# fauzanardh/OsuFusion

Measured on AMD Instinct MI355X. Metric: denoise-steps/sec (train fwd+bwd) at B=32 L=4096, higher is better.
Workload: dtype bf16; 1 GPU; full OsuFusion UNet dim_h=256 (343.5M params) train step: fwd+bwd+grad-norm+clip+AdamW, per-GPU batch 32, L=4096, x (B,6,L), audio (B,96,L) [BASELINE 'audio-ctx=1024x128' maps to the (B,1024,L/8) bottleneck code]; global_batch=32, seq_len=4096, parallelism=dp1

## Files before the change

### include/osufusion_hip.h

```cpp
#ifndef OSUFUSION_HIP_H
#define OSUFUSION_HIP_H

#include <hip/hip_runtime_api.h>

#ifdef __cplusplus
extern "C" {
#endif

#define OSUF_DT_F32 0
#define OSUF_DT_BF16 1
#define OSUF_DT_F32X3 2
#define OSUF_ATTN_AUTO 0
#define OSUF_ATTN_PLAIN 1
#define OSUF_ATTN_PIPE 2
#define OSUF_DQ_ATOMIC 0
#define OSUF_DQ_SLABS 1
#define OSUF_DQ_ATOMIC_256 2
#define OSUF_DQ_ATOMIC_512 3
#define OSUF_DQ_ATOMIC_512A 5
#define OSUF_DQ_PREZEROED 0x100

int osuf_version(void);

int osuf_gemm_nt(int dtype, const void* A, long lda, const void* W, long ldw, long tapstride,
                 void* C, long ldc, void* C2, long ldc2, const void* R, long ldr, const void* U, long ldu,
                 const float* bias, const float* rscale, double* stats,
                 int M, int N, int K, int taps, int Lin, int Lout, int stride, int pad, int mode, int act,
                 hipStream_t stream);

int osuf_gemm_nt_rowdot(int dtype, const void* A, long lda, const void* W, long ldw, void* C, long ldc, const void* O, long ldo,
                        float* delta, int M, int N, int K, int L, int heads, hipStream_t stream);

int osuf_gemm_tn(int dtype, const void* dY, long ldy, const void* X, long ldx, float* dW, long ldw, long tapstride,
                 int M, int N1, int N2, int taps, int Lin, int Lout, int stride, int pad, int mode,
                 int splits, int out_layout, int accumulate, float* workspace, long workspace_bytes, hipStream_t stream);
long osuf_gemm_tn_workspace_bytes(int dtype, int M, int N1, int N2, int taps);
int osuf_gemm_tn_bias(int dtype, const void* dY, long ldy, const void* X, long ldx, float* dW, long ldw, long tapstride,
                      int M, int N1, int N2, int taps, int Lin, int Lout, int stride, int pad, int mode,
                      int splits, int out_layout, int accumulate, float* workspace, long workspace_bytes, float* dbias, hipStream_t stream);

int osuf_colsum(int dtype, const void* Y, long ldy, int M, int N, float* out, hipStream_t stream);

int osuf_gn_finalize(const double* stats, float* mean_rstd, int B, long count, hipStream_t stream);
int osuf_gn_stats(int dtype, const void* y, long ldy, double* partial, float* mean_rstd, int M, int C, int L, hipStream_t stream);
long osuf_gn_stats_workspace_bytes(int M, int C, int L);
int osuf_gn_apply_fwd(int dtype, const void* y, long ldy, void* h, long ldh, const float* mean_rstd, const float* gamma,
                      const float* beta, const float* scale_shift, int M, int C, int L, hipStream_t stream);
int osuf_gn_apply_fwd_stats(int dtype, const void* y, long ldy, void* h, long ldh, const double* stats, long count, float* mr_out,
                            const float* gamma, const float* beta, const float* ss, int M, int C, int L, hipStream_t stream);
int osuf_gn_stats_parts(int dtype, const void* y, long ldy, double* partial, int M, int C, int L, hipStream_t stream);
int osuf_gn_apply_fwd_parts(int dtype, const void* y, long ldy, void* h, long ldh, const double* partial, float* mr_out,
                            const float* gamma, const float* beta, const float* ss, int M, int C, int L, hipStream_t stream);
int osuf_gn_bwd(int dtype, const void* dh, long lddh, const void* y, long ldy, void* dy, long lddy, const float* mean_rstd,
                const float* gamma, const float* beta, const float* scale_shift, float* T1234, float* S, float* dss,
                float* dgamma, float* dbeta, float* dbias, float* dyy, int M, int C, int L, hipStream_t stream);

int osuf_ln_fwd(int dtype, const void* x, long ldx, void* out, long ldo, float* mean_rstd, const float* gamma, const float* beta,
                int M, int C, hipStream_t stream);
int osuf_ln_bwd(int dtype, const void* dy, long lddy, const void* x, long ldx, void* dx, long lddx, const float* mean_rstd,
                const float* gamma, float* dgamma, float* dbeta, int M, int C, hipStream_t stream);

int osuf_rowdot(int dtype, const void* h, long ldh, const float* w, long w_stride, const float* bias, float* out,
                int M, int C, int L, hipStream_t stream);
long osuf_gca_pool_workspace_bytes(int M, int C, int L);
int osuf_gca_pool(int dtype, const void* h, long ldh, const float* wk, const float* bk, float* part, float* p, float* pooled,
                  int M, int C, int L, hipStream_t stream);
int osuf_softmax_rows(float* p, int B, int L, hipStream_t stream);
int osuf_wcolsum(int dtype, const void* a, long lda, const void* bmul, long ldb, const float* w, float* out,
                 int B, int C, int L, float* partial, hipStream_t stream);
int osuf_gate_residual(int dtype, const void* h, long ldh, const float* gate, const void* res, long ldr, void* out, long ldo,
                       int M, int C, int L, hipStream_t stream);
int osuf_gca_bwd_apply(int dtype, const void* dout, long lddo, const void* h, long ldh, void* dh, long lddh, const float* p,
                       const float* gate, const float* dpooled, const float* sdot, const float* wk, float* dlogit,
                       int M, int C, int L, float* dwk, float* dbk, float* workspace, long workspace_bytes, hipStream_t stream);
long osuf_gca_bwd_apply_workspace_bytes(int M, int C);

int osuf_rope_cast(int dtype, const void* in, long ld_in, void* out_bf16, long ld_out, const float* cos_tab, const float* sin_tab,
                   int M, int N, int n_rot_heads, int n_heads_total, int head_dim, hipStream_t stream);
int osuf_rope_cast_qs(int dtype, const void* in, long ld_in, void* out_bf16, long ld_out, const float* cos_tab, const float* sin_tab,
                      int M, int N, int n_rot_heads, int n_heads_total, int head_dim, float q_mul, int n_q_heads, hipStream_t stream);
int osuf_rope_bwd(int dtype, const float* in, long ld_in, void* out, long ld_out, const float* cos_tab, const float* sin_tab,
                  int M, int N, int n_rot_heads, int n_heads_total, int head_dim, hipStream_t stream);
int osuf_mqa_fwd(const void* q, long ldq, const void* k, long ldk, const void* v, long ldv, void* o, long ldo, int o_dtype,
                 float* lse2, int B, int H, int N, int head_dim, float scale, hipStream_t stream);
int osuf_gqa_fwd(const void* q, long ldq, const void* k, long ldk, const void* v, long ldv, void* o, long ldo, int o_dtype,
                 float* lse2, int B, int H, int G, int N, int head_dim, float scale, hipStream_t stream);
int osuf_mqa_fwd_qs(const void* q, long ldq, const void* k, long ldk, const void* v, long ldv, void* o, long ldo, int o_dtype,
                    float* lse2, int B, int H, int N, int head_dim, float scale, hipStream_t stream);
int osuf_mqa_fwd_zdq(const void* q, long ldq, const void* k, long ldk, const void* v, long ldv, void* o, long ldo, int o_dtype,
                     float* lse2, int B, int H, int N, int head_dim, float scale, int qs, float* zero_dq, hipStream_t stream);
int osuf_mqa_fwd_rope(const void* q_raw, long ldq, const void* k, long ldk, const void* v, long ldv, void* o, long ldo, int o_dtype,
                      float* lse2, int B, int H, int N, int head_dim, float scale, const float* rope_cos, const float* rope_sin,
                      float q_mul, void* q_out, long ldqo, float* zero_dq, hipStream_t stream);
int osuf_mqa_fwd_masked(const void* q, long ldq, const void* k, long ldk, const void* v, long ldv, void* o, long ldo, int o_dtype,
                        float* lse2, const void* mask, long mask_b, long mask_h, long mask_q, long mask_k, int B, int H, int N,
                        int head_dim, float scale, hipStream_t stream);
int osuf_mqa_bwd_masked(const void* q, long ldq, const void* k, long ldk, const void* v, long ldv, const void* dout, long lddo,
                        const float* lse2, const float* delta, const void* mask, long mask_b, long mask_h, long mask_q, long mask_k,
                        void* dq, long lddq, void* dk, void* dv, long lddk, int B, int H, int N, int head_dim, float scale,
                        int out_dtype, float* dbias, hipStream_t stream);
int osuf_xattn_fwd(const void* q, long ldq, const void* k, long ldk, const void* v, long ldv, void* o, long ldo, int o_dtype,
                   float* lse2, const void* mask, long mask_b, long mask_h, long mask_q, long mask_k, int B, int H, int Nq, int Nk,
                   int head_dim, float scale, hipStream_t stream);
int osuf_xattn_bwd(const void* q, long ldq, const void* k, long ldk, const void* v, long ldv, const void* dout, long lddo,
                   const float* lse2, const float* delta, const void* mask, long mask_b, long mask_h, long mask_q, long mask_k,
                   void* dq, long lddq, void* dk, void* dv, long lddk, int B, int H, int Nq, int Nk, int head_dim, float scale,
                   int out_dtype, float* dbias, hipStream_t stream);
int osuf_attn_delta(const void* dout, long lddo, const void* o, long ldo, int o_dtype, float* delta, int B, int H, int N,
                    int head_dim, hipStream_t stream);
int osuf_mqa_bwd_dq(const void* q, long ldq, const void* k, long ldk, const void* v, long ldv, const void* dout, long lddo,
                    const float* lse2, const float* delta, void* dq, long lddq, int B, int H, int N, int head_dim, float scale,
                    int out_dtype, const float* rope_cos, const float* rope_sin, int variant, hipStream_t stream);
int osuf_mqa_bwd_dkv(const void* q, long ldq, const void* k, long ldk, const void* v, long ldv, const void* dout, long lddo,
                     const float* lse2, const float* delta, void* dk, void* dv, long lddk, int B, int H, int N, int head_dim,
                     float scale, int out_dtype, const float* rope_cos, const float* rope_sin, float* workspace, long workspace_bytes,
                     int qsplit, int variant, hipStream_t stream);
long osuf_mqa_bwd_dkv_workspace_bytes(int B, int N, int qsplit);

int osuf_mqa_bwd_fused(const void* q, long ldq, const void* k, long ldk, const void* v, long ldv, const void* dout, long lddo,
                       const float* lse2, const float* delta, void* dq, long lddq, void* dk, void* dv, long lddk, int B, int H,
                       int N, int head_dim, float scale, int out_dtype, const float* rope_cos, const float* rope_sin,
                       float* workspace, long workspace_bytes, int qsplit, int dq_mode, hipStream_t stream);
int osuf_mqa_bwd_fused_qs(const void* q, long ldq, const void* k, long ldk, const void* v, long ldv, const void* dout, long lddo,
                          const float* lse2, const float* delta, void* dq, long lddq, void* dk, void* dv, long lddk, int B, int H,
                          int N, int head_dim, float scale, int out_dtype, const float* rope_cos, const float* rope_sin,
                          float* workspace, long workspace_bytes, int qsplit, int dq_mode, hipStream_t stream);
long osuf_mqa_bwd_fused_workspace_bytes(int B, int H, int N, int out_dtype, int qsplit, int dq_mode);

int osuf_ncl_to_rows(int dtype, const float* in, void* out, long ld, int width, int B, int C, int L, int KT, hipStream_t stream);
int osuf_rows_to_ncl(int dtype, const void* in, long ld, float* out, int B, int C, int L, hipStream_t stream);
int osuf_copy2d(int src_dtype, const void* src, long lds, int dst_dtype, void* dst, long ldd, int M, int cols, hipStream_t stream);
int osuf_add2d(int dtype, const void* a, long lda, const void* b, long ldb, void* dst, long ldd, int M, int cols, hipStream_t stream);
int osuf_axpby_rows(const float* x, const float* y, const float* ca, const float* cb, float* out, int B, long per_sample, hipStream_t stream);
int osuf_ddim_step(const float* x, const float* cond, const float* nullp, float cond_scale, const float* coef, float* out,
                   int B, long per_sample, hipStream_t stream);
int osuf_ct_schedule(const float* t, const float* t_next, int kind, float* out, int B, hipStream_t stream);
int osuf_ct_step(const float* x, const float* cond, const float* nullp, float cond_scale, const float* coef, const float* noise,
                 float* out, int B, long per_sample, hipStream_t stream);
#define OSUF_CT_OBJ_NOISE 0
#define OSUF_CT_OBJ_X_START 1
#define OSUF_CT_OBJ_V 2
int osuf_ct_step_ex(const float* x, const float* cond, const float* nullp, float cond_scale, const float* coef, const float* noise,
                    int objective, const float* s, long s_ld, float* out, int B, long per_sample, hipStream_t stream);
int osuf_ct_x0_quantile(const float* x, const float* cond, const float* nullp, float cond_scale, const float* coef, int objective,
                        long k_lo, float frac, float* out, void* workspace, int B, long per_sample, hipStream_t stream);
long osuf_ct_x0_quantile_workspace_bytes(int B);
int osuf_ct_qsample(const float* x0, const float* noise, const float* sched, int sched_ld, int objective, float* x_noisy, float* target,
                    int B, long per_sample, hipStream_t stream);
#define OSUF_CT_SAMPLER_DDIM 0
#define OSUF_CT_SAMPLER_DPMPP_2M 1
int osuf_ct_solver_schedule(const float* log_snr, int steps, int sampler, float eta, float* rows, float* fac, int B, hipStream_t stream);
int osuf_ct_solver_step(const float* x, const float* cond, const float* nullp, float cond_scale, const float* coef, const float* fac,
                        const float* x0_prev, const float* noise, int objective, const float* s, long s_ld, float* x_next, float* x0, int B,
                        long per_sample, hipStream_t stream);
int osuf_mse(const float* pred, const float* target, const int* orig_len, float* grad, double* loss_sum, int B, int Dch, int L,
             hipStream_t stream);
int osuf_mse_w(const float* pred, const float* target, const int* orig_len, const float* w, float* grad, double* loss_sum, int B, int Dch,
               int L, hipStream_t stream);
int osuf_sqnorm(const float* g, long n, double* out, hipStream_t stream);
int osuf_adamw(float* p, const float* g, float* m, float* v, long n, float lr, float beta1, float beta2, float eps, float wd,
               int step, const float* gscale, hipStream_t stream);
int osuf_clip_coef(const double* sumsq, float max_norm, float base, float* coef, float* total_norm, hipStream_t stream);
int osuf_cast_f32_bf16(const float* src, void* dst, long n, hipStream_t stream);
int osuf_pack_weight(const float* w, int O, int I, int k, int out_dtype, void* F, long f_ld, long f_tapstride, void* D, long d_ld,
                     long d_tapstride, int dkind, hipStream_t stream);

#ifndef OSUF_PACK_DESC_DEFINED
#define OSUF_PACK_DESC_DEFINED
typedef struct osuf_pack_desc {
  const float* w;
  void* F;
  void* D;
  long f_ld, f_tapstride, d_ld, d_tapstride;
  int O, I, k, dkind;
  int block0, reserved;
} osuf_pack_desc;
#endif
int osuf_pack_weight_group(const osuf_pack_desc* descs, int n, int total_blocks, int out_dtype, hipStream_t stream);

int osuf_dora_effective(const float* W, const float* A, const float* B, const float* mag, int O, int IK, int r, float scaling,
                        float* Weff, float* g, hipStream_t stream);
int osuf_dora_gain(const float* W, const float* A, const float* B, const float* mag, int O, int I, int k, int r, float scaling,
                   float* partial, float* g, float* sgbt32, void* sgbt16, hipStream_t stream);
int osuf_pack_weight_adapted(const float* w, const float* A, const float* B, const float* g, float scaling, int r, int O, int I, int k,
                             int out_dtype, void* F, long f_ld, long f_tapstride, void* D, long d_ld, long d_tapstride, int dkind,
                             hipStream_t stream);
int osuf_adapter_finish(const float* tb, const float* sg, float* dB, const float* gt, float* dA, const float* s0, const float* s1,
                        const float* bias, const float* m, float* dm, int O, int I, int k, int r, int accumulate, hipStream_t stream);

int osuf_skinny_fwd(int mode, const float* x, long ldx, const float* W, const float* bias, float* y, long ldy, int M, int N, int K,
                    int in_act, int out_act, hipStream_t stream);
int osuf_skinny_bwd(int mode, const float* dy, long lddy, const float* y, long ldy, const float* x, long ldx, const float* W,
                    float* dx, long lddx, float* dW, float* db, int M, int N, int K, int in_act, int out_act, int accumulate,
                    hipStream_t stream);

#ifndef OSUF_LINEAR_DESC_DEFINED
#define OSUF_LINEAR_DESC_DEFINED
typedef struct osuf_linear_desc {
  const float* W;
  const float* bias;
  float* y;
  const float* dy;
  long ldy, lddy;
  int N, block0;
} osuf_linear_desc;
#endif
int osuf_skinny_fwd_group(int mode, const float* x, long ldx, const osuf_linear_desc* descs, int n, int total_blocks, int M, int K,
                          int in_act, hipStream_t stream);
int osuf_skinny_dx_group(int mode, const osuf_linear_desc* descs, int n, int total_slices, const float* x, long ldx, float* dx, long lddx,
                         int M, int K, int in_act, hipStream_t stream);

int osuf_log_vqt(const float* wave_pad, long n_pad, const float* bank, int K, int bins, int hop, const float* scale, float eps,
                 float* spec_ws, float* out, long ldo, long frames, hipStream_t stream);
int osuf_vqt_logmag(const float* spec, long ld, float* out, long ldo, const float* scale, int bins, long frames, float eps,
                    hipStream_t stream);

int osuf_fir_decimate2(const float* in, long n_in, const float* taps, int ntaps, float* out, long n_out, hipStream_t stream);
int osuf_frame_rows(const float* in, long n_in, int hop, int K, float* out, long frames, hipStream_t stream);

int osuf_adaln_fwd(int dtype, const void* x, long ldx, void* out, long ldo, float* mr, const float* shift, const float* scale, long ldm,
                   int M, int C, int L, float eps, hipStream_t stream);
long osuf_adaln_bwd_workspace_bytes(int M, int C, int L);
int osuf_adaln_bwd(int dtype, const void* dy, long lddy, const void* x, long ldx, const void* dres, long ldr, void* dx, long lddx,
                   const float* mr, const float* scale, long ldm, float* dmod, long ldd, long off2, float* workspace, long workspace_bytes,
                   int M, int C, int L, hipStream_t stream);
int osuf_qknorm_fwd(int dtype, const void* x, long ldx, void* y, long ldy, float* inv, const float* gamma_q, const float* gamma_k,
                    int M, int H, int D, hipStream_t stream);
long osuf_qknorm_bwd_workspace_bytes(int M, int H, int D);
int osuf_qknorm_bwd(int dtype, const float* g, long ldg, const void* x, long ldx, const float* inv, const float* gamma_q,
                    const float* gamma_k, void* dx, long lddx, float* dgamma, float* workspace, long workspace_bytes,
                    int M, int H, int D, hipStream_t stream);
int osuf_stat_pool(const float* a, float* out, int B, int C, int L, hipStream_t stream);

int osuf_joint_qknorm_fwd(int dtype, const void* x, long ldx, void* y, long ldy, float* inv, const float* gamma_q, const float* gamma_k,
                          int M, int Ns, int Nj, int off, int H, int G, int D, hipStream_t stream);
int osuf_joint_pack(int dtype, const void* x, long ldx, void* joint, long ldj, int M, int Ns, int Nj, int off, int H, int G, int D,
                    hipStream_t stream);
int osuf_joint_unpack(int dtype, const void* joint, long ldj, void* out, long ldo, int M, int Ns, int Nj, int off, int H, int G, int D,
                      hipStream_t stream);
long osuf_joint_qknorm_bwd_workspace_bytes(int M, int H, int G, int D);
int osuf_joint_qknorm_bwd(int dtype, const float* g, long ldg, const void* x, long ldx, const float* inv, const float* gamma_q,
                          const float* gamma_k, void* dx, long lddx, float* dgamma, float* workspace, long workspace_bytes,
                          int M, int Ns, int Nj, int off, int H, int G, int D, hipStream_t stream);

int osuf_clock_probe(int blocks, int iters, int mode, long* out, hipStream_t stream);

#ifdef __cplusplus
}
#endif
#endif
```

### osufusion_amd/_lib.py

```python
from __future__ import annotations

import ctypes
import os
from ctypes import c_double, c_float, c_int, c_long, c_void_p
from pathlib import Path

_CSRC = Path(__file__).resolve().parent / "csrc"
LIB_PATH = Path(os.environ["OSUF_HIP_LIB"]).resolve() if os.environ.get("OSUF_HIP_LIB") else _CSRC / "libosuf_hip.so"

P, L, I, F = c_void_p, c_long, c_int, c_float

SIGNATURES = {
    "osuf_version": [],
    "osuf_gemm_nt": [I, P, L, P, L, L, P, L, P, L, P, L, P, L, P, P, P, I, I, I, I, I, I, I, I, I, I, P],
    "osuf_gemm_nt_rowdot": [I, P, L, P, L, P, L, P, L, P, I, I, I, I, I, P],
    "osuf_gemm_tn": [I, P, L, P, L, P, L, L, I, I, I, I, I, I, I, I, I, I, I, I, P, L, P],
    "osuf_gemm_tn_bias": [I, P, L, P, L, P, L, L, I, I, I, I, I, I, I, I, I, I, I, I, P, L, P, P],
    "osuf_gemm_tn_workspace_bytes": [I, I, I, I, I],
    "osuf_colsum": [I, P, L, I, I, P, P],
    "osuf_gn_finalize": [P, P, I, L, P],
    "osuf_gn_apply_fwd": [I, P, L, P, L, P, P, P, P, I, I, I, P],
    "osuf_gn_apply_fwd_stats": [I, P, L, P, L, P, L, P, P, P, P, I, I, I, P],
    "osuf_gn_bwd": [I, P, L, P, L, P, L, P, P, P, P, P, P, P, P, P, P, P, I, I, I, P],
    "osuf_ln_fwd": [I, P, L, P, L, P, P, P, I, I, P],
    "osuf_ln_bwd": [I, P, L, P, L, P, L, P, P, P, P, I, I, P],
    "osuf_rowdot": [I, P, L, P, L, P, P, I, I, I, P],
    "osuf_softmax_rows": [P, I, I, P],
    "osuf_wcolsum": [I, P, L, P, L, P, P, I, I, I, P, P],
    "osuf_gn_stats": [I, P, L, P, P, I, I, I, P],
    "osuf_gca_pool": [I, P, L, P, P, P, P, P, I, I, I, P],
    "osuf_gca_pool_workspace_bytes": [I, I, I],
    "osuf_gn_stats_parts": [I, P, L, P, I, I, I, P],
    "osuf_gn_apply_fwd_parts": [I, P, L, P, L, P, P, P, P, P, I, I, I, P],
    "osuf_gn_stats_workspace_bytes": [I, I, I],
    "osuf_gate_residual": [I, P, L, P, P, L, P, L, I, I, I, P],
    "osuf_gca_bwd_apply": [I, P, L, P, L, P, L, P, P, P, P, P, P, I, I, I, P, P, P, L, P],
    "osuf_gca_bwd_apply_workspace_bytes": [I, I],
    "osuf_rope_cast": [I, P, L, P, L, P, P, I, I, I, I, I, P],
    "osuf_rope_cast_qs": [I, P, L, P, L, P, P, I, I, I, I, I, F, I, P],
    "osuf_rope_bwd": [I, P, L, P, L, P, P, I, I, I, I, I, P],
    "osuf_mqa_fwd": [P, L, P, L, P, L, P, L, I, P, I, I, I, I, F, P],
    "osuf_gqa_fwd": [P, L, P, L, P, L, P, L, I, P, I, I, I, I, I, F, P],
    "osuf_mqa_fwd_qs": [P, L, P, L, P, L, P, L, I, P, I, I, I, I, F, P],
    "osuf_mqa_fwd_zdq": [P, L, P, L, P, L, P, L, I, P, I, I, I, I, F, I, P, P],
    "osuf_mqa_fwd_rope": [P, L, P, L, P, L, P, L, I, P, I, I, I, I, F, P, P, F, P, L, P, P],
    "osuf_mqa_fwd_masked": [P, L, P, L, P, L, P, L, I, P, P, L, L, L, L, I, I, I, I, F, P],
    "osuf_mqa_bwd_masked": [P, L, P, L, P, L, P, L, P, P, P, L, L, L, L, P, L, P, P, L, I, I, I, I, F, I, P, P],
    "osuf_xattn_fwd": [P, L, P, L, P, L, P, L, I, P, P, L, L, L, L, I, I, I, I, I, F, P],
    "osuf_xattn_bwd": [P, L, P, L, P, L, P, L, P, P, P, L, L, L, L, P, L, P, P, L, I, I, I, I, I, F, I, P, P],
    "osuf_attn_delta": [P, L, P, L, I, P, I, I, I, I, P],
    "osuf_mqa_bwd_dq": [P, L, P, L, P, L, P, L, P, P, P, L, I, I, I, I, F, I, P, P, I, P],
    "osuf_mqa_bwd_dkv": [P, L, P, L, P, L, P, L, P, P, P, P, L, I, I, I, I, F, I, P, P, P, L, I, I, P],
    "osuf_mqa_bwd_dkv_workspace_bytes": [I, I, I],
    "osuf_mqa_bwd_fused": [P, L, P, L, P, L, P, L, P, P, P, L, P, P, L, I, I, I, I, F, I, P, P, P, L, I, I, P],
    "osuf_mqa_bwd_fused_qs": [P, L, P, L, P, L, P, L, P, P, P, L, P, P, L, I, I, I, I, F, I, P, P, P, L, I, I, P],
    "osuf_mqa_bwd_fused_workspace_bytes": [I, I, I, I, I, I],
    "osuf_ncl_to_rows": [I, P, P, L, I, I, I, I, I, P],
    "osuf_rows_to_ncl": [I, P, L, P, I, I, I, P],
    "osuf_copy2d": [I, P, L, I, P, L, I, I, P],
    "osuf_add2d": [I, P, L, P, L, P, L, I, I, P],
    "osuf_axpby_rows": [P, P, P, P, P, I, L, P],
    "osuf_ddim_step": [P, P, P, F, P, P, I, L, P],
    "osuf_ct_schedule": [P, P, I, P, I, P],
    "osuf_ct_step": [P, P, P, F, P, P, P, I, L, P],
    "osuf_ct_step_ex": [P, P, P, F, P, P, I, P, L, P, I, L, P],
    "osuf_ct_x0_quantile": [P, P, P, F, P, I, L, F, P, P, I, L, P],
    "osuf_ct_x0_quantile_workspace_bytes": [I],
    "osuf_ct_qsample": [P, P, P, I, I, P, P, I, L, P],
    "osuf_ct_solver_schedule": [P, I, I, F, P, P, I, P],
    "osuf_ct_solver_step": [P, P, P, F, P, P, P, P, I, P, L, P, P, I, L, P],
    "osuf_mse": [P, P, P, P, P, I, I, I, P],
    "osuf_mse_w": [P, P, P, P, P, P, I, I, I, P],
    "osuf_sqnorm": [P, L, P, P],
    "osuf_adamw": [P, P, P, P, L, F, F, F, F, F, I, P, P],
    "osuf_clip_coef": [P, F, F, P, P, P],
    "osuf_cast_f32_bf16": [P, P, L, P],
    "osuf_pack_weight": [P, I, I, I, I, P, L, L, P, L, L, I, P],
    "osuf_pack_weight_group": [P, I, I, I, P],
    "osuf_dora_effective": [P, P, P, P, I, I, I, F, P, P, P],
    "osuf_dora_gain": [P, P, P, P, I, I, I, I, F, P, P, P, P, P],
    "osuf_adapter_finish": [P, P, P, P, P, P, P, P, P, P, I, I, I, I, I, P],
    "osuf_pack_weight_adapted": [P, P, P, P, F, I, I, I, I, I, P, L, L, P, L, L, I, P],
    "osuf_clock_probe": [I, I, I, P, P],
    "osuf_log_vqt": [P, L, P, I, I, I, P, F, P, P, L, L, P],
    "osuf_vqt_logmag": [P, L, P, L, P, I, L, F, P],
    "osuf_fir_decimate2": [P, L, P, I, P, L, P],
    "osuf_frame_rows": [P, L, I, I, P, L, P],
    "osuf_skinny_fwd": [I, P, L, P, P, P, L, I, I, I, I, I, P],
    "osuf_skinny_bwd": [I, P, L, P, L, P, L, P, P, L, P, P, I, I, I, I, I, I, P],
    "osuf_skinny_fwd_group": [I, P, L, P, I, I, I, I, I, P],
    "osuf_skinny_dx_group": [I, P, I, I, P, L, P, L, I, I, I, P],
    "osuf_adaln_fwd": [I, P, L, P, L, P, P, P, L, I, I, I, F, P],
    "osuf_adaln_bwd_workspace_bytes": [I, I, I],
    "osuf_adaln_bwd": [I, P, L, P, L, P, L, P, L, P, P, L, P, L, L, P, L, I, I, I, P],
    "osuf_qknorm_fwd": [I, P, L, P, L, P, P, P, I, I, I, P],
    "osuf_qknorm_bwd_workspace_bytes": [I, I, I],
    "osuf_qknorm_bwd": [I, P, L, P, L, P, P, P, P, L, P, P, L, I, I, I, P],
    "osuf_stat_pool": [P, P, I, I, I, P],
    "osuf_joint_qknorm_fwd": [I, P, L, P, L, P, P, P, I, I, I, I, I, I, I, P],
    "osuf_joint_pack": [I, P, L, P, L, I, I, I, I, I, I, I, P],
    "osuf_joint_unpack": [I, P, L, P, L, I, I, I, I, I, I, I, P],
    "osuf_joint_qknorm_bwd_workspace_bytes": [I, I, I, I],
    "osuf_joint_qknorm_bwd": [I, P, L, P, L, P, P, P, P, L, P, P, L, I, I, I, I, I, I, I, P],
}

_lib = None


class HipExtensionMissing(RuntimeError):
    pass


def load(build_if_missing: bool = True) -> ctypes.CDLL:
    global _lib
    if _lib is not None:
        return _lib
    if not LIB_PATH.exists() and build_if_missing:
        try:
            from .csrc import build as _build
            _build.build()
        except Exception as e:
            raise HipExtensionMissing(f"libosuf_hip.so is missing and could not be built: {e}") from e
    if not LIB_PATH.exists():
        raise HipExtensionMissing(f"{LIB_PATH} not found: run `python -c 'import __graft_entry__ as g; g.build()'`")
    try:
        lib = ctypes.CDLL(str(LIB_PATH), mode=os.RTLD_NOW | os.RTLD_LOCAL)
    except OSError as e:
        raise HipExtensionMissing(f"cannot load {LIB_PATH}: {e}") from e
    for name, argtypes in SIGNATURES.items():
        try:
            fn = getattr(lib, name)
        except AttributeError as e:
            raise HipExtensionMissing(f"{LIB_PATH} does not export {name} (stale or partial build of the C ABI)") from e
        fn.argtypes = argtypes
        fn.restype = c_long if name.endswith("_bytes") else c_int
    _lib = lib
    return lib


def check(status: int, what: str) -> None:
    if status != 0:
        kind = {-1: "invalid argument", -2: "unsupported configuration"}.get(status, f"hipError {status}")
        raise RuntimeError(f"{what} failed: {kind}")
```

### osufusion_amd/csrc/common.hpp

```cpp
#pragma once
#include <hip/hip_runtime.h>
#include <stdint.h>

#ifndef OSUF_PACK_DESC_DEFINED
#define OSUF_PACK_DESC_DEFINED
typedef struct osuf_pack_desc {
  const float* w;
  void* F;
  void* D;
  long f_ld, f_tapstride, d_ld, d_tapstride;
  int O, I, k, dkind;
  int block0, reserved;
} osuf_pack_desc;
#endif
static_assert(sizeof(osuf_pack_desc) == 80, "osuf_pack_desc is part of the C ABI");
#ifndef OSUF_LINEAR_DESC_DEFINED
#define OSUF_LINEAR_DESC_DEFINED
typedef struct osuf_linear_desc {
  const float* W;
  const float* bias;
  float* y;
  const float* dy;
  long ldy, lddy;
  int N, block0;
} osuf_linear_desc;
#endif
static_assert(sizeof(osuf_linear_desc) == 56, "osuf_linear_desc is part of the C ABI");

#define OSUF_DT_F32 0
#define OSUF_DT_BF16 1
#define OSUF_DT_F32X3 2
#define OSUF_ATTN_AUTO 0
#define OSUF_ATTN_PLAIN 1
#define OSUF_ATTN_PIPE 2
#define OSUF_DQ_ATOMIC 0
#define OSUF_DQ_SLABS 1
#define OSUF_DQ_ATOMIC_256 2
#define OSUF_DQ_ATOMIC_512 3
#define OSUF_DQ_ATOMIC_512A 5
#define OSUF_DQ_PREZEROED 0x100

typedef uint16_t bf16_t;
typedef __attribute__((ext_vector_type(4))) float f32x4;
typedef __attribute__((ext_vector_type(16))) float f32x16;
typedef __attribute__((ext_vector_type(8))) __bf16 bf16x8;
typedef __attribute__((ext_vector_type(4))) short s16x4;
typedef __attribute__((ext_vector_type(4))) uint32_t u32x4;
typedef __attribute__((ext_vector_type(2))) uint32_t u32x2;

#define LDS_PTR(T) __attribute__((address_space(3))) T*

__device__ __forceinline__ float bf16_to_f32(bf16_t v) { return __uint_as_float(((uint32_t)v) << 16); }

__device__ __forceinline__ bf16_t f32_to_bf16(float f) {
  __bf16 b = (__bf16)f;
  return __builtin_bit_cast(uint16_t, b);
}
__device__ __forceinline__ uint32_t pack_bf16x2(float lo, float hi) {
  typedef __attribute__((ext_vector_type(2))) float f32x2_t;
  typedef __attribute__((ext_vector_type(2))) __bf16 bf16x2_t;
  f32x2_t v = {lo, hi};
  return __builtin_bit_cast(uint32_t, __builtin_convertvector(v, bf16x2_t));
}
__device__ __forceinline__ float round_bf16(float f) { return bf16_to_f32(f32_to_bf16(f)); }

template <typename T> struct ElemTraits;
template <> struct ElemTraits<float> {
  static constexpr int kPer16B = 4;
  __device__ static __forceinline__ float load(const float* p) { return *p; }
  __device__ static __forceinline__ void store(float* p, float v) { *p = v; }
  __device__ static __forceinline__ float rnd(float v) { return v; }
};
template <> struct ElemTraits<bf16_t> {
  static constexpr int kPer16B = 8;
  __device__ static __forceinline__ float load(const bf16_t* p) { return bf16_to_f32(*p); }
  __device__ static __forceinline__ void store(bf16_t* p, float v) { *p = f32_to_bf16(v); }
  __device__ static __forceinline__ float rnd(float v) { return round_bf16(v); }
};

__device__ __forceinline__ void load8(const bf16_t* p, float (&v)[8]) {
  u32x4 r = *reinterpret_cast<const u32x4*>(p);
#pragma unroll
  for (int i = 0; i < 4; ++i) {
    v[2 * i] = __uint_as_float(r[i] << 16);
    v[2 * i + 1] = __uint_as_float(r[i] & 0xFFFF0000u);
  }
}
__device__ __forceinline__ void load8(const float* p, float (&v)[8]) {
  f32x4 a = *reinterpret_cast<const f32x4*>(p);
  f32x4 b = *reinterpret_cast<const f32x4*>(p + 4);
#pragma unroll
  for (int i = 0; i < 4; ++i) { v[i] = a[i]; v[4 + i] = b[i]; }
}
__device__ __forceinline__ void store8(bf16_t* p, const float (&v)[8]) {
  u32x4 r;
#pragma unroll
  for (int i = 0; i < 4; ++i) r[i] = pack_bf16x2(v[2 * i], v[2 * i + 1]);
  *reinterpret_cast<u32x4*>(p) = r;
}
__device__ __forceinline__ void store8(float* p, const float (&v)[8]) {
  f32x4 a, b;
#pragma unroll
  for (int i = 0; i < 4; ++i) { a[i] = v[i]; b[i] = v[4 + i]; }
  *reinterpret_cast<f32x4*>(p) = a;
  *reinterpret_cast<f32x4*>(p + 4) = b;
}
__device__ __forceinline__ void load4(const bf16_t* p, float (&v)[4]) {
  u32x2 r = *reinterpret_cast<const u32x2*>(p);
  v[0] = __uint_as_float(r[0] << 16); v[1] = __uint_as_float(r[0] & 0xFFFF0000u);
  v[2] = __uint_as_float(r[1] << 16); v[3] = __uint_as_float(r[1] & 0xFFFF0000u);
}
__device__ __forceinline__ void load4(const float* p, float (&v)[4]) {
  f32x4 a = *reinterpret_cast<const f32x4*>(p);
  v[0] = a[0]; v[1] = a[1]; v[2] = a[2]; v[3] = a[3];
}
__device__ __forceinline__ void store4(bf16_t* p, const float (&v)[4]) {
  u32x2 r; r[0] = pack_bf16x2(v[0], v[1]); r[1] = pack_bf16x2(v[2], v[3]);
  *reinterpret_cast<u32x2*>(p) = r;
}
__device__ __forceinline__ void store4(float* p, const float (&v)[4]) {
  f32x4 a; a[0] = v[0]; a[1] = v[1]; a[2] = v[2]; a[3] = v[3];
  *reinterpret_cast<f32x4*>(p) = a;
}

__device__ __forceinline__ float sigmoid_f(float x) { return __builtin_amdgcn_rcpf(1.0f + __expf(-x)); }
__device__ __forceinline__ float silu_f(float x) { return x * sigmoid_f(x); }
__device__ __forceinline__ float silu_grad_f(float x) {
  float s = sigmoid_f(x);
  return s * (1.0f + x * (1.0f - s));
}

template <int WIDTH = 64> __device__ __forceinline__ float group_sum(float v) {
#pragma unroll
  for (int o = WIDTH >> 1; o > 0; o >>= 1) v += __shfl_xor(v, o, 64);
  return v;
}
template <int WIDTH = 64> __device__ __forceinline__ float group_max(float v) {
#pragma unroll
  for (int o = WIDTH >> 1; o > 0; o >>= 1) v = fmaxf(v, __shfl_xor(v, o, 64));
  return v;
}
__device__ __forceinline__ float group_sum_dyn(float v, int width) {
  for (int o = width >> 1; o > 0; o >>= 1) v += __shfl_xor(v, o, 64);
  return v;
}
__device__ __forceinline__ float group_max_dyn(float v, int width) {
  for (int o = width >> 1; o > 0; o >>= 1) v = fmaxf(v, __shfl_xor(v, o, 64));
  return v;
}

__device__ __forceinline__ void atomic_add_f64(double* p, double v) { unsafeAtomicAdd(p, v); }
__device__ __forceinline__ void atomic_add_f32(float* p, float v) { unsafeAtomicAdd(p, v); }

#define OSUF_OK 0
#define OSUF_EINVAL (-1)
#define OSUF_EUNSUPPORTED (-2)

static inline int osuf_launch_status() {
  hipError_t e = hipGetLastError();
  return e == hipSuccess ? OSUF_OK : (int)e;
}

#define DISPATCH_T(dtype, ...)                                  \
  if ((dtype) == OSUF_DT_BF16) { using T = bf16_t; __VA_ARGS__; } \
  else if ((dtype) == OSUF_DT_F32) { using T = float; __VA_ARGS__; } \
  else return OSUF_EUNSUPPORTED;
static inline int ew_grid(long total_threads) {
  long blocks = (total_threads + 255) / 256;
  if (blocks > 2048) blocks = 2048;
  if (blocks < 1) blocks = 1;
  return (int)blocks;
}
static inline bool al16(const void* p) { return (reinterpret_cast<uintptr_t>(p) & 15) == 0; }
static inline bool bad_c(int C) { return C <= 0 || (C & 7) || C > 2048; }

template <auto KERNEL> static void allow_lds(int bytes) {
  static const bool once = ((void)hipFuncSetAttribute((const void*)KERNEL, hipFuncAttributeMaxDynamicSharedMemorySize, bytes), true);
  (void)once;
}
```

### osufusion_amd/csrc/gemm.hip

```cpp
#include "common.hpp"
#include <optional>
#include <stdlib.h>

struct RowMap {
  int Lin, Lout, stride, pad, mode;
};
__device__ __forceinline__ int map_row(const RowMap& rm, int i, int t) {
  if (rm.mode == 3) {
    if (t == 3) return (i == rm.Lout - 2) ? rm.Lin - 1 : -1;
    int e = i - t;
    if (e < 0 || (e & 1)) return -1;
    e >>= 1;
    return e < rm.Lin ? e : -1;
  }
  int s = i * rm.stride + t - rm.pad;
  if (rm.mode == 2) {
    if (s < 0 || s >= 2 * rm.Lin) return -1;
    return s >> 1;
  }
  if (rm.mode == 1 && s == rm.Lin) s = rm.Lin - 2;
  return (s >= 0 && s < rm.Lin) ? s : -1;
}

struct GemmArgs {
// ... 1651 lines not shown
  asm volatile("s_waitcnt lgkmcnt(" #n ")"                                                                        \
               : "+v"(fa[slot][0][0]), "+v"(fa[slot][0][1]), "+v"(fa[slot][1][0]), "+v"(fa[slot][1][1]), "+v"(fb[slot][0][0]),  \
                 "+v"(fb[slot][0][1]), "+v"(fb[slot][1][0]), "+v"(fb[slot][1][1]), "+v"(fb[slot][2][0]), "+v"(fb[slot][2][1]));  \
  __builtin_amdgcn_sched_barrier(0);
#define T3_MFMA(slot)                                                                                             \
  _Pragma("unroll") for (int i = 0; i < 2; ++i) _Pragma("unroll") for (int t = 0; t < 3; ++t) {                   \
    u32x4 va = {fa[slot][i][0][0], fa[slot][i][0][1], fa[slot][i][1][0], fa[slot][i][1][1]};                       \
    u32x4 vb = {fb[slot][t][0][0], fb[slot][t][0][1], fb[slot][t][1][0], fb[slot][t][1][1]};                       \
    acc[i][t] = __builtin_amdgcn_mfma_f32_32x32x16_bf16(__builtin_bit_cast(bf16x8, va), __builtin_bit_cast(bf16x8, vb), acc[i][t], 0, 0, 0); \
  }

  const bool do_bias = g.dbias != nullptr && n2_0 == 0 && wc == 0;
  float bsum[2] = {0.f, 0.f};
#define T3_BIAS(slot)                                                                                             \
  if (do_bias) { _Pragma("unroll") for (int i = 0; i < 2; ++i) bsum[i] = bf16x8_sum(fa[slot][i][0], fa[slot][i][1], bsum[i]); }
  issue(m_begin, 0);
  asm volatile("s_waitcnt vmcnt(0)" ::: "memory");
  __builtin_amdgcn_s_barrier();
  int buf = 0;
  for (int mb = m_begin; mb < m_end; mb += BKM, buf ^= 1) {
    if (mb + BKM < m_end) issue(mb + BKM, buf ^ 1);
    const uint32_t base = lds0 + buf * STAGE;
    T3_READS(0, 0, base)
    T3_READS(1, 1, base)
    T3_WAIT(0, 10)  T3_MFMA(0)  T3_BIAS(0)  T3_READS(0, 2, base)
    T3_WAIT(1, 10)  T3_MFMA(1)  T3_BIAS(1)  T3_READS(1, 3, base)
    T3_WAIT(0, 10)  T3_MFMA(0)  T3_BIAS(0)  T3_READS(0, 4, base)
    T3_WAIT(1, 10)  T3_MFMA(1)  T3_BIAS(1)  T3_READS(1, 5, base)
    T3_WAIT(0, 10)  T3_MFMA(0)  T3_BIAS(0)  T3_READS(0, 6, base)
    T3_WAIT(1, 10)  T3_MFMA(1)  T3_BIAS(1)  T3_READS(1, 7, base)
    T3_WAIT(0, 10)  T3_MFMA(0)  T3_BIAS(0)
    T3_WAIT(1, 0)   T3_MFMA(1)  T3_BIAS(1)
    asm volatile("s_waitcnt vmcnt(0)" ::: "memory");
    __builtin_amdgcn_s_barrier();
  }
#undef T3_READS
#undef T3_WAIT
#undef T3_MFMA
#undef T3_BIAS
  if (do_bias) {
#pragma unroll
    for (int i = 0; i < 2; ++i) {
      const float v = bsum[i] + __shfl_xor(bsum[i], 32, 64);
      const int n1 = n1_0 + wr * 64 + i * 32 + lr;
      if (lh == 0 && n1 < g.N1) atomic_add_f32(g.dbias + n1, v);
    }
  }

  if (g.ws && g.ws_pk) {
#pragma unroll
    for (int t = 0; t < 3; ++t) {
      uint32_t* out = reinterpret_cast<uint32_t*>(g.ws) + ((long)split * 3 + t) * (g.N1 >> 1) * g.N2;
#pragma unroll
      for (int i = 0; i < 2; ++i) {
        const int n2 = n2_0 + wc * 32 + lr;
        if (n2 < g.N2) {
#pragma unroll
          for (int r = 0; r < 16; r += 2) {
            const int n1 = n1_0 + wr * 64 + i * 32 + (r & 3) + 8 * (r >> 2) + 4 * lh;
            if (n1 < g.N1) out[(long)(n1 >> 1) * g.N2 + n2] = pack_bf16x2(acc[i][t][r], acc[i][t][r + 1]);
          }
        }
      }
    }
    return;
  }
#pragma unroll
  for (int t = 0; t < 3; ++t) {
    float* out = g.ws ? g.ws + ((long)split * 3 + t) * g.N1 * g.N2 : g.dW + (long)t * g.tapstride;
#pragma unroll
    for (int i = 0; i < 2; ++i) {
      const int n2 = n2_0 + wc * 32 + lr;
      if (n2 < g.N2) {
#pragma unroll
        for (int r = 0; r < 16; ++r) {
          const int n1 = n1_0 + wr * 64 + i * 32 + (r & 3) + 8 * (r >> 2) + 4 * lh;
          if (n1 < g.N1) {
            if (g.ws) out[(long)n1 * g.N2 + n2] = acc[i][t][r];
            else atomic_add_f32(out + (long)n1 * g.ldw + (long)n2 * g.es, acc[i][t][r]);
          }
        }
      }
    }
  }
}

__global__ __launch_bounds__(512, 2) void gemm_tn_taps3_x3_kernel(WgradArgs g) {
  extern __shared__ __attribute__((aligned(16))) char smem[];
  constexpr int BKM = 64, ROWB = 512, YB = BKM * ROWB, XROWS = 66, STAGE = YB + XROWS * ROWB;
  const int tid = threadIdx.x, lane = tid & 63;
  const int wave = __builtin_amdgcn_readfirstlane(tid >> 6);
  const int wr = wave >> 2, wc = wave & 3;
  const WgradUnit u = wgrad_unit<128>(g, 1);
  const int split = u.split, n1_0 = u.n1_0, n2_0 = u.n2_0, m_begin = u.m_begin, m_end = u.m_end;
  if (m_begin >= m_end) return;
  const float* dY = reinterpret_cast<const float*>(g.dY);
  const float* X = reinterpret_cast<const float*>(g.X);
  const char* zero = reinterpret_cast<const char*>(g_zero_page);
  const int L = g.rm.Lout;
  const int col = (lane & 31) * 4;
  const bool y_ok = n1_0 + col < g.N1, x_ok = n2_0 + col < g.N2;
  int pos = m_begin % L;
  auto issue = [&](int mb, int buf) {
    char* sy = smem + buf * STAGE;
    char* sx = sy + YB;
#pragma unroll
    for (int i = 0; i < 4; ++i) {
      const int m = mb + (wave * 4 + i) * 2 + (lane >> 5);
      const char* qy = (m < m_end && y_ok) ? reinterpret_cast<const char*>(dY + (long)m * g.ldy + n1_0 + col) : zero;
      __builtin_amdgcn_global_load_lds((gas_ptr)qy, (las_ptr)(sy + (wave * 4 + i) * 1024), 16, 0, 0);
    }
#pragma unroll
    for (int i = 0; i < 5; ++i) {
      if (i == 4 && wave != 0) break;
      const int gi = i < 4 ? wave * 4 + i : 32;
      const int pr = gi * 2 + (lane >> 5);
      const int q = pos - 1 + pr;
      const bool ok = q >= 0 && q < L && mb - 1 + pr < g.M && x_ok;
      const char* qx = ok ? reinterpret_cast<const char*>(X + (long)(mb - 1 + pr) * g.ldx + n2_0 + col) : zero;
      __builtin_amdgcn_global_load_lds((gas_ptr)qx, (las_ptr)(sx + gi * 1024), 16, 0, 0);
    }
    pos += BKM;
    if (pos >= L) pos -= L;
  };

  f32x16 acc[2][3];
  zero_acc(acc);

  const int lr = lane & 31, lh = lane >> 5;
  issue(m_begin, 0);
  asm volatile("s_waitcnt vmcnt(0)" ::: "memory");
  __builtin_amdgcn_s_barrier();
  int buf = 0;
  for (int mb = m_begin; mb < m_end; mb += BKM, buf ^= 1) {
    if (mb + BKM < m_end) issue(mb + BKM, buf ^ 1);
    const char* sy = smem + buf * STAGE;
    const char* sx = sy + YB;
#pragma unroll
    for (int kk = 0; kk < 4; ++kk) {
      bf16x8 ah[2], al[2], bh[3], bl[3];
      {
        typedef __attribute__((ext_vector_type(2))) float f32x2;
        f32x2 y[8];
#pragma unroll
        for (int e = 0; e < 8; ++e) y[e] = *reinterpret_cast<const f32x2*>(sy + (16 * kk + 8 * lh + e) * ROWB + (wr * 64 + 2 * lr) * 4);
#pragma unroll
        for (int i = 0; i < 2; ++i) {
          const float x[8] = {y[0][i], y[1][i], y[2][i], y[3][i], y[4][i], y[5][i], y[6][i], y[7][i]};
          split_bf16x8(x, ah[i], al[i]);
        }
      }
      {
        float xw[10];
#pragma unroll
        for (int e = 0; e < 10; ++e) xw[e] = *reinterpret_cast<const float*>(sx + (16 * kk + 8 * lh + e) * ROWB + (wc * 32 + lr) * 4);
#pragma unroll
        for (int t = 0; t < 3; ++t) {
          const float x[8] = {xw[t], xw[t + 1], xw[t + 2], xw[t + 3], xw[t + 4], xw[t + 5], xw[t + 6], xw[t + 7]};
          split_bf16x8(x, bh[t], bl[t]);
        }
      }
#pragma unroll
      for (int i = 0; i < 2; ++i)
#pragma unroll
        for (int t = 0; t < 3; ++t) mfma_x3(acc[i][t], ah[i], al[i], bh[t], bl[t]);
    }
    asm volatile("s_waitcnt vmcnt(0)" ::: "memory");
    __builtin_amdgcn_s_barrier();
  }
#pragma unroll
  for (int t = 0; t < 3; ++t) {
    float* out = g.ws ? g.ws + ((long)split * 3 + t) * g.N1 * g.N2 : g.dW + (long)t * g.tapstride;
#pragma unroll
    for (int i = 0; i < 2; ++i) {
      const int n2 = n2_0 + wc * 32 + lr;
      if (n2 < g.N2) {
#pragma unroll
        for (int r = 0; r < 16; ++r) {
          const int n1 = n1_0 + wr * 64 + 2 * ((r & 3) + 8 * (r >> 2) + 4 * lh) + i;
          if (n1 < g.N1) {
            if (g.ws) out[(long)n1 * g.N2 + n2] = acc[i][t][r];
            else atomic_add_f32(out + (long)n1 * g.ldw + (long)n2 * g.es, acc[i][t][r]);
          }
        }
      }
    }
  }
}

__global__ __launch_bounds__(512, 2) void gemm_tn_skinny_kernel(WgradArgs g) {
  extern __shared__ __attribute__((aligned(16))) char smem[];
  constexpr int BKM = 64, ROWB = 512, TILEB = BKM * ROWB, XTILEB = BKM * 64, STAGE = TILEB + XTILEB;
  const int tid = threadIdx.x, lane = tid & 63;
  const int wave = __builtin_amdgcn_readfirstlane(tid >> 6);
  const int tiles_n1 = (g.N1 + kBig - 1) / kBig;
  const int tile = blockIdx.x % tiles_n1;
  const int t = (blockIdx.x / tiles_n1) % g.taps;
  const int split = blockIdx.x / (tiles_n1 * g.taps);
  const int n1_0 = tile * kBig;
  const int m_begin = split * g.rows_per_split;
  const int m_end = min(g.M, m_begin + g.rows_per_split);
  if (m_begin >= m_end) return;
  const bf16_t* dY = reinterpret_cast<const bf16_t*>(g.dY);
  const bf16_t* X = reinterpret_cast<const bf16_t*>(g.X);
  const char* zero = reinterpret_cast<const char*>(g_zero_page);

  int srow[4], scol[4];
  const char* py[4];
  bool y_ok[4];
#pragma unroll
  for (int i = 0; i < 4; ++i) {
    srow[i] = (wave * 4 + i) * 2 + (lane >> 5);
    scol[i] = ((lane & 31) ^ ((srow[i] & 3) << 2)) * 8;
    y_ok[i] = n1_0 + scol[i] < g.N1;
    py[i] = reinterpret_cast<const char*>(dY + (long)(m_begin + srow[i]) * g.ldy + n1_0 + scol[i]);
  }
  const long ystep = (long)BKM * g.ldy * (long)sizeof(bf16_t);
  const int xrow = wave * 16 + (lane >> 2), xcol = (lane & 3) * 8;
  const bool x_ok = wave < 4 && xcol < g.N2;
  int xb = 0, xp = 0;
  if (wave < 4) { const int m = m_begin + xrow; xb = m / g.rm.Lout; xp = m - xb * g.rm.Lout; }
  auto issue = [&](int mb, int buf) {
    char* sy = smem + buf * STAGE + wave * 4096;
#pragma unroll
    for (int i = 0; i < 4; ++i) {
      const char* qy = (mb + srow[i] < m_end && y_ok[i]) ? py[i] : zero;
      __builtin_amdgcn_global_load_lds((gas_ptr)qy, (las_ptr)(sy + i * 1024), 16, 0, 0);
      py[i] += ystep;
    }
    if (wave < 4) {
      const char* qx = zero;
      if (x_ok && mb + xrow < m_end) {
        const int s2 = map_row(g.rm, xp, t);
        if (s2 >= 0) qx = reinterpret_cast<const char*>(X + (long)(xb * g.rm.Lin + s2) * g.ldx + xcol);
      }
      __builtin_amdgcn_global_load_lds((gas_ptr)qx, (las_ptr)(smem + buf * STAGE + TILEB + wave * 1024), 16, 0, 0);
      xp += BKM;
      while (xp >= g.rm.Lout) { xp -= g.rm.Lout; ++xb; }
    }
  };

  f32x16 acc;
#pragma unroll
  for (int r = 0; r < 16; ++r) acc[r] = 0.f;
  const int lr = lane & 31, lh = lane >> 5;
  const int ip = lane & 15, cb = ((lane >> 4) & 1) * 16, tq = ip >> 2, tp = ip & 3;
  const uint32_t lds0 = (uint32_t)(uintptr_t)(LDS_PTR(char))smem;
  const uint32_t offA = (8 * lh + tq) * ROWB + ((((wave * 32 + cb + 4 * tp) * 2)) ^ (tq << 6));
  const uint32_t offB = TILEB + (8 * lh + tq) * 64 + (cb + 4 * tp) * 2;

  issue(m_begin, 0);
  asm volatile("s_waitcnt vmcnt(0)" ::: "memory");
  __builtin_amdgcn_s_barrier();
  int buf = 0;
  for (int mb = m_begin; mb < m_end; mb += BKM, buf ^= 1) {
    if (mb + BKM < m_end) issue(mb + BKM, buf ^ 1);
    const uint32_t base = lds0 + buf * STAGE;
    u32x2 a0[4], a1[4], b0[4], b1[4];
    OSUF_TR_READ(a0[0], base + offA, 0 * 16 * 512);  OSUF_TR_READ(a1[0], base + offA, (0 * 16 + 4) * 512);
    OSUF_TR_READ(b0[0], base + offB, 0 * 16 * 64);   OSUF_TR_READ(b1[0], base + offB, (0 * 16 + 4) * 64);
    OSUF_TR_READ(a0[1], base + offA, 1 * 16 * 512);  OSUF_TR_READ(a1[1], base + offA, (1 * 16 + 4) * 512);
    OSUF_TR_READ(b0[1], base + offB, 1 * 16 * 64);   OSUF_TR_READ(b1[1], base + offB, (1 * 16 + 4) * 64);
    OSUF_TR_READ(a0[2], base + offA, 2 * 16 * 512);  OSUF_TR_READ(a1[2], base + offA, (2 * 16 + 4) * 512);
    OSUF_TR_READ(b0[2], base + offB, 2 * 16 * 64);   OSUF_TR_READ(b1[2], base + offB, (2 * 16 + 4) * 64);
    OSUF_TR_READ(a0[3], base + offA, 3 * 16 * 512);  OSUF_TR_READ(a1[3], base + offA, (3 * 16 + 4) * 512);
    OSUF_TR_READ(b0[3], base + offB, 3 * 16 * 64);   OSUF_TR_READ(b1[3], base + offB, (3 * 16 + 4) * 64);
    asm volatile("s_waitcnt lgkmcnt(0)"
                 : "+v"(a0[0]), "+v"(a1[0]), "+v"(b0[0]), "+v"(b1[0]), "+v"(a0[1]), "+v"(a1[1]), "+v"(b0[1]), "+v"(b1[1]),
                   "+v"(a0[2]), "+v"(a1[2]), "+v"(b0[2]), "+v"(b1[2]), "+v"(a0[3]), "+v"(a1[3]), "+v"(b0[3]), "+v"(b1[3]));
#pragma unroll
    for (int ks = 0; ks < 4; ++ks) {
      const u32x4 va = {a0[ks][0], a0[ks][1], a1[ks][0], a1[ks][1]};
      const u32x4 vb = {b0[ks][0], b0[ks][1], b1[ks][0], b1[ks][1]};
      acc = __builtin_amdgcn_mfma_f32_32x32x16_bf16(__builtin_bit_cast(bf16x8, va), __builtin_bit_cast(bf16x8, vb), acc, 0, 0, 0);
    }
    asm volatile("s_waitcnt vmcnt(0)" ::: "memory");
    __builtin_amdgcn_s_barrier();
  }
  float* dW = g.dW + (long)t * g.tapstride;
  if (lr < g.N2) {
#pragma unroll
    for (int r = 0; r < 16; ++r) {
      const int n1 = n1_0 + wave * 32 + (r & 3) + 8 * (r >> 2) + 4 * lh;
      if (n1 < g.N1) atomic_add_f32(dW + (long)n1 * g.ldw + (long)lr * g.es, acc[r]);
    }
  }
}

__device__ __forceinline__ f32x4 sum_partials(const float* p, long stride, int splits) {
  f32x4 a0 = {0.f, 0.f, 0.f, 0.f}, a1 = a0, a2 = a0, a3 = a0;
  int sidx = 0;
  for (; sidx + 4 <= splits; sidx += 4) {
    const f32x4 b0 = *reinterpret_cast<const f32x4*>(p + (long)sidx * stride);
    const f32x4 b1 = *reinterpret_cast<const f32x4*>(p + (long)(sidx + 1) * stride);
    const f32x4 b2 = *reinterpret_cast<const f32x4*>(p + (long)(sidx + 2) * stride);
    const f32x4 b3 = *reinterpret_cast<const f32x4*>(p + (long)(sidx + 3) * stride);
    a0 += b0; a1 += b1; a2 += b2; a3 += b3;
  }
  for (; sidx < splits; ++sidx) a0 += *reinterpret_cast<const f32x4*>(p + (long)sidx * stride);
  return (a0 + a1) + (a2 + a3);
}

template <int LAYOUT>
__global__ __launch_bounds__(256) void wgrad_reduce_kernel(const float* ws, float* dW, long n12, int taps, int splits, int accumulate) {
  if constexpr (LAYOUT == 0) {
    const long n = n12 * taps, n4 = n >> 2;
    for (long i = (long)blockIdx.x * blockDim.x + threadIdx.x; i < n4; i += (long)gridDim.x * blockDim.x) {
      f32x4 a = sum_partials(ws + 4 * i, n, splits);
      if (accumulate) a += reinterpret_cast<f32x4*>(dW)[i];
      reinterpret_cast<f32x4*>(dW)[i] = a;
    }
  } else {
    const long n = n12 * taps, q12 = n12 >> 2;
    for (long q = (long)blockIdx.x * blockDim.x + threadIdx.x; q < q12; q += (long)gridDim.x * blockDim.x) {
      if (taps == 3) {
        f32x4 a[3];
#pragma unroll
        for (int t = 0; t < 3; ++t) a[t] = sum_partials(ws + (long)t * n12 + 4 * q, n, splits);
        f32x4* dst = reinterpret_cast<f32x4*>(dW + 12 * q);
        f32x4 o0 = {a[0][0], a[1][0], a[2][0], a[0][1]}, o1 = {a[1][1], a[2][1], a[0][2], a[1][2]}, o2 = {a[2][2], a[0][3], a[1][3], a[2][3]};
        if (accumulate) { o0 += dst[0]; o1 += dst[1]; o2 += dst[2]; }
        dst[0] = o0; dst[1] = o1; dst[2] = o2;
      } else {
        for (int t = 0; t < taps; ++t) {
          const f32x4 a = sum_partials(ws + (long)t * n12 + 4 * q, n, splits);
#pragma unroll
          for (int e = 0; e < 4; ++e) {
            float* dst = dW + (4 * q + e) * taps + t;
            *dst = accumulate ? *dst + a[e] : a[e];
          }
        }
      }
    }
  }
}

template <int LAYOUT>
__global__ __launch_bounds__(256) void wgrad_reduce4_kernel(const float* ws, float* dW, long n12, int taps, int splits, int accumulate) {
  __shared__ f32x4 red[3][3][64];
  const int tq = threadIdx.x & 63, ts = threadIdx.x >> 6;
  const long n = n12 * taps;
  const int mine = (splits - ts + 3) >> 2;
  if constexpr (LAYOUT == 0) {
    const long n4 = n >> 2;
    const long i = (long)blockIdx.x * 64 + tq;
    const long ic = min(i, n4 - 1);
    f32x4 a = sum_partials(ws + (long)ts * n + 4 * ic, 4 * n, mine);
    if (ts) red[ts - 1][0][tq] = a;
    __syncthreads();
    if (ts == 0 && i < n4) {
      a = ((a + red[0][0][tq]) + red[1][0][tq]) + red[2][0][tq];
      if (accumulate) a += reinterpret_cast<f32x4*>(dW)[i];
      reinterpret_cast<f32x4*>(dW)[i] = a;
    }
  } else {
    const long q12 = n12 >> 2;
    const long q = (long)blockIdx.x * 64 + tq;
    const long qc = min(q, q12 - 1);
    f32x4 a[3];
#pragma unroll
    for (int t = 0; t < 3; ++t) a[t] = sum_partials(ws + (long)ts * n + (long)t * n12 + 4 * qc, 4 * n, mine);
    if (ts) {
#pragma unroll
      for (int t = 0; t < 3; ++t) red[ts - 1][t][tq] = a[t];
    }
    __syncthreads();
    if (ts == 0 && q < q12) {
#pragma unroll
      for (int t = 0; t < 3; ++t) a[t] = ((a[t] + red[0][t][tq]) + red[1][t][tq]) + red[2][t][tq];
      f32x4* dst = reinterpret_cast<f32x4*>(dW + 12 * q);
      f32x4 o0 = {a[0][0], a[1][0], a[2][0], a[0][1]}, o1 = {a[1][1], a[2][1], a[0][2], a[1][2]}, o2 = {a[2][2], a[0][3], a[1][3], a[2][3]};
      if (accumulate) { o0 += dst[0]; o1 += dst[1]; o2 += dst[2]; }
      dst[0] = o0; dst[1] = o1; dst[2] = o2;
    }
  }
}

template <int LAYOUT, int NT>
__global__ __launch_bounds__(256) void wgrad_reduce_pk_kernel(const uint32_t* ws, float* dW, int N1, int N2, int taps, int splits, int accumulate) {
  __shared__ f32x4 red[3][2 * NT][64];
  const int tq = threadIdx.x & 63, ts = threadIdx.x >> 6;
  const long quads = N2 >> 2, per_tap = (long)(N1 >> 1) * quads, groups = NT == 3 ? per_tap : per_tap * taps;
  const long gi = (long)blockIdx.x * 64 + tq, gc = min(gi, groups - 1);
  const int t0 = NT == 3 ? 0 : (int)(gc / per_tap);
  const long rem = gc - (long)t0 * per_tap;
  const long p = rem / quads, q = rem - p * quads;
  const long tile = (long)(N1 >> 1) * N2, stride = tile * taps;
  const uint32_t* src = ws + (long)t0 * tile + p * N2 + 4 * q;
  f32x4 ev[NT], od[NT];
#pragma unroll
  for (int t = 0; t < NT; ++t) { ev[t] = f32x4{0.f, 0.f, 0.f, 0.f}; od[t] = ev[t]; }
  for (int sidx = ts; sidx < splits; sidx += 4) {
    u32x4 a[NT];
#pragma unroll
    for (int t = 0; t < NT; ++t) a[t] = *reinterpret_cast<const u32x4*>(src + (long)sidx * stride + (long)t * tile);
#pragma unroll
    for (int t = 0; t < NT; ++t)
#pragma unroll
      for (int e = 0; e < 4; ++e) {
        ev[t][e] += __builtin_bit_cast(float, a[t][e] << 16);
        od[t][e] += __builtin_bit_cast(float, a[t][e] & 0xffff0000u);
      }
  }
  if (ts) {
#pragma unroll
    for (int t = 0; t < NT; ++t) { red[ts - 1][2 * t][tq] = ev[t]; red[ts - 1][2 * t + 1][tq] = od[t]; }
  }
  __syncthreads();
  if (ts == 0 && gi < groups) {
#pragma unroll
    for (int t = 0; t < NT; ++t) {
      ev[t] = ((ev[t] + red[0][2 * t][tq]) + red[1][2 * t][tq]) + red[2][2 * t][tq];
      od[t] = ((od[t] + red[0][2 * t + 1][tq]) + red[1][2 * t + 1][tq]) + red[2][2 * t + 1][tq];
    }
#pragma unroll
    for (int h = 0; h < 2; ++h) {
      const long n1 = 2 * p + h;
      if constexpr (NT == 3) {
        const f32x4 a0 = h ? od[0] : ev[0], a1 = h ? od[1] : ev[1], a2 = h ? od[2] : ev[2];
        f32x4* dst = reinterpret_cast<f32x4*>(dW + (n1 * N2 + 4 * q) * 3);
        f32x4 o0 = {a0[0], a1[0], a2[0], a0[1]}, o1 = {a1[1], a2[1], a0[2], a1[2]}, o2 = {a2[2], a0[3], a1[3], a2[3]};
        if (accumulate) { o0 += dst[0]; o1 += dst[1]; o2 += dst[2]; }
        dst[0] = o0; dst[1] = o1; dst[2] = o2;
      } else if constexpr (LAYOUT == 0) {
        const f32x4 v = h ? od[0] : ev[0];
        f32x4* dst = reinterpret_cast<f32x4*>(dW + ((long)t0 * N1 + n1) * N2 + 4 * q);
        *dst = accumulate ? *dst + v : v;
      } else {
        const f32x4 v = h ? od[0] : ev[0];
#pragma unroll
        for (int e = 0; e < 4; ++e) {
          float* dst = dW + (n1 * N2 + 4 * q + e) * taps + t0;
          *dst = accumulate ? *dst + v[e] : v[e];
        }
      }
    }
  }
}

static void launch_wgrad_reduce(const WgradArgs& gb, float* dW, int N1, int N2, int taps, int sp, int out_layout, int accumulate, bool many_splits_ok,
                                hipStream_t stream) {
  const long n12 = (long)N1 * N2, n = n12 * taps;
  if (gb.ws_pk) {
    const uint32_t* w = reinterpret_cast<const uint32_t*>(gb.ws);
    const long per_tap = (long)(N1 >> 1) * (N2 >> 2);
    if (out_layout == 1 && taps == 3) hipLaunchKernelGGL((wgrad_reduce_pk_kernel<1, 3>), dim3((int)((per_tap + 63) / 64)), dim3(256), 0, stream, w, dW, N1, N2, taps, sp, accumulate);
    else if (out_layout == 1) hipLaunchKernelGGL((wgrad_reduce_pk_kernel<1, 1>), dim3((int)((per_tap * taps + 63) / 64)), dim3(256), 0, stream, w, dW, N1, N2, taps, sp, accumulate);
    else hipLaunchKernelGGL((wgrad_reduce_pk_kernel<0, 1>), dim3((int)((per_tap * taps + 63) / 64)), dim3(256), 0, stream, w, dW, N1, N2, taps, sp, accumulate);
    return;
  }
  const long groups = out_layout == 1 ? n12 / 4 : n / 4;
  long blocks = (groups + 255) / 256;
  if (blocks > 2048) blocks = 2048;
  if (sp >= 8 && blocks < 512 && many_splits_ok) {
    const long b4 = (groups + 63) / 64;
    if (out_layout == 1) hipLaunchKernelGGL(wgrad_reduce4_kernel<1>, dim3((int)b4), dim3(256), 0, stream, gb.ws, dW, n12, taps, sp, accumulate);
    else hipLaunchKernelGGL(wgrad_reduce4_kernel<0>, dim3((int)b4), dim3(256), 0, stream, gb.ws, dW, n12, taps, sp, accumulate);
  } else if (out_layout == 1) hipLaunchKernelGGL(wgrad_reduce_kernel<1>, dim3((int)blocks), dim3(256), 0, stream, gb.ws, dW, n12, taps, sp, accumulate);
  else hipLaunchKernelGGL(wgrad_reduce_kernel<0>, dim3((int)blocks), dim3(256), 0, stream, gb.ws, dW, n12, taps, sp, accumulate);
}

template <typename T>
__global__ __launch_bounds__(256) void colsum_kernel(const T* Y, long ldy, int M, int N, float* out, int rows_per_block) {
  const int cchunk = blockIdx.x * 32 + (threadIdx.x & 31);
  const int rl = threadIdx.x >> 5;
  const int n = cchunk * 8;
  const int m_begin = blockIdx.y * rows_per_block;
  const int m_end = min(M, m_begin + rows_per_block);
  float acc[8] = {0, 0, 0, 0, 0, 0, 0, 0};
  if (n < N) {
    int m = m_begin + rl;
    for (; m + 24 < m_end; m += 32) {
      float v0[8], v1[8], v2[8], v3[8];
      load8(Y + (long)m * ldy + n, v0);
      load8(Y + (long)(m + 8) * ldy + n, v1);
      load8(Y + (long)(m + 16) * ldy + n, v2);
      load8(Y + (long)(m + 24) * ldy + n, v3);
#pragma unroll
      for (int e = 0; e < 8; ++e) acc[e] += (v0[e] + v1[e]) + (v2[e] + v3[e]);
    }
    for (; m < m_end; m += 8) {
      float v[8];
      load8(Y + (long)m * ldy + n, v);
#pragma unroll
      for (int e = 0; e < 8; ++e) acc[e] += v[e];
    }
  }
  __shared__ float red[8][32 * 8 + 1];
#pragma unroll
  for (int e = 0; e < 8; ++e) red[rl][(threadIdx.x & 31) * 8 + e] = acc[e];
  __syncthreads();
  const int col = threadIdx.x;
  float s = 0.f;
#pragma unroll
  for (int r = 0; r < 8; ++r) s += red[r][col];
  const int nn = blockIdx.x * 256 + col;
  if (nn < N) atomic_add_f32(out + nn, s);
}

static bool aligned16(const void* p) { return (reinterpret_cast<uintptr_t>(p) & 15) == 0; }

static std::optional<long> big_min_tiles_override() {
  const char* s = getenv("OSUF_GEMM_BIG_MIN_TILES");
  if (!s) return std::nullopt;
  return atol(s);
}

static int gemm_nt_launch(int dtype, const void* A, long lda, const void* W, long ldw, long tapstride,
                          void* C, long ldc, void* C2, long ldc2, const void* R, long ldr, const void* U, long ldu,
                          const float* bias, const float* rscale, double* stats,
                          int M, int N, int K, int taps, int Lin, int Lout, int stride, int pad, int mode, int act,
                          float* delta, int heads, hipStream_t stream) {
  const int epc = dtype == OSUF_DT_BF16 ? 8 : 4;
  if (dtype != OSUF_DT_BF16 && dtype != OSUF_DT_F32 && dtype != OSUF_DT_F32X3) return OSUF_EUNSUPPORTED;
  if (M <= 0 || N <= 0 || K <= 0 || taps <= 0 || Lout <= 0 || Lin <= 0) return OSUF_EINVAL;
  if (M % Lout != 0) return OSUF_EINVAL;
  if (K % epc || lda % epc || ldw % epc || tapstride % epc || N % 4 || ldc % 4) return OSUF_EINVAL;
  if ((C2 && ldc2 % 4) || (R && ldr % 4) || (U && ldu % 4)) return OSUF_EINVAL;
  if (!aligned16(A) || !aligned16(W) || !aligned16(C) || (bias && !aligned16(bias)) || (rscale && !aligned16(rscale))) return OSUF_EINVAL;
  if ((long)(M / Lout) * Lin >= (1L << 31)) return OSUF_EINVAL;
  GemmArgs g;
  g.A = A; g.W = W; g.C = C; g.C2 = C2; g.R = R; g.U = U; g.bias = bias; g.rscale = rscale; g.stats = stats;
  g.delta = delta; g.heads = heads;
  g.lda = lda; g.ldw = ldw; g.tapstride = tapstride; g.ldc = ldc; g.ldc2 = ldc2; g.ldr = ldr; g.ldu = ldu;
  g.M = M; g.N = N; g.K = K; g.taps = taps;
  g.rm = RowMap{Lin, Lout, stride, pad, mode};
  g.act = act;
  const int grid = ((M + kTile - 1) / kTile) * ((N + kTile - 1) / kTile);
  const int lds = 2 * kStageBytes + 512;
  allow_lds<gemm_nt_glds_kernel<bf16_t>>(lds);
  allow_lds<gemm_nt_glds_kernel<float>>(lds);
  allow_lds<gemm_nt_glds_kernel<float, true>>(lds);
  if (dtype == OSUF_DT_BF16 && N <= 32 && N % 8 == 0 && ldc % 8 == 0 && M >= 4096 && !C2 && !R && !U && !bias && !rscale && !stats &&
      act == 0) {
    const int lds_sk = 2 * kSkStage;
    allow_lds<gemm_nt_skinny_kernel>(lds_sk);
    hipLaunchKernelGGL(gemm_nt_skinny_kernel, dim3((M + kBig - 1) / kBig), dim3(512), lds_sk, stream, g);
    return osuf_launch_status();
  }
  const std::optional<long> bigenv = big_min_tiles_override();
  const long min_tiles = bigenv.value_or(192);
  const long big_tiles = (long)((M + kBig - 1) / kBig) * ((N + kBig - 1) / kBig);
  const bool use_big = (dtype == OSUF_DT_BF16 || dtype == OSUF_DT_F32X3) && min_tiles > 0 && big_tiles >= min_tiles && (N >= 192 || bigenv) && N % 8 == 0 &&
                       ldc % 8 == 0 && (!C2 || ldc2 % 8 == 0) && (!R || ldr % 8 == 0) && (!U || ldu % 8 == 0) &&
                       (!bias || (reinterpret_cast<uintptr_t>(bias) & 31) == 0) && (!rscale || (reinterpret_cast<uintptr_t>(rscale) & 31) == 0);
  if (use_big) {
    const int lds_big = 2 * kBigStage + 2112;
    const int lds_p8 = kP8Tbl + taps * kBig * 4;
    allow_lds<gemm_nt_big_kernel<bf16_t>>(lds_big);
    allow_lds<gemm_nt_big_kernel<float, true>>(lds_big);
    const long tm = (M + kBig - 1) / kBig, tn = (N + kBig - 1) / kBig;
    const dim3 grid_big((int)(((tm + 7) / 8) * 8 * tn));
    const bool halo3 = taps == 3 && mode == 0 && stride == 1 && pad == 1 && Lin == Lout && Lout % kBig == 0 && K % (dtype == OSUF_DT_BF16 ? 64 : 32) == 0 &&
                       getenv("OSUF_GEMM_NOHALO") == nullptr;
    if (halo3) {
      allow_lds<gemm_nt_big_halo3_kernel<bf16_t>>(lds_big);
      allow_lds<gemm_nt_big_halo3_kernel<float>>(lds_big);
      if (dtype == OSUF_DT_BF16 && getenv("OSUF_GEMM_NO8P") == nullptr && K <= 8192) {
        const int lds_h8 = kH8B + 65536 + 2112;
        allow_lds<gemm_nt_big8_halo3_kernel>(lds_h8);
        hipLaunchKernelGGL(gemm_nt_big8_halo3_kernel, grid_big, dim3(512), lds_h8, stream, g);
      } else if (dtype == OSUF_DT_BF16) hipLaunchKernelGGL(gemm_nt_big_halo3_kernel<bf16_t>, grid_big, dim3(512), lds_big, stream, g);
      else hipLaunchKernelGGL(gemm_nt_big_halo3_kernel<float>, grid_big, dim3(512), lds_big, stream, g);
    } else if (dtype == OSUF_DT_BF16 && getenv("OSUF_GEMM_NO8P") == nullptr && taps <= kP8MaxTaps && K <= 8192 && K % 64 == 0) {
      allow_lds<gemm_nt_big8_kernel>(kP8Tbl + kP8MaxTaps * kBig * 4);
      hipLaunchKernelGGL(gemm_nt_big8_kernel, grid_big, dim3(512), lds_p8, stream, g);
    } else if (dtype == OSUF_DT_F32X3) hipLaunchKernelGGL((gemm_nt_big_kernel<float, true>), grid_big, dim3(512), lds_big, stream, g);
    else hipLaunchKernelGGL(gemm_nt_big_kernel<bf16_t>, grid_big, dim3(512), lds_big, stream, g);
  } else {
    if (dtype == OSUF_DT_BF16) hipLaunchKernelGGL(gemm_nt_glds_kernel<bf16_t>, dim3(grid), dim3(256), lds, stream, g);
    else if (dtype == OSUF_DT_F32X3) hipLaunchKernelGGL((gemm_nt_glds_kernel<float, true>), dim3(grid), dim3(256), lds, stream, g);
    else hipLaunchKernelGGL(gemm_nt_glds_kernel<float>, dim3(grid), dim3(256), lds, stream, g);
  }
  return osuf_launch_status();
}

extern "C" int osuf_gemm_nt(int dtype, const void* A, long lda, const void* W, long ldw, long tapstride,
                            void* C, long ldc, void* C2, long ldc2, const void* R, long ldr, const void* U, long ldu,
                            const float* bias, const float* rscale, double* stats,
                            int M, int N, int K, int taps, int Lin, int Lout, int stride, int pad, int mode, int act,
                            hipStream_t stream) {
  return gemm_nt_launch(dtype, A, lda, W, ldw, tapstride, C, ldc, C2, ldc2, R, ldr, U, ldu, bias, rscale, stats, M, N, K, taps, Lin, Lout,
                        stride, pad, mode, act, nullptr, 0, stream);
}

extern "C" int osuf_gemm_nt_rowdot(int dtype, const void* A, long lda, const void* W, long ldw, void* C, long ldc, const void* O, long ldo,
                                   float* delta, int M, int N, int K, int L, int heads, hipStream_t stream) {
  if (!O || !delta || heads <= 0 || N != heads * 64 || L <= 0 || !aligned16(O) || ldo % 8) return OSUF_EINVAL;
  return gemm_nt_launch(dtype, A, lda, W, ldw, 0, C, ldc, nullptr, 0, O, ldo, nullptr, 0, nullptr, nullptr, nullptr, M, N, K, 1, L, L, 1, 0, 0, 0,
                        delta, heads, stream);
}

static bool tn_big_plan(int dtype, int M, int N1, int N2, int taps, int* rows_out, int* splits_out) {
  const std::optional<long> bigenv = big_min_tiles_override();
  const bool forced = bigenv == 1, off = bigenv && *bigenv <= 0;
  if ((dtype != OSUF_DT_BF16 && dtype != OSUF_DT_F32X3) || off || !(forced || (N1 >= 64 && N2 >= 64 && (N1 >= 192 || N2 >= 192)))) return false;
  const int btiles = ((N1 + kBig - 1) / kBig) * ((N2 + kBig - 1) / kBig);
  int sp = (256 + btiles * taps / 2) / (btiles * taps);
  if (sp < 1) sp = 1;
  while (sp > 1 && ((sp * btiles + 7) / 8) * 8 * taps > 256) --sp;
  int rows = (M + sp - 1) / sp;
  rows = ((rows + 63) / 64) * 64;
  if (rows_out) *rows_out = rows;
  if (splits_out) *splits_out = (M + rows - 1) / rows;
  return true;
}

extern "C" long osuf_gemm_tn_workspace_bytes(int dtype, int M, int N1, int N2, int taps) {
  int rows, sp;
  if (M <= 0 || N1 <= 0 || N2 <= 0 || taps <= 0 || !tn_big_plan(dtype, M, N1, N2, taps, &rows, &sp)) return 0;
  if ((N1 * (long)N2 * taps) % 4) return 0;
  return (long)sp * taps * N1 * N2 * (long)sizeof(float);
}
static bool wgrad_pk(int dtype, int N1, int N2) {
  return dtype == OSUF_DT_BF16 && (N1 % 2) == 0 && (N2 % 4) == 0 && getenv("OSUF_WGRAD_F32_PARTIALS") == nullptr;
}

extern "C" int osuf_colsum(int dtype, const void* Y, long ldy, int M, int N, float* out, hipStream_t stream) {
  if (M <= 0 || N <= 0 || N % 8 || ldy % 8 || !aligned16(Y)) return OSUF_EINVAL;
  const int rows_per_block = 256;
  dim3 grid((N + 255) / 256, (M + rows_per_block - 1) / rows_per_block);
  if (dtype == OSUF_DT_BF16) {
    hipLaunchKernelGGL(colsum_kernel<bf16_t>, grid, dim3(256), 0, stream, (const bf16_t*)Y, ldy, M, N, out, rows_per_block);
  } else if (dtype == OSUF_DT_F32) {
    hipLaunchKernelGGL(colsum_kernel<float>, grid, dim3(256), 0, stream, (const float*)Y, ldy, M, N, out, rows_per_block);
  } else {
    return OSUF_EUNSUPPORTED;
  }
  return osuf_launch_status();
}

static int gemm_tn_launch(int dtype, const void* dY, long ldy, const void* X, long ldx, float* dW, long ldw, long tapstride,
                          int M, int N1, int N2, int taps, int Lin, int Lout, int stride, int pad, int mode,
                          int splits, int out_layout, int accumulate, float* workspace, long workspace_bytes, float* dbias, hipStream_t stream) {
  long es = 1;
  if (out_layout == 1) { ldw = (long)N2 * taps; tapstride = 1; es = taps; }
  else if (out_layout != 0) return OSUF_EINVAL;
  const int epc = dtype == OSUF_DT_BF16 ? 8 : 4;
  if (dtype != OSUF_DT_BF16 && dtype != OSUF_DT_F32 && dtype != OSUF_DT_F32X3) return OSUF_EUNSUPPORTED;
  if (M <= 0 || N1 <= 0 || N2 <= 0 || taps <= 0 || Lout <= 0 || Lin <= 0 || M % Lout) return OSUF_EINVAL;
  if (N1 % epc || N2 % epc || ldy % epc || ldx % epc) return OSUF_EINVAL;
  if (!aligned16(dY) || !aligned16(X)) return OSUF_EINVAL;
  auto bias_by_colsum = [&]() -> int {
    return dbias ? osuf_colsum(dtype == OSUF_DT_BF16 ? OSUF_DT_BF16 : OSUF_DT_F32, dY, ldy, M, N1, dbias, stream) : OSUF_OK;
  };
  auto wgrad_args = [&](int rows_per_split) {
    WgradArgs a{};
    a.dY = dY; a.X = X; a.dW = dW; a.es = es; a.ldy = ldy; a.ldx = ldx; a.ldw = ldw; a.tapstride = tapstride;
    a.M = M; a.N1 = N1; a.N2 = N2; a.taps = taps; a.rm = RowMap{Lin, Lout, stride, pad, mode};
    a.rows_per_split = rows_per_split;
    return a;
  };
  auto plan_partials = [&](WgradArgs& gb, int sp) -> int {
    const long n = (long)taps * N1 * N2;
    const bool dense = (out_layout == 1 && ((long)N1 * N2) % 4 == 0) ||
                       (out_layout == 0 && ldw == N2 && (taps == 1 || tapstride == (long)N1 * N2) && n % 4 == 0 && aligned16(dW));
    gb.ws = (workspace && dense && aligned16(workspace) && workspace_bytes >= (long)sp * n * (long)sizeof(float)) ? workspace : nullptr;
    gb.ws_pk = gb.ws && wgrad_pk(dtype, N1, N2);
    gb.dbias = dtype == OSUF_DT_BF16 ? dbias : nullptr;
    if (dtype != OSUF_DT_BF16) { if (int rc = bias_by_colsum()) return rc; }
    if (!gb.ws && !accumulate) (void)hipMemsetAsync(dW, 0, (size_t)n * sizeof(float), stream);
    return OSUF_OK;
  };
  const int bkm = dtype == OSUF_DT_BF16 ? 64 : 32;
  if (splits <= 0 && dtype == OSUF_DT_BF16 && N2 <= 32 && M >= 4096) {
    const int tiles_n1 = (N1 + kBig - 1) / kBig;
    int sp = 512 / (tiles_n1 * taps);
    if (sp < 1) sp = 1;
    int rows = (M + sp - 1) / sp;
    rows = ((rows + 63) / 64) * 64;
    if (rows < 256) rows = 256;
    sp = (M + rows - 1) / rows;
    WgradArgs gs = wgrad_args(rows);
    if (!accumulate) {
      if (out_layout == 0 && !(ldw == N2 && (taps == 1 || tapstride == (long)N1 * N2))) return OSUF_EINVAL;
      (void)hipMemsetAsync(dW, 0, (size_t)taps * N1 * N2 * sizeof(float), stream);
    }
    const int lds_sk = 2 * (64 * 512 + 64 * 64);
    allow_lds<gemm_tn_skinny_kernel>(lds_sk);
    hipLaunchKernelGGL(gemm_tn_skinny_kernel, dim3(tiles_n1 * taps * sp), dim3(512), lds_sk, stream, gs);
    if (int rc = bias_by_colsum()) return rc;
    return osuf_launch_status();
  }
  if (splits <= 0 && (dtype == OSUF_DT_BF16 || dtype == OSUF_DT_F32X3) && taps == 3 && mode == 0 && stride == 1 && pad == 1 && Lin == Lout && Lout % 128 == 0 && N1 >= 64 &&
      N2 >= 64 && tn_big_plan(dtype, M, N1, N2, taps, nullptr, nullptr) && getenv("OSUF_GEMM_NOHALO") == nullptr) {
    const int btiles = ((N1 + 127) / 128) * ((N2 + 127) / 128);
    int sp = 256 / btiles;
    if (sp < 1) sp = 1;
    int rows = (M + sp - 1) / sp;
    rows = ((rows + 127) / 128) * 128;
    sp = (M + rows - 1) / rows;
    WgradArgs gb = wgrad_args(rows);
    if (int rc = plan_partials(gb, sp)) return rc;
    const int lds_t3 = 2 * (128 * 256 + 132 * 256);
    allow_lds<gemm_tn_taps3_kernel>(lds_t3);
    allow_lds<gemm_tn_taps3_x3_kernel>(lds_t3);
    const dim3 grid_t3(((sp * btiles + 7) / 8) * 8);
    if (dtype == OSUF_DT_F32X3) hipLaunchKernelGGL(gemm_tn_taps3_x3_kernel, grid_t3, dim3(512), lds_t3, stream, gb);
    else hipLaunchKernelGGL(gemm_tn_taps3_kernel, grid_t3, dim3(512), lds_t3, stream, gb);
    if (gb.ws) launch_wgrad_reduce(gb, dW, N1, N2, taps, sp, out_layout, accumulate, true, stream);
    return osuf_launch_status();
  }
  {
    int rows, sp;
    if (splits <= 0 && tn_big_plan(dtype, M, N1, N2, taps, &rows, &sp)) {
      WgradArgs gb = wgrad_args(rows);
      if (int rc = plan_partials(gb, sp)) return rc;
      const int btiles = ((N1 + kBig - 1) / kBig) * ((N2 + kBig - 1) / kBig);
      const int lds_big = 2 * 65536;
      allow_lds<gemm_tn_big_kernel>(lds_big);
      allow_lds<gemm_tn_big_x3_kernel>(lds_big);
      if (dtype == OSUF_DT_F32X3) hipLaunchKernelGGL(gemm_tn_big_x3_kernel, dim3(((sp * btiles + 7) / 8) * 8 * taps), dim3(512), lds_big, stream, gb);
      else hipLaunchKernelGGL(gemm_tn_big_kernel, dim3(((sp * btiles + 7) / 8) * 8 * taps), dim3(512), lds_big, stream, gb);
      if (gb.ws) launch_wgrad_reduce(gb, dW, N1, N2, taps, sp, out_layout, accumulate, out_layout == 0 || taps == 3, stream);
      return osuf_launch_status();
    }
  }
  const int tiles = ((N1 + kTile - 1) / kTile) * ((N2 + kTile - 1) / kTile);
  if (splits <= 0) {
    splits = (768 + tiles * taps - 1) / (tiles * taps);
  }
  int rows = (M + splits - 1) / splits;
  rows = ((rows + bkm - 1) / bkm) * bkm;
  splits = (M + rows - 1) / rows;
  const WgradArgs g = wgrad_args(rows);
  if (!accumulate) {
    if (out_layout == 0 && !(ldw == N2 && (taps == 1 || tapstride == (long)N1 * N2))) return OSUF_EINVAL;
    (void)hipMemsetAsync(dW, 0, (size_t)taps * N1 * N2 * sizeof(float), stream);
  }
  if (int rc = bias_by_colsum()) return rc;
  const int lds = 4 * 16384;
  if (dtype == OSUF_DT_BF16) {
    hipLaunchKernelGGL(gemm_tn_kernel<bf16_t>, dim3(tiles, taps, splits), dim3(256), lds, stream, g);
  } else if (dtype == OSUF_DT_F32X3) {
    hipLaunchKernelGGL((gemm_tn_kernel<float, true>), dim3(tiles, taps, splits), dim3(256), lds, stream, g);
  } else {
    hipLaunchKernelGGL(gemm_tn_kernel<float>, dim3(tiles, taps, splits), dim3(256), lds, stream, g);
  }
  return osuf_launch_status();
}

extern "C" int osuf_gemm_tn(int dtype, const void* dY, long ldy, const void* X, long ldx, float* dW, long ldw, long tapstride,
                            int M, int N1, int N2, int taps, int Lin, int Lout, int stride, int pad, int mode,
                            int splits, int out_layout, int accumulate, float* workspace, long workspace_bytes, hipStream_t stream) {
  return gemm_tn_launch(dtype, dY, ldy, X, ldx, dW, ldw, tapstride, M, N1, N2, taps, Lin, Lout, stride, pad, mode, splits, out_layout, accumulate,
                        workspace, workspace_bytes, nullptr, stream);
}

extern "C" int osuf_gemm_tn_bias(int dtype, const void* dY, long ldy, const void* X, long ldx, float* dW, long ldw, long tapstride,
                                 int M, int N1, int N2, int taps, int Lin, int Lout, int stride, int pad, int mode,
                                 int splits, int out_layout, int accumulate, float* workspace, long workspace_bytes, float* dbias,
                                 hipStream_t stream) {
  if (!dbias) return OSUF_EINVAL;
  return gemm_tn_launch(dtype, dY, ldy, X, ldx, dW, ldw, tapstride, M, N1, N2, taps, Lin, Lout, stride, pad, mode, splits, out_layout, accumulate,
                        workspace, workspace_bytes, dbias, stream);
}
```

### osufusion_amd/functional.py

```python
from __future__ import annotations

import weakref
from typing import Dict, Optional, Tuple

import torch

from . import ops
from .tracing import scope

_WEIGHT_EPOCH = 0


def bump_weight_epoch() -> None:
    global _WEIGHT_EPOCH
    _WEIGHT_EPOCH += 1


class PackCache:

    def __init__(self) -> None:
        self._d: Dict[Tuple, Tuple] = {}

    def get(self, key: Tuple, params: Tuple[torch.Tensor, ...], builder) -> torch.Tensor:
        ver = (_WEIGHT_EPOCH, *[(p._version, p.data_ptr()) for p in params])
        hit = self._d.get(key)
        if hit is not None and hit[0] == ver:
            return hit[1]
        with torch.no_grad():
            t = builder().contiguous()
        self._d[key] = (ver, t, None)
        return t

    def packs(self, key: Tuple, params: Tuple[torch.Tensor, ...], weights, kind: str, dt: torch.dtype):
        ver = (_WEIGHT_EPOCH, *[(p._version, p.data_ptr()) for p in params])
        hit = self._d.get(key)
        if hit is not None and hit[0] == ver:
            if hit[2] is not None:
                hit[2].used = True
            return hit[1]
        ws = weights if isinstance(weights, (tuple, list)) else (weights,)
        with torch.no_grad():
            if len(ws) == 1:
                pair = _pack_one(ws[0], dt, kind)
            else:
                I = ws[0].shape[1]
                total = sum(w.shape[0] for w in ws)
                dev = ws[0].device
                fwd = torch.empty((1, total, I), dtype=dt, device=dev)
                dgr = torch.empty((1, I, total), dtype=dt, device=dev)
                off = 0
                for w in ws:
                    _pack_one(w, dt, kind, fwd=fwd, dgrad=dgr, row_offset=off)
                    off += w.shape[0]
                pair = (fwd, dgr)
        job = None
        if all(_plain_master(w, params) for w in ws):
            job = _PackJob(self, key, tuple(params), tuple(ws), kind, dt, pair)
            _PACK_JOBS[(id(self), key)] = job
        self._d[key] = (ver, pair, job)
        return pair


def _plain_master(w, params=()) -> bool:
    return (isinstance(w, torch.nn.Parameter) and any(w is p for p in params) and w.dtype == torch.float32
            and w.is_contiguous() and w.is_cuda)


class _PackJob:
    __slots__ = ("cache", "key", "params", "ws", "kind", "dt", "pair", "used")

    def __init__(self, cache, key, params, ws, kind, dt, pair) -> None:
        self.cache, self.key, self.params, self.ws, self.kind, self.dt, self.pair = weakref.ref(cache), key, params, ws, kind, dt, pair
        self.used = True


_PACK_JOBS: Dict[Tuple, _PackJob] = {}
_PACK_TABLES: Dict[torch.dtype, Tuple] = {}


def refresh_packs() -> int:
    by_dt: Dict[torch.dtype, list] = {}
    for k, job in list(_PACK_JOBS.items()):
        cache = job.cache()
        ent = cache._d.get(job.key) if cache is not None else None
        if ent is None or ent[2] is not job:
            del _PACK_JOBS[k]
            continue
        if job.used:
            by_dt.setdefault(job.dt, []).append(job)
    done = 0
    with torch.no_grad():
        for dt, jobs in by_dt.items():
            sig = tuple((id(j), tuple(w.data_ptr() for w in j.ws)) for j in jobs)
            tab = _PACK_TABLES.get(dt)
            if tab is None or tab[0] != sig:
                items = []
                for j in jobs:
                    off = 0
                    for w in j.ws:
                        items.append((w.detach(), j.kind, j.pair[0], j.pair[1], off))
                        off += w.shape[0]
                dev, n, blocks = ops.pack_desc_table(items, dt, jobs[0].ws[0].device)
                tab = (sig, dev, n, blocks)
                _PACK_TABLES[dt] = tab
            ops.pack_weight_group(tab[1], tab[2], tab[3], dt)
            for j in jobs:
                ver = (_WEIGHT_EPOCH, *[(p._version, p.data_ptr()) for p in j.params])
                j.cache()._d[j.key] = (ver, j.pair, j)
                j.used = False
            done += len(jobs)
    return done


def _pack_one(w, dt, kind, **kw):
    if isinstance(w, EffWeight):
        ad = w.ad
        return ops.pack_weight(ad.w.detach().float().contiguous(), dt, kind, adapt=(ad.a.detach().float().contiguous(),
                               ad.b.detach().float().contiguous(), w.g if ad.m is not None else None, ad.scaling), **kw)
    return ops.pack_weight(w.detach().float().contiguous(), dt, kind, **kw)


class EffWeight:

    def __init__(self, ad, g) -> None:
        self.ad, self.g, self.shape, self.device = ad, g, ad.w.shape, ad.w.device

    def dim(self) -> int:
        return len(self.shape)


_DIRECT = False
_GRAD_DONE_CB = None
_GRAD_COMPLETE_CB = None
_PENDING_USES: Dict[int, int] = {}


def enable_direct_grads(flag: bool, done_callback=None, complete_callback=None) -> None:
    global _DIRECT, _GRAD_DONE_CB, _GRAD_COMPLETE_CB
    _DIRECT, _GRAD_DONE_CB, _GRAD_COMPLETE_CB = bool(flag), done_callback, complete_callback
    _PENDING_USES.clear()


def grad_use(p: torch.Tensor) -> None:
    _PENDING_USES[id(p)] = _PENDING_USES.get(id(p), 0) + 1


def grad_used(p: torch.Tensor) -> None:
    left = _PENDING_USES.get(id(p), 1) - 1
    if left > 0:
        _PENDING_USES[id(p)] = left
        return
    _PENDING_USES.pop(id(p), None)
    if _GRAD_DONE_CB is not None:
        _GRAD_DONE_CB(p)
    if _GRAD_COMPLETE_CB is not None:
        _GRAD_COMPLETE_CB(p)


def reset_grad_uses() -> None:
    _PENDING_USES.clear()


def grad_target(p: Optional[torch.Tensor]) -> Optional[torch.Tensor]:
    if not _DIRECT or p is None or not p.is_leaf or not p.requires_grad:
        return None
    g = p.grad
    if g is None or g.dtype != torch.float32 or g.shape != p.shape or not g.is_contiguous():
        return None
    return g


def grad_done(p: torch.Tensor) -> None:
    if _GRAD_DONE_CB is not None:
        _GRAD_DONE_CB(p)


def _bias_grad(dy: torch.Tensor, bias: Optional[torch.Tensor], n: Optional[int] = None):
    tgt = grad_target(bias)
    if tgt is not None:
        ops.colsum(dy, n, out=tgt)
        grad_done(bias)
        return None
    return ops.colsum(dy, n)


def _rc(t: torch.Tensor) -> torch.Tensor:
    if t.stride(-1) != 1 or (t.dim() == 3 and t.shape[0] > 1 and t.stride(0) != t.shape[1] * t.stride(1)) or t.data_ptr() % 16:
        return t.contiguous()
    if t.dim() == 3 and t.stride(1) % 8:
        return t.contiguous()
    return t


_CONV_KINDS = {
    "same": dict(stride=1, mode=0),
    "down": dict(stride=2, mode=1),
    "up": dict(stride=1, mode=2),
}


def _conv_geom(kind: str, k: int, Lin: int) -> Tuple[int, int, int, int]:
    if kind == "same":
        return Lin, 1, k // 2, 0
    if kind == "down":
        if Lin % 2:
            raise ValueError("Downsample needs an even length (UNet pads to a multiple of 2^depth)")
        return Lin // 2, 2, 0, 1
    if kind == "up":
        return 2 * Lin, 1, 1, 2
    raise ValueError(kind)


def _vkey(vp, w):
    return (vp[0], tuple(vp[1:])) if vp is not None else ("", (w,))


def conv_forward(x, w, bias, cache: PackCache, kind: str, vp=None, **epi):
    B, Lin, Cin = x.shape
    k = w.shape[2] if w.dim() == 3 else 1
    Lout, stride, pad, mode = _conv_geom(kind, k, Lin)
    tag, vparams = _vkey(vp, w)
    wp = cache.packs(("p", kind, x.dtype, tag), vparams, w, kind, x.dtype)[0]
    return ops.gemm_nt(x, wp, bias, taps=k, lin=Lin, lout=Lout, stride=stride, pad=pad, mode=mode, out_shape=(B, Lout, wp.shape[1]), **epi)


def conv_dgrad(dy, w, cache: PackCache, kind: str, Lin: int, residual=None, vp=None):
    B, Lout, Cout = dy.shape
    k = w.shape[2] if w.dim() == 3 else 1
    tag, vparams = _vkey(vp, w)
    wp = cache.packs(("p", kind, dy.dtype, tag), vparams, w, kind, dy.dtype)[1]
    Cin = wp.shape[1]
    if kind == "same":
        geom = dict(taps=k, stride=1, pad=k - 1 - k // 2, mode=0)
    elif kind == "down":
        geom = dict(taps=4, stride=1, pad=0, mode=3)
    else:
        geom = dict(taps=4, stride=2, pad=1, mode=0)
    return ops.gemm_nt(dy, wp, None, lin=Lout, lout=Lin, residual=residual, out_shape=(B, Lin, Cin), **geom)


def conv_wgrad_bias(dy, x, w, kind: str, bias, need_w: bool, need_b: bool, n: Optional[int] = None):
    if need_w and need_b and bias is not None:
        tgt = grad_target(bias)
        if tgt is not None and tgt.numel() == w.shape[0]:
            dw = conv_wgrad(dy, x, w, kind, bias_out=tgt)
            grad_done(bias)
            return dw, None
    dw = conv_wgrad(dy, x, w, kind) if need_w else None
    db = _bias_grad(dy, bias, n) if (need_b and bias is not None) else None
    return dw, db


def conv_wgrad(dy, x, w, kind: str, direct: bool = True, bias_out: Optional[torch.Tensor] = None):
    B, Lin, Cin = x.shape
    conv = w.dim() == 3
    k = w.shape[2] if conv else 1
    Lout, stride, pad, mode = _conv_geom(kind, k, Lin)
    tgt = grad_target(w) if direct else None
    g = ops.gemm_tn(dy, x, taps=k, lin=Lin, lout=Lout, stride=stride, pad=pad, mode=mode, n1=w.shape[0], out=tgt, conv_layout=conv,
                    accumulate=tgt is not None, bias_out=bias_out)
    if tgt is not None:
        grad_done(w)
        return None
    return g if conv else g[0]


class Adapter:

    def __init__(self, base_weight, lora_a, lora_b, magnitude, scaling: float) -> None:
        self.w, self.a, self.b, self.m, self.scaling = base_weight, lora_a, lora_b, magnitude, float(scaling)
        self._eff = None

    @property
    def params(self) -> Tuple[torch.Tensor, ...]:
        return (self.w, self.a, self.b) + ((self.m,) if self.m is not None else ())

    def effective(self):
        ver = (_WEIGHT_EPOCH, *[(p._version, p.data_ptr()) for p in self.params])
        if self._eff is None or self._eff[0] != ver:
            with torch.no_grad():
                m = self.m.detach().float().reshape(-1).contiguous() if self.m is not None else None
                g, t32, t16 = ops.dora_gain(self.w.detach().float().contiguous(), self.a.detach().float().contiguous(),
                                            self.b.detach().float().contiguous(), m, self.scaling)
                self.sg = g * self.scaling
                self.sgbt = {torch.float32: t32, torch.bfloat16: t16}
            self._eff = (ver, EffWeight(self, g), g)
        return self._eff[1], self._eff[2]


def adapter_grads(ad: Adapter, dy, x, y, bias, kind: str, cache: PackCache, sums=None):
    B_, Lin, I = x.shape
    O = dy.shape[-1]
    r = ad.a.shape[0]
    conv = ad.a.dim() == 3
    k = ad.a.shape[2] if conv else 1
    dt = x.dtype
    _, g = ad.effective()
    Lout, stride, pad, mode = _conv_geom(kind, k, Lin)
    with torch.no_grad():
        pa = cache.packs(("lora_a", id(ad), kind, dt), (ad.a,), ad.a, "same", dt)[0]
        sg, pbt = ad.sg, ad.sgbt[dt]
        u = ops.gemm_nt(x, pa, None, taps=k, lin=Lin, lout=Lout, stride=stride, pad=pad, mode=mode, out_shape=(B_, Lout, r))
        du = ops.gemm_nt(dy, pbt, None, out_shape=(B_, Lout, r))
        tb = ops.gemm_tn(dy, u, n1=O, out=ops.zeros((1, O, r), torch.float32, x.device), accumulate=True)
        s0 = s1 = None
        if ad.m is not None:
            if sums is not None:
                s0, s1 = sums
            else:
                s0 = ops.wcolsum(dy, y, None, B_, Lout).sum(0)
                s1 = ops.colsum(dy, O) if bias is not None else None
        bias32 = bias.detach().float().contiguous() if bias is not None else None
        if kind == "same":
            gt = ops.gemm_tn(x, du, taps=k, lin=Lin, lout=Lout, stride=1, pad=k - 1 - pad, mode=0, n1=I,
                             out=ops.zeros((k, I, r), torch.float32, x.device), accumulate=True)
            tgt = [grad_target(ad.a), grad_target(ad.b)] + ([grad_target(ad.m)] if ad.m is not None else [])
            direct = all(t is not None for t in tgt)
            da = tgt[0] if direct else torch.empty(ad.a.shape, dtype=torch.float32, device=x.device)
            db = tgt[1] if direct else torch.empty(ad.b.shape, dtype=torch.float32, device=x.device)
            dm = None
            if ad.m is not None:
                dm = tgt[2] if direct else torch.empty(ad.m.shape, dtype=torch.float32, device=x.device)
            ops.adapter_finish(tb, sg, db, gt, da, s0, s1, bias32, ad.m.detach().float().contiguous() if ad.m is not None else None, dm,
                               O, I, k, r, accumulate=direct)
            if direct:
                for p_ in (ad.a, ad.b) + ((ad.m,) if ad.m is not None else ()):
                    grad_done(p_)
                return None, None, None
            return da, db, dm
        db = tb[0] * sg[:, None]
        da = ops.gemm_tn(du, x, taps=k, lin=Lin, lout=Lout, stride=stride, pad=pad, mode=mode, n1=r, conv_layout=conv)
        da = da if conv else da[0]
        dm = None
        if ad.m is not None:
            sm = s0 - bias32 * s1 if bias is not None else s0
            dm = (sm / ad.m.detach().float().reshape(-1)).reshape(ad.m.shape)
    return da.reshape(ad.a.shape), db.reshape(ad.b.shape), dm


class ConvFn(torch.autograd.Function):

    @staticmethod
    def forward(ctx, x, w, bias, cache, kind, vp=None):
        ctx.save_for_backward(x, w)
        ctx.cache, ctx.kind, ctx.has_bias, ctx.vp = cache, kind, bias is not None, vp
        ctx.bias_ref = bias
        return conv_forward(x, w, bias, cache, kind, vp)

    @staticmethod
    def backward(ctx, dy):
        with scope({"up": "Upsample (backward)", "down": "Downsample (backward)"}.get(ctx.kind, "Conv (backward)")):
            return ConvFn._backward(ctx, dy)

    @staticmethod
    def _backward(ctx, dy):
        x, w = ctx.saved_tensors
        dy = _rc(dy)
        dx = conv_dgrad(dy, w, ctx.cache, ctx.kind, x.shape[1], vp=ctx.vp) if ctx.needs_input_grad[0] else None
        dw, db = conv_wgrad_bias(dy, x, w, ctx.kind, ctx.bias_ref if ctx.has_bias else None, ctx.needs_input_grad[1], ctx.needs_input_grad[2], w.shape[0])
        return dx, dw, db, None, None, None


class AdaptedConvFn(torch.autograd.Function):

    @staticmethod
    def forward(ctx, x, bias, cache, kind, adapter, la, lb, lm):
        y = conv_forward(x, adapter.effective()[0], bias, cache, kind, ("dora", *adapter.params))
        ctx.save_for_backward(x, y)
        ctx.cache, ctx.kind, ctx.adapter, ctx.bias_ref = cache, kind, adapter, bias
        return y

    @staticmethod
    def backward(ctx, dy):
        x, y = ctx.saved_tensors
        ad, need = ctx.adapter, ctx.needs_input_grad
        dy = _rc(dy)
        dx = conv_dgrad(dy, ad.effective()[0], ctx.cache, ctx.kind, x.shape[1], vp=("dora", *ad.params)) if need[0] else None
        db = _bias_grad(dy, ctx.bias_ref, dy.shape[-1]) if ctx.bias_ref is not None and need[1] else None
        da = dlb = dm = None
        if need[5] or need[6] or need[7]:
            da, dlb, dm = adapter_grads(ad, dy, x, y, ctx.bias_ref, ctx.kind, ctx.cache)
        return dx, db, None, None, None, da, dlb, dm


class SkinnyLinearFn(torch.autograd.Function):

    @staticmethod
    def forward(ctx, x, w, bias, mode_dtype, in_act, out_act):
        x = x.contiguous()
        y = ops.skinny_fwd(x, w, bias, mode_dtype, in_act, out_act)
        ctx.save_for_backward(x, w, y if out_act else x)
        ctx.cfg, ctx.bias_ref = (mode_dtype, in_act, out_act), bias
        return y

    @staticmethod
    def backward(ctx, dy):
        x, w, y = ctx.saved_tensors
        mode_dtype, in_act, out_act = ctx.cfg
        need = ctx.needs_input_grad
        bias = ctx.bias_ref
        dy = dy.contiguous().float()
        dw = db = None
        tw = tb = None
        direct = False
        if need[1]:
            tw = grad_target(w)
            direct = tw is not None
            if not direct:
                dw = tw = torch.empty(w.shape, dtype=torch.float32, device=w.device)
            if bias is not None and need[2]:
                tb = grad_target(bias) if direct else None
                if tb is None:
                    db = tb = torch.zeros(bias.shape, dtype=torch.float32, device=w.device)
        dx = ops.skinny_bwd(dy, y if out_act else None, x, w, mode_dtype, in_act, out_act, need[0], tw, tb, direct)
        if direct:
            grad_done(w)
            if tb is not None and db is None:
                grad_done(bias)
        return dx, dw, db, None, None, None


class LinearGroupFn(torch.autograd.Function):

    @staticmethod
    def forward(ctx, x, mode_dtype, in_act, direct, *wb):
        n = len(wb) // 2
        ws, bs = wb[:n], wb[n:]
        x = x.contiguous()
        ys = ops.skinny_fwd_group(x, ws, bs, mode_dtype, in_act)
        ctx.save_for_backward(x, *ws)
        ctx.cfg, ctx.bs = (mode_dtype, in_act, direct, n), bs
        ctx.set_materialize_grads(False)
        return tuple(ys)

    @staticmethod
    def backward(ctx, *gouts):
        x, *ws = ctx.saved_tensors
        mode_dtype, in_act, direct, n = ctx.cfg
        dys = [g.contiguous().float() if g is not None else None for g in gouts]
        dx = ops.skinny_dx_group(dys, ws, x, mode_dtype, in_act) if ctx.needs_input_grad[0] else None
        dws, dbs = [None] * n, [None] * n
        if not direct:
            for i, (dy, w, b) in enumerate(zip(dys, ws, ctx.bs)):
                if dy is None or not ctx.needs_input_grad[4 + i]:
                    continue
                dws[i] = torch.empty(w.shape, dtype=torch.float32, device=w.device)
                if b is not None and ctx.needs_input_grad[4 + n + i]:
                    dbs[i] = torch.zeros(b.shape, dtype=torch.float32, device=w.device)
                ops.skinny_bwd(dy, None, x, w, mode_dtype, in_act, 0, False, dws[i], dbs[i], False)
        return (dx, None, None, None, *dws, *dbs)


def film_group(x: torch.Tensor, linears, mode_dtype: torch.dtype, in_act: int):
    ws = tuple(l.weight for l in linears)
    bs = tuple(l.bias for l in linears)
    direct = _DIRECT and _GRAD_COMPLETE_CB is not None and torch.is_grad_enabled() and x.requires_grad and \
        all(not w.requires_grad or grad_target(w) is not None for w in ws) and \
        all(b is None or not b.requires_grad or grad_target(b) is not None for b in bs)
    if direct:
        ys = LinearGroupFn.apply(x, mode_dtype, in_act, True, *(w.detach() for w in ws), *(None if b is None else b.detach() for b in bs))
        xs = x.detach()
        return {id(w): (y, (xs, w, b, mode_dtype, in_act) if y.requires_grad and w.requires_grad else None) for w, b, y in zip(ws, bs, ys)}
    ys = LinearGroupFn.apply(x, mode_dtype, in_act, False, *ws, *bs)
    return {id(w): (y, None) for w, y in zip(ws, ys)}


def film_tap(entry):
    y, info = entry
    if info is None:
        return y
    xs, w, b, mode_dtype, in_act = info
    grad_use(w)
    if b is not None and b.requires_grad:
        grad_use(b)
    return _FilmTapFn.apply(y, xs, (w, b), mode_dtype, in_act)


class _FilmTapFn(torch.autograd.Function):

    @staticmethod
    def forward(ctx, y, x, wb, mode_dtype, in_act):
        ctx.refs = (x, wb[0], wb[1], mode_dtype, in_act)
        return y.view_as(y)

    @staticmethod
    def backward(ctx, dy):
        x, w, b, mode_dtype, in_act = ctx.refs
        dy = dy.contiguous().float()
        tb = grad_target(b) if b is not None and b.requires_grad else None
        ops.skinny_bwd(dy, None, x, w.detach(), mode_dtype, in_act, 0, False, grad_target(w), tb, True)
        grad_used(w)
        if tb is not None:
            grad_used(b)
        return dy, None, None, None, None


_UNIT_NORM: Dict[Tuple, Tuple[torch.Tensor, torch.Tensor]] = {}


def _unit_norm(C: int, device):
    key = (C, str(device))
    if key not in _UNIT_NORM:
        _UNIT_NORM[key] = (torch.ones(C, dtype=torch.float32, device=device), torch.zeros(C, dtype=torch.float32, device=device))
    return _UNIT_NORM[key]


class BlockFn(torch.autograd.Function):

    @staticmethod
    def forward(ctx, x, w, bias, gamma, beta, ss, cache, adapter=None, la=None, lb=None, lm=None, reslink=None):
        B, L, _ = x.shape
        C = w.shape[0]
        ctx.identity_norm = gamma is None
        if ctx.identity_norm:
            gamma, beta = _unit_norm(C, x.device)
        repro = ops.reproducible() or ctx.identity_norm
        stats = None if repro else ops.zeros((B, 2), torch.float64, x.device)
        if adapter is not None:
            weff, _ = adapter.effective()
            y = conv_forward(x, weff, bias, cache, "same", ("dora", *adapter.params), stats=stats)
        else:
            y = conv_forward(x, w, bias, cache, "same", None, stats=stats)
        ssc = ss.contiguous() if ss is not None else None
        if ctx.identity_norm:
            mr = torch.tensor([0.0, 1.0], dtype=torch.float32, device=x.device).repeat(B, 1)
            h = ops.gn_apply(y, mr, gamma, beta, ssc, L)
        elif repro:
            h, mr = ops.gn_apply_reproducible(y, gamma, beta, ssc, L)
        else:
            h, mr = ops.gn_apply_from_stats(y, stats, gamma, beta, ssc, L)
        ctx.save_for_backward(x, w, y, mr, gamma, beta, ssc if ssc is not None else mr)
        ctx.cache, ctx.has_ss, ctx.adapter = cache, ss is not None, adapter
        ctx.bias_ref, ctx.reslink = bias, reslink
        return h

    @staticmethod
    def backward(ctx, dh):
        with scope("Residual's Block (backward)"):
            return BlockFn._backward(ctx, dh)

    @staticmethod
    def _backward(ctx, dh):
        x, w, y, mr, gamma, beta, ss = ctx.saved_tensors
        ss = ss if ctx.has_ss else None
        L = x.shape[1]
        need = ctx.needs_input_grad
        tg, tb = (None, None) if ctx.identity_norm else (grad_target(gamma), grad_target(beta))
        direct_norm = tg is not None and tb is not None
        bias = ctx.bias_ref
        ad = ctx.adapter
        db = None
        tbias = dyy = sdy = None
        if need[2] and bias is not None:
            tbias = grad_target(bias)
            if tbias is None:
                db = tbias = torch.zeros(bias.shape, dtype=torch.float32, device=dh.device)
        want_dm = ad is not None and ad.m is not None and need[10]
        if want_dm:
            dyy = ops.zeros((y.shape[-1],), torch.float32, dh.device)
            sdy = tbias if db is not None else ops.zeros((y.shape[-1],), torch.float32, dh.device)
        dy, dgamma, dbeta, dss = ops.gn_bwd(_rc(dh), y, mr, gamma, beta, ss, L, tg if direct_norm else None, tb if direct_norm else None,
                                            sdy if want_dm else tbias, dyy, identity_norm=ctx.identity_norm)
        if tbias is not None and db is None:
            if want_dm:
                tbias.add_(sdy)
            grad_done(bias)
        if direct_norm:
            grad_done(gamma); grad_done(beta)
            dgamma = dbeta = None
        dx = None
        if need[0]:
            extra = None
            if ctx.reslink is not None and ctx.reslink.dx is not None:
                extra, ctx.reslink.dx = ctx.reslink.dx, None
            dx = conv_dgrad(dy, ad.effective()[0], ctx.cache, "same", L, residual=extra, vp=("dora", *ad.params)) if ad is not None \
                else conv_dgrad(dy, w, ctx.cache, "same", L, residual=extra)
        dw = conv_wgrad(dy, x, w, "same") if need[1] else None
        da = dlb = dm = None
        if ad is not None and (need[8] or need[9] or need[10]):
            da, dlb, dm = adapter_grads(ad, dy, x, y, ctx.bias_ref, "same", ctx.cache, sums=(dyy, sdy) if want_dm else None)
        return dx, dw, db, dgamma if need[3] else None, dbeta if need[4] else None, dss, None, None, da, dlb, dm, None


class GateLink:
    __slots__ = ("dout", "gate")

    def __init__(self) -> None:
        self.dout = self.gate = None


class ResLink:
    __slots__ = ("dx",)

    def __init__(self) -> None:
        self.dx = None


class GCAPoolFn(torch.autograd.Function):

    @staticmethod
    def forward(ctx, h, wk, bk, link=None):
        wkv = wk.reshape(-1).contiguous()
        pooled, p = ops.gca_pool(h, wkv, bk.reshape(-1), h.shape[1])
        ctx.save_for_backward(h, wkv, p, pooled)
        ctx.wshape, ctx.link = wk.shape, link
        ctx.wk_ref, ctx.bk_ref = wk, bk
        return pooled

    @staticmethod
    def backward(ctx, dpooled):
        with scope("GlobalContext (backward)"):
            return GCAPoolFn._backward(ctx, dpooled)

    @staticmethod
    def _backward(ctx, dpooled):
        h, wkv, p, pooled = ctx.saved_tensors
        B, L, C = h.shape
        dpooled = dpooled.contiguous().float()
        sdot = ops.rowdot(pooled, dpooled, None, 1, per_sample=True)
        link = ctx.link
        if link is not None and link.dout is not None:
            dout, gate = link.dout, link.gate
            link.dout = link.gate = None
        else:
            dout, gate = h, torch.zeros((B, C), dtype=torch.float32, device=h.device)
        need_w, need_b = ctx.needs_input_grad[1], ctx.needs_input_grad[2]
        dwk = dbk = tw = tb = None
        direct = False
        if need_w or need_b:
            gw, gb = grad_target(ctx.wk_ref), grad_target(ctx.bk_ref)
            direct = gw is not None and gb is not None
            if direct:
                tw, tb = gw.view(-1), gb.view(-1)
            else:
                tw = ops.zeros(C, torch.float32, h.device)
                tb = ops.zeros(1, torch.float32, h.device)
        dh, dlogit = ops.gca_bwd_apply(dout, h, p, gate, dpooled, sdot, wkv, L, tw, tb)
        if direct:
            grad_done(ctx.wk_ref); grad_done(ctx.bk_ref)
        elif tw is not None:
            dwk = tw.reshape(ctx.wshape) if need_w else None
            dbk = tb.reshape(ctx.bk_ref.shape) if need_b else None
        return dh, dwk, dbk, None


class MeanPoolFn(torch.autograd.Function):

    @staticmethod
    def forward(ctx, h, link=None):
        B, L, C = h.shape
        ctx.save_for_backward(h)
        ctx.link = link
        return ops.wcolsum(h, None, None, B, L) * (1.0 / L)

    @staticmethod
    def backward(ctx, dpooled):
        (h,) = ctx.saved_tensors
        B, L, C = h.shape
        dev = h.device
        dpooled = dpooled.contiguous().float()
        link = ctx.link
        if link is not None and link.dout is not None:
            dout, gate = link.dout, link.gate
            link.dout = link.gate = None
        else:
            dout, gate = h, torch.zeros((B, C), dtype=torch.float32, device=dev)
        p = torch.full((B * L,), 1.0 / L, dtype=torch.float32, device=dev)
        dh, _ = ops.gca_bwd_apply(dout, h, p, gate, dpooled, torch.zeros(B, dtype=torch.float32, device=dev),
                                  torch.zeros(C, dtype=torch.float32, device=dev), L)
        return dh, None


def _gate_dh(link, dout, gate, L):
    if link is not None:
        link.dout, link.gate = dout, gate
        return None
    return ops.gate_residual(dout, gate, None, L)


class GateResFn(torch.autograd.Function):

    @staticmethod
    def forward(ctx, h, gate, res, link=None, rlink=None):
        L = h.shape[1]
        gate = gate.contiguous()
        ctx.save_for_backward(h, gate)
        ctx.link, ctx.rlink = link, rlink
        return ops.gate_residual(h, gate, res, L)

    @staticmethod
    def backward(ctx, dout):
        h, gate = ctx.saved_tensors
        B, L, C = h.shape
        dout = _rc(dout)
        dgate = ops.wcolsum(dout, h, None, B, L)
        dres = dout
        if ctx.rlink is not None and ctx.needs_input_grad[2]:
            ctx.rlink.dx, dres = dout, None
        return _gate_dh(ctx.link, dout, gate, L), dgate, dres, None, None


class GateResConvFn(torch.autograd.Function):

    @staticmethod
    def forward(ctx, h, gate, x, w, bias, cache, link=None, rlink=None):
        gate = gate.contiguous()
        ctx.save_for_backward(h, gate, x, w)
        ctx.cache, ctx.bias_ref, ctx.link, ctx.rlink = cache, bias, link, rlink
        return conv_forward(x, w, bias, cache, "same", None, residual=h, rscale=gate)

    @staticmethod
    def backward(ctx, dout):
        h, gate, x, w = ctx.saved_tensors
        B, L, C = h.shape
        dout = _rc(dout)
        dgate = ops.wcolsum(dout, h, None, B, L)
        dh = _gate_dh(ctx.link, dout, gate, L)
        dx = conv_dgrad(dout, w, ctx.cache, "same", L) if ctx.needs_input_grad[2] else None
        if ctx.rlink is not None and dx is not None:
            ctx.rlink.dx, dx = dx, None
        dw, db = conv_wgrad_bias(dout, x, w, "same", ctx.bias_ref, ctx.needs_input_grad[3], ctx.needs_input_grad[4])
        return dh, dgate, dx, dw, db, None, None, None


class FeedForwardFn(torch.autograd.Function):

    @staticmethod
    def forward(ctx, x, w1, b1, w2, b2, cache):
        h, pre = conv_forward(x, w1, b1, cache, "same", None, act=1, want_pre=True)
        wp2 = cache.packs(("p2", x.dtype), (w2,), w2, "same", x.dtype)[0]
        out = ops.gemm_nt(h, wp2, b2, residual=x, out_shape=x.shape)
        ctx.save_for_backward(x, w1, w2, h, pre)
        ctx.cache, ctx.b1, ctx.b2 = cache, b1, b2
        return out

    @staticmethod
    def backward(ctx, dout):
        x, w1, w2, h, pre = ctx.saved_tensors
        dout = _rc(dout)
        cache = ctx.cache
        wd2 = cache.packs(("p2", x.dtype), (w2,), w2, "same", x.dtype)[1]
        dpre = ops.gemm_nt(dout, wd2, None, dact=pre, out_shape=pre.shape)
        need = ctx.needs_input_grad
        dw2, db2 = conv_wgrad_bias(dout, h, w2, "same", ctx.b2, need[3], need[4])
        dw1, db1 = conv_wgrad_bias(dpre, x, w1, "same", ctx.b1, need[1], need[2])
        wd1 = cache.packs(("p", "same", x.dtype, ""), (w1,), w1, "same", x.dtype)[1]
        dx = ops.gemm_nt(dpre, wd1, None, residual=dout, out_shape=x.shape)
        return dx, dw1, db1, dw2, db2, None


_ROPE_TABLES: Dict[Tuple, Tuple[torch.Tensor, torch.Tensor]] = {}


def rope_tables(n: int, dim: int, scale_base: int, device, theta: float = 10000.0):
    key = (n, dim, scale_base, float(theta), str(device))
    hit = _ROPE_TABLES.get(key)
    if hit is None:
        inv_freq = 1.0 / (theta ** (torch.arange(0, dim, 2).float() / dim))
        t = torch.arange(n, dtype=torch.float32)
        t *= scale_base / n
        freqs = torch.einsum("i , j -> i j", t, inv_freq)
        hit = (freqs.cos().contiguous().to(device), freqs.sin().contiguous().to(device))
        _ROPE_TABLES[key] = hit
    return hit


class AttentionFn(torch.autograd.Function):

    @staticmethod
    def forward(ctx, x, nw, nb, wq, wkv, wo, bo, cache, heads, dim_head, scale_base, aq=None, akv=None,
                qa=None, qb=None, qm=None, kva=None, kvb=None, kvm=None, kv_heads=1, base=None, grad_mode=False):
        B, N, C = x.shape
        H, D, G = heads, dim_head, kv_heads
        dt = x.dtype
        xn, mr = ops.ln_fwd(x, nw, nb)
        wqkv = AttentionFn._qkv_packs(cache, dt, wq, wkv, aq, akv, base)[0]
        qkv = ops.gemm_nt(xn, wqkv, None, out_shape=(B, N, (H + 2 * G) * D))
        cos, sin = rope_tables(N, D, scale_base, x.device)
        scale = D ** -0.5
        qs = ops.q_prescale_ok(D, ops.ATTN_BWD_DEFAULT)
        will_bwd = grad_mode and any(ctx.needs_input_grad)
        dq_ws = ops.fused_bwd_workspace(B, N, H, D, dt, x.device) if (G == 1 and will_bwd) else None
        if ops.fwd_rope_ok(qkv, D, G, qs) and (N >= 2048 or not will_bwd):
            qkv_r, o, lse = ops.mqa_fwd_rope(qkv, cos, sin, B, N, H, D, dt, scale, write_q=will_bwd, zero_dq=dq_ws)
        else:
            qkv_r = ops.rope_cast(qkv, cos, sin, N, H + G, H + 2 * G, D, q_mul=scale * ops.LOG2E if qs else 1.0, n_q_heads=H)
            o, lse = ops.mqa_fwd(qkv_r, B, N, H, D, dt, scale, kv_heads=G, qs=qs, zero_dq=dq_ws)
        keep_raw = will_bwd and ((aq is not None and aq.m is not None) or (akv is not None and akv.m is not None))
        ctx.qkv_raw = qkv if keep_raw else None
        del qkv
        ctx.dq_ws = dq_ws
        wpo = cache.packs(("po", dt), (wo,) if base is None else (base[1],), wo, "same", dt)[0]
        out = ops.gemm_nt(o, wpo, bo, residual=xn, out_shape=x.shape)
        ctx.base = base
        ctx.save_for_backward(x, nw, mr, xn, wq, wkv, wo, qkv_r, o, lse)
        ctx.cache, ctx.geom = cache, (H, D, scale_base, scale, G)
        ctx.nb, ctx.bo = nb, bo
        ctx.aq, ctx.akv = aq, akv
        ctx.qs = qs
        return out

    @staticmethod
    def _qkv_packs(cache, dt, wq, wkv, aq, akv, base=None):
        if aq is None and akv is None:
            return cache.packs(("qkv", dt), (wq, wkv) if base is None else (base[0], wkv), (wq, wkv), "same", dt)
        ws = (aq.effective()[0] if aq is not None else wq, akv.effective()[0] if akv is not None else wkv)
        params = (wq, wkv) + (aq.params if aq is not None else ()) + (akv.params if akv is not None else ())
        return cache.packs(("qkv_dora", dt), params, ws, "same", dt)

    @staticmethod
    def backward(ctx, dout):
        with scope("Attention (backward)"):
            return AttentionFn._backward(ctx, dout)

    @staticmethod
    def _backward(ctx, dout):
        x, nw, mr, xn, wq, wkv, wo, qkv_r, o, lse = ctx.saved_tensors
        H, D, scale_base, scale, G = ctx.geom
        cache = ctx.cache
        need = ctx.needs_input_grad
        B, N, C = x.shape
        dt = x.dtype
        dout = _rc(dout)
        dwo, dbo = conv_wgrad_bias(dout, o, wo, "same", ctx.bo, need[5], need[6])
        wdo = cache.packs(("po", dt), (wo,) if ctx.base is None else (ctx.base[1],), wo, "same", dt)[1]
        if ops.FUSE_ROWDOT and G == 1 and D == 64:
            do, delta = ops.gemm_nt_rowdot(dout, wdo, o, N, H)
        else:
            do, delta = ops.gemm_nt(dout, wdo, None, out_shape=o.shape), None
        do16 = ops.cast_rows(do, torch.bfloat16)
        cos, sin = rope_tables(N, D, scale_base, x.device)
        variant = ops.ATTN_BWD_DEFAULT
        if ctx.qs and variant not in ops._FUSED_DQ_MODE:
            variant = ops.ATTN_FUSED
        dqkv = ops.mqa_bwd(qkv_r, o, do16, lse, B, N, H, D, scale, dt, cos, sin, variant=variant, delta=delta,
                           kv_heads=G, qs=ctx.qs, workspace=ctx.dq_ws)
        ctx.dq_ws = None
        dwq = conv_wgrad(dqkv[..., : H * D], xn, wq, "same") if need[3] else None
        dwkv = conv_wgrad(dqkv[..., H * D:], xn, wkv, "same") if need[4] else None
        aq, akv = ctx.aq, ctx.akv
        packs = AttentionFn._qkv_packs(cache, dt, wq, wkv, aq, akv, ctx.base)
        gq = gkv = (None, None, None)
        if (aq is not None and any(need[13:16])) or (akv is not None and any(need[16:19])):
            qkv = ctx.qkv_raw
            if qkv is None:
                qkv = ops.gemm_nt(xn, packs[0], None, out_shape=(B, N, (H + 2 * G) * D))
            ctx.qkv_raw = None
            if aq is not None:
                gq = adapter_grads(aq, dqkv[..., : H * D], xn, qkv[..., : H * D], None, "same", cache)
            if akv is not None:
                gkv = adapter_grads(akv, dqkv[..., H * D:], xn, qkv[..., H * D:], None, "same", cache)
            del qkv
        dxn = ops.gemm_nt(dqkv, packs[1], None, residual=dout, out_shape=x.shape)
        tg, tb = grad_target(nw), grad_target(ctx.nb)
        direct_norm = tg is not None and tb is not None
        dx, dnw, dnb = ops.ln_bwd(dxn, x, mr, nw, tg if direct_norm else None, tb if direct_norm else None)
        if direct_norm:
            grad_done(nw); grad_done(ctx.nb)
            dnw = dnb = None
        return (dx, dnw if need[1] else None, dnb if need[2] else None, dwq, dwkv, dwo, dbo, None, None, None, None, None, None,
                *gq, *gkv, None, None, None)


class RowsFromNCLFn(torch.autograd.Function):

    @staticmethod
    def forward(ctx, x, dtype, width, kt):
        ctx.shape, ctx.kt = x.shape, kt
        return ops.ncl_to_rows(x.contiguous().float(), dtype, width, kt)

    @staticmethod
    def backward(ctx, d):
        if ctx.kt != 1:
            raise NotImplementedError("gradient w.r.t. the raw x input of the im2col stem is not provided")
        return ops.rows_to_ncl(_rc(d), ctx.shape[1]), None, None, None


class NCLFromRowsFn(torch.autograd.Function):

    @staticmethod
    def forward(ctx, rows, C):
        ctx.meta = (rows.dtype, rows.shape[2])
        return ops.rows_to_ncl(rows, C)

    @staticmethod
    def backward(ctx, d):
        dtype, width = ctx.meta
        return ops.ncl_to_rows(d.contiguous().float(), dtype, width, 1), None
```

### osufusion_amd/ops.py

```python
from __future__ import annotations

from typing import Optional, Tuple

import os

import numpy as np
import torch

from . import _lib

F32, BF16 = 0, 1
_DT = {torch.float32: F32, torch.bfloat16: BF16}


def _stream() -> int:
    return torch.cuda.current_stream().cuda_stream


def _p(t: Optional[torch.Tensor]) -> Optional[int]:
    return None if t is None else t.data_ptr()


def _rows(t: torch.Tensor) -> Tuple[int, int, int]:
    assert t.is_cuda, "osufusion_amd kernels run on the GPU only (no CPU fallback)"
    assert t.stride(-1) == 1, "last dim must be contiguous"
    cols = t.shape[-1]
    if t.dim() == 2:
        return t.shape[0], cols, t.stride(0)
    assert t.dim() == 3
    B, Lr = t.shape[0], t.shape[1]
    ld = t.stride(1)
    assert t.stride(0) == Lr * ld or B == 1, "batch dim must be densely stacked rows"
    return B * Lr, cols, ld


def dt_of(t: torch.Tensor) -> int:
    return _DT[t.dtype]


F32X3 = 2
F32_MATMUL = "exact"


def set_f32_matmul(mode: str) -> str:
    global F32_MATMUL
    assert mode in ("exact", "x3")
    prev, F32_MATMUL = F32_MATMUL, mode
    return prev


def gemm_dt(t: torch.Tensor) -> int:
    return F32X3 if (t.dtype == torch.float32 and F32_MATMUL == "x3") else _DT[t.dtype]


class LaunchSize(int):
    def __new__(cls, n, b=0):
        x = int.__new__(cls, n)
        x.b = b
        return x


class KernelTimer:

    def __init__(self, names) -> None:
        self.names = set(names)
        self.records = {n: [] for n in names}

    def summary(self):
        torch.cuda.synchronize()
        out = {}
        for n, recs in self.records.items():
            if recs:
                out[n] = dict(launches=len(recs), total_ms=sum(s.elapsed_time(e) for s, e, _ in recs), sizes=[m for _, _, m in recs])
        return out


_TIMER: Optional[KernelTimer] = None

_REPRODUCIBLE = False


def reproducible() -> bool:
    return _REPRODUCIBLE


class reproducible_mode:
    def __init__(self, flag: bool = True) -> None:
        self.flag = bool(flag)

    def __enter__(self):
        global _REPRODUCIBLE
        self.prev, _REPRODUCIBLE = _REPRODUCIBLE, self.flag
        return self

    def __exit__(self, *exc):
        global _REPRODUCIBLE
        _REPRODUCIBLE = self.prev
        return False


_ONE_LAUNCH_ATTENTION = False


def one_launch_attention_on() -> bool:
    return _ONE_LAUNCH_ATTENTION


class one_launch_attention:
    def __init__(self, flag: bool = True) -> None:
        self.flag = bool(flag)

    def __enter__(self):
        global _ONE_LAUNCH_ATTENTION
        self.prev, _ONE_LAUNCH_ATTENTION = _ONE_LAUNCH_ATTENTION, self.flag
        return self

    def __exit__(self, *exc):
        global _ONE_LAUNCH_ATTENTION
        _ONE_LAUNCH_ATTENTION = self.prev
        return False


def set_kernel_timer(t: Optional[KernelTimer]) -> None:
    global _TIMER
    _TIMER = t


class ZeroArena:

    ALIGN = 256

    def __init__(self, device, nbytes: int = 192 << 20) -> None:
        self.buf = torch.zeros(nbytes, dtype=torch.uint8, device=device)
        self.off = 0
        self.dirty = 0
        self.misses = 0

    def begin(self) -> None:
        if self.dirty:
            self.buf[: self.dirty].zero_()
        self.off = self.dirty = 0

    def take(self, shape, dtype: torch.dtype) -> Optional[torch.Tensor]:
        n = 1
        for d in (shape if isinstance(shape, (tuple, list)) else (shape,)):
            n *= int(d)
        nbytes = n * torch.empty(0, dtype=dtype).element_size()
        end = self.off + (nbytes + self.ALIGN - 1) // self.ALIGN * self.ALIGN
        if end > self.buf.numel():
            self.misses += 1
            return None
        t = self.buf[self.off: self.off + nbytes].view(dtype).view(shape)
        self.off = self.dirty = end
        return t


_ARENA: Optional[ZeroArena] = None


def set_zero_arena(arena: Optional[ZeroArena]) -> None:
    global _ARENA
    _ARENA = arena


def zeros(shape, dtype: torch.dtype, device) -> torch.Tensor:
    if _ARENA is not None and _ARENA.buf.device == torch.device(device):
        t = _ARENA.take(shape, dtype)
        if t is not None:
            return t
    return torch.zeros(shape, dtype=dtype, device=device)


_TIMED_AS = {"osuf_mqa_fwd_qs": "osuf_mqa_fwd", "osuf_mqa_fwd_zdq": "osuf_mqa_fwd", "osuf_mqa_fwd_rope": "osuf_mqa_fwd", "osuf_mqa_bwd_fused_qs": "osuf_mqa_bwd_fused"}


def call(name: str, *args, meta=None) -> None:
    lib = _lib.load()
    tname = _TIMED_AS.get(name, name)
    if _TIMER is not None and tname in _TIMER.names:
        s, e = torch.cuda.Event(enable_timing=True), torch.cuda.Event(enable_timing=True)
        s.record()
        _lib.check(getattr(lib, name)(*args), name)
        e.record()
        _TIMER.records[tname].append((s, e, meta))
        return
    _lib.check(getattr(lib, name)(*args), name)


def gemm_nt(a: torch.Tensor, w: torch.Tensor, bias: Optional[torch.Tensor] = None, *, taps: int = 1, n_out: Optional[int] = None,
            lin: Optional[int] = None, lout: Optional[int] = None, stride: int = 1, pad: int = 0, mode: int = 0, act: int = 0,
            residual: Optional[torch.Tensor] = None, rscale: Optional[torch.Tensor] = None, dact: Optional[torch.Tensor] = None,
            stats: Optional[torch.Tensor] = None, want_pre: bool = False, out: Optional[torch.Tensor] = None,
            out_shape: Optional[Tuple[int, ...]] = None):
    Min, K, lda = _rows(a)
    assert w.dtype == a.dtype and w.is_contiguous()
    w3 = w if w.dim() == 3 else w.unsqueeze(0)
    assert w3.shape[0] == taps and w3.shape[2] == K, (tuple(w3.shape), taps, K)
    N = w3.shape[1] if n_out is None else n_out
    if lin is None:
        lin = lout = Min
    nb = Min // lin
    M = nb * lout
    if out is None:
        shape = out_shape if out_shape is not None else (M, N)
        out = torch.empty(shape, dtype=a.dtype, device=a.device)
    Mo, No, ldc = _rows(out)
    assert Mo == M and No >= N
    pre = torch.empty_like(out) if want_pre else None
    ldc2 = _rows(pre)[2] if want_pre else 0
    ldr = _rows(residual)[2] if residual is not None else 0
    ldu = _rows(dact)[2] if dact is not None else 0
    if bias is not None:
        assert bias.dtype == torch.float32 and bias.numel() >= N
    call("osuf_gemm_nt", gemm_dt(a), _p(a), lda, _p(w3), K, N * K if taps > 1 else 0, _p(out), ldc, _p(pre), ldc2, _p(residual), ldr,
         _p(dact), ldu, _p(bias), _p(rscale), _p(stats), M, N, K, taps, lin, lout, stride, pad, mode, act, _stream())
    return (out, pre) if want_pre else out


def gemm_nt_rowdot(a: torch.Tensor, w: torch.Tensor, o: torch.Tensor, L: int, heads: int):
    M, K, lda = _rows(a)
    w3 = w if w.dim() == 3 else w.unsqueeze(0)
    assert w3.dtype == a.dtype and w3.is_contiguous() and w3.shape[0] == 1 and w3.shape[2] == K and w3.shape[1] == heads * 64
    Mo, No, ldo = _rows(o)
    assert Mo == M and No == heads * 64 and o.dtype == a.dtype and M % L == 0
    out = torch.empty(o.shape, dtype=a.dtype, device=a.device)
    delta = torch.empty((M // L, heads, L), dtype=torch.float32, device=a.device)
    call("osuf_gemm_nt_rowdot", gemm_dt(a), _p(a), lda, _p(w3), K, _p(out), heads * 64, _p(o), ldo, _p(delta), M, heads * 64, K, L, heads, _stream())
    return out, delta


def gemm_tn(dy: torch.Tensor, x: torch.Tensor, *, taps: int = 1, lin: Optional[int] = None, lout: Optional[int] = None, stride: int = 1,
            pad: int = 0, mode: int = 0, n1: Optional[int] = None, out: Optional[torch.Tensor] = None, conv_layout: bool = False,
            accumulate: bool = False, bias_out: Optional[torch.Tensor] = None) -> torch.Tensor:
    M, N1, ldy = _rows(dy)
    Mx, N2, ldx = _rows(x)
    if n1 is not None:
        N1 = n1
    if lin is None:
        lin = lout = M
    assert dy.dtype == x.dtype and Mx // lin == M // lout
    shape = (N1, N2, taps) if conv_layout else (taps, N1, N2)
    if out is None:
        assert not accumulate
        out = torch.empty(shape, dtype=torch.float32, device=dy.device)
    assert out.dtype == torch.float32 and out.is_contiguous() and out.numel() == taps * N1 * N2
    need = _lib.load().osuf_gemm_tn_workspace_bytes(gemm_dt(dy), M, N1, N2, taps)
    ws = _workspace(need, dy.device) if need > 0 else None
    args = (gemm_dt(dy), _p(dy), ldy, _p(x), ldx, _p(out), N2, N1 * N2, M, N1, N2, taps, lin, lout, stride, pad, mode, 0,
            1 if conv_layout else 0, 1 if accumulate else 0, _p(ws), need if ws is not None else 0)
    if bias_out is not None:
        assert bias_out.dtype == torch.float32 and bias_out.is_contiguous() and bias_out.numel() == N1
        call("osuf_gemm_tn_bias", *args, _p(bias_out), _stream())
    else:
        call("osuf_gemm_tn", *args, _stream())
    return out


_WS = {}


def _workspace(nbytes: int, device) -> torch.Tensor:
    key = str(device)
    cur = _WS.get(key)
    if cur is None or cur.numel() * 4 < nbytes:
        cur = torch.empty(max(nbytes // 4, 1 << 24) * 5 // 4, dtype=torch.float32, device=device)
        _WS[key] = cur
    return cur


def colsum(y: torch.Tensor, n: Optional[int] = None, out: Optional[torch.Tensor] = None) -> torch.Tensor:
    M, N, ld = _rows(y)
    N = N if n is None else n
    if out is None:
        out = zeros(N, torch.float32, y.device)
    call("osuf_colsum", dt_of(y), _p(y), ld, M, N, _p(out), _stream())
    return out


def gn_finalize(stats: torch.Tensor, count: int) -> torch.Tensor:
    B = stats.shape[0]
    mr = torch.empty((B, 2), dtype=torch.float32, device=stats.device)
    call("osuf_gn_finalize", _p(stats), _p(mr), B, count, _stream())
    return mr


def _gn_stats_parts_len(M: int, C: int, L: int) -> int:
    return max(_lib.load().osuf_gn_stats_workspace_bytes(M, C, L) // 8, 1)


def gn_stats(y: torch.Tensor, L: int) -> torch.Tensor:
    M, C, ld = _rows(y)
    B = M // L
    part = torch.empty(_gn_stats_parts_len(M, C, L), dtype=torch.float64, device=y.device)
    mr = torch.empty((B, 2), dtype=torch.float32, device=y.device)
    call("osuf_gn_stats", dt_of(y), _p(y), ld, _p(part), _p(mr), M, C, L, _stream())
    return mr


def gn_apply_reproducible(y: torch.Tensor, gamma: torch.Tensor, beta: torch.Tensor, ss: Optional[torch.Tensor], L: int):
    M, C, ld = _rows(y)
    B = M // L
    part = torch.empty(_gn_stats_parts_len(M, C, L), dtype=torch.float64, device=y.device)
    h = torch.empty(y.shape, dtype=y.dtype, device=y.device)
    mr = torch.empty((B, 2), dtype=torch.float32, device=y.device)
    call("osuf_gn_stats_parts", dt_of(y), _p(y), ld, _p(part), M, C, L, _stream())
    call("osuf_gn_apply_fwd_parts", dt_of(y), _p(y), ld, _p(h), C, _p(part), _p(mr), _p(gamma), _p(beta), _p(ss), M, C, L, _stream())
    return h, mr


def gn_apply_from_stats(y: torch.Tensor, stats: torch.Tensor, gamma: torch.Tensor, beta: torch.Tensor, ss: Optional[torch.Tensor], L: int):
    M, C, ld = _rows(y)
    h = torch.empty(y.shape, dtype=y.dtype, device=y.device)
    mr = torch.empty((M // L, 2), dtype=torch.float32, device=y.device)
    call("osuf_gn_apply_fwd_stats", dt_of(y), _p(y), ld, _p(h), C, _p(stats), L * C, _p(mr), _p(gamma), _p(beta), _p(ss), M, C, L, _stream())
    return h, mr


def gn_apply(y: torch.Tensor, mr: torch.Tensor, gamma: torch.Tensor, beta: torch.Tensor, ss: Optional[torch.Tensor], L: int) -> torch.Tensor:
    M, C, ld = _rows(y)
    h = torch.empty(y.shape, dtype=y.dtype, device=y.device)
    call("osuf_gn_apply_fwd", dt_of(y), _p(y), ld, _p(h), C, _p(mr), _p(gamma), _p(beta), _p(ss), M, C, L, _stream())
    return h


def gn_bwd(dh: torch.Tensor, y: torch.Tensor, mr: torch.Tensor, gamma: torch.Tensor, beta: torch.Tensor, ss: Optional[torch.Tensor], L: int,
           dgamma_out: Optional[torch.Tensor] = None, dbeta_out: Optional[torch.Tensor] = None, dbias_out: Optional[torch.Tensor] = None,
           dyy_out: Optional[torch.Tensor] = None, identity_norm: bool = False):
    M, C, ldy = _rows(y)
    B = M // L
    dev = y.device
    dy = torch.empty(y.shape, dtype=y.dtype, device=dev)
    T12 = zeros((B, 4, C), torch.float32, dev)
    S = torch.empty((B, 2), dtype=torch.float32, device=dev)
    dss = torch.empty((B, 2 * C), dtype=torch.float32, device=dev) if ss is not None else None
    if identity_norm:
        dgamma_out = dbeta_out = None
    elif dgamma_out is None or dbeta_out is None:
        dgb = zeros((2, C), torch.float32, dev)
        dgamma_out, dbeta_out = dgb[0], dgb[1]
    call("osuf_gn_bwd", dt_of(y), _p(dh), _rows(dh)[2], _p(y), ldy, _p(dy), C, _p(mr), _p(gamma), _p(beta), _p(ss), _p(T12), _p(S),
         _p(dss), _p(dgamma_out), _p(dbeta_out), _p(dbias_out), _p(dyy_out), M, C, L, _stream())
    return dy, dgamma_out, dbeta_out, dss


def ln_fwd(x: torch.Tensor, gamma: torch.Tensor, beta: torch.Tensor):
    M, C, ld = _rows(x)
    out = torch.empty(x.shape, dtype=x.dtype, device=x.device)
    mr = torch.empty((M, 2), dtype=torch.float32, device=x.device)
    call("osuf_ln_fwd", dt_of(x), _p(x), ld, _p(out), C, _p(mr), _p(gamma), _p(beta), M, C, _stream())
    return out, mr


def ln_bwd(dy: torch.Tensor, x: torch.Tensor, mr: torch.Tensor, gamma: torch.Tensor, dgamma_out: Optional[torch.Tensor] = None,
           dbeta_out: Optional[torch.Tensor] = None):
    M, C, ld = _rows(x)
    dx = torch.empty(x.shape, dtype=x.dtype, device=x.device)
    if dgamma_out is None or dbeta_out is None:
        dgb = torch.zeros((2, C), dtype=torch.float32, device=x.device)
        dgamma_out, dbeta_out = dgb[0], dgb[1]
    call("osuf_ln_bwd", dt_of(x), _p(dy), _rows(dy)[2], _p(x), ld, _p(dx), C, _p(mr), _p(gamma), _p(dgamma_out), _p(dbeta_out), M, C, _stream())
    return dx, dgamma_out, dbeta_out


def rowdot(h: torch.Tensor, w: torch.Tensor, bias: Optional[torch.Tensor], L: int, per_sample: bool = False) -> torch.Tensor:
    M, C, ld = _rows(h)
    out = torch.empty(M, dtype=torch.float32, device=h.device)
    call("osuf_rowdot", dt_of(h), _p(h), ld, _p(w), C if per_sample else 0, _p(bias), _p(out), M, C, L, _stream())
    return out


def gca_pool(h: torch.Tensor, wk: torch.Tensor, bk: Optional[torch.Tensor], L: int):
    M, C, ld = _rows(h)
    B = M // L
    need = _lib.load().osuf_gca_pool_workspace_bytes(M, C, L)
    part = torch.empty(max(need // 4, 1), dtype=torch.float32, device=h.device)
    p = torch.empty(M, dtype=torch.float32, device=h.device)
    pooled = torch.empty((B, C), dtype=torch.float32, device=h.device)
    call("osuf_gca_pool", dt_of(h), _p(h), ld, _p(wk), _p(bk), _p(part), _p(p), _p(pooled), M, C, L, _stream())
    return pooled, p


def softmax_rows_(p: torch.Tensor, B: int, L: int) -> torch.Tensor:
    call("osuf_softmax_rows", _p(p), B, L, _stream())
    return p


def wcolsum(a: torch.Tensor, bmul: Optional[torch.Tensor], w: Optional[torch.Tensor], B: int, L: int) -> torch.Tensor:
    M, C, ld = _rows(a)
    part = None
    if _REPRODUCIBLE:
        out = torch.empty((B, C), dtype=torch.float32, device=a.device)
        part = torch.empty((B, (L + 63) // 64, C), dtype=torch.float32, device=a.device)
    else:
        out = zeros((B, C), torch.float32, a.device)
    call("osuf_wcolsum", dt_of(a), _p(a), ld, _p(bmul), _rows(bmul)[2] if bmul is not None else 0, _p(w), _p(out), B, C, L, _p(part), _stream())
    return out


def gate_residual(h: torch.Tensor, gate: torch.Tensor, res: Optional[torch.Tensor], L: int) -> torch.Tensor:
    M, C, ld = _rows(h)
    out = torch.empty(h.shape, dtype=h.dtype, device=h.device)
    call("osuf_gate_residual", dt_of(h), _p(h), ld, _p(gate), _p(res), _rows(res)[2] if res is not None else 0, _p(out), C, M, C, L, _stream())
    return out


def gca_bwd_apply(dout, h, p, gate, dpooled, sdot, wk, L: int, dwk_out: Optional[torch.Tensor] = None,
                  dbk_out: Optional[torch.Tensor] = None):
    M, C, ld = _rows(h)
    dh = torch.empty(h.shape, dtype=h.dtype, device=h.device)
    dlogit = torch.empty(M, dtype=torch.float32, device=h.device)
    ws, need = None, 0
    if dwk_out is not None:
        need = _lib.load().osuf_gca_bwd_apply_workspace_bytes(M, C)
        ws = torch.empty(need // 4, dtype=torch.float32, device=h.device)
    call("osuf_gca_bwd_apply", dt_of(h), _p(dout), _rows(dout)[2], _p(h), ld, _p(dh), C, _p(p), _p(gate), _p(dpooled), _p(sdot), _p(wk),
         _p(dlogit), M, C, L, _p(dwk_out), _p(dbk_out), _p(ws), need, _stream())
    return dh, dlogit


LOG2E = 1.4426950408889634


def q_prescale_ok(head_dim: int, variant: int) -> bool:
    return head_dim == 64 and variant in _FUSED_DQ_MODE


def rope_cast(qkv: torch.Tensor, cos: torch.Tensor, sin: torch.Tensor, N: int, n_rot: int, n_heads: int, head_dim: int,
              q_mul: float = 1.0, n_q_heads: int = 0) -> torch.Tensor:
    M, W, ld = _rows(qkv)
    out = torch.empty(qkv.shape, dtype=torch.bfloat16, device=qkv.device)
    if q_mul != 1.0:
        call("osuf_rope_cast_qs", dt_of(qkv), _p(qkv), ld, _p(out), W, _p(cos), _p(sin), M, N, n_rot, n_heads, head_dim, q_mul, n_q_heads, _stream())
    else:
        call("osuf_rope_cast", dt_of(qkv), _p(qkv), ld, _p(out), W, _p(cos), _p(sin), M, N, n_rot, n_heads, head_dim, _stream())
    return out


def rope_bwd(dqkv32: torch.Tensor, out_dtype: torch.dtype, cos, sin, N: int, n_rot: int, n_heads: int, head_dim: int) -> torch.Tensor:
    M, W, ld = _rows(dqkv32)
    out = torch.empty(dqkv32.shape, dtype=out_dtype, device=dqkv32.device)
    call("osuf_rope_bwd", _DT[out_dtype], _p(dqkv32), ld, _p(out), W, _p(cos), _p(sin), M, N, n_rot, n_heads, head_dim, _stream())
    return out


DQ_PREZEROED = 0x100


def fused_bwd_workspace(B: int, N: int, H: int, D: int, out_dtype: torch.dtype, device, variant: Optional[int] = None, qsplit: int = 0):
    variant = ATTN_BWD_DEFAULT if variant is None else variant
    if D != 64 or variant not in _FUSED_DQ_MODE or variant == ATTN_FUSED_SLABS or os.environ.get("OSUF_ATTN_NO_ZDQ") == "1":
        return None
    need = _lib.load().osuf_mqa_bwd_fused_workspace_bytes(B, H, N, _DT[out_dtype], qsplit, _FUSED_DQ_MODE[variant])
    if need <= 0:
        return None
    ws = torch.empty((need + 3) // 4, dtype=torch.float32, device=device)
    ws.fused_variant = variant
    return ws


def mqa_fwd(qkv: torch.Tensor, B: int, N: int, H: int, D: int, out_dtype: torch.dtype, scale: float, kv_heads: int = 1, qs: bool = False,
            zero_dq: Optional[torch.Tensor] = None):
    M, W, ld = _rows(qkv)
    G = kv_heads
    assert qkv.dtype == torch.bfloat16 and W == (H + 2 * G) * D and H % G == 0
    assert zero_dq is None or (G == 1 and D == 64 and zero_dq.dtype == torch.float32 and zero_dq.numel() >= B * N * H * D)
    r = H // G
    o = torch.empty((B, N, H * D), dtype=out_dtype, device=qkv.device)
    lse = torch.empty((B, H, N) if G == 1 else (G, B, r, N), dtype=torch.float32, device=qkv.device)
    base, eo = qkv.data_ptr(), o.element_size()
    if zero_dq is not None:
        call("osuf_mqa_fwd_zdq", base, ld, base + 2 * H * D, ld, base + 2 * (H + 1) * D, ld, o.data_ptr(), H * D, _DT[out_dtype], lse.data_ptr(), B, H, N, D, scale,
             1 if qs else 0, zero_dq.data_ptr(), _stream(), meta=LaunchSize(N, B))
        return o, lse
    for g in range(G):
        call("osuf_mqa_fwd_qs" if qs else "osuf_mqa_fwd", base + 2 * g * r * D, ld, base + 2 * (H + g) * D, ld, base + 2 * (H + G + g) * D, ld, o.data_ptr() + eo * g * r * D,
             H * D, _DT[out_dtype], lse.data_ptr() + 4 * g * B * r * N, B, r, N, D, scale, _stream(), meta=LaunchSize(N, B))
    return o, lse


def gqa_fwd(qkv: torch.Tensor, B: int, N: int, H: int, D: int, out_dtype: torch.dtype, scale: float, kv_heads: int = 1):
    from . import gqa
    return gqa.gqa_fwd(qkv, B, N, H, D, out_dtype, scale, kv_heads)


def fwd_rope_ok(qkv: torch.Tensor, head_dim: int, kv_heads: int, qs: bool) -> bool:
    return qs and head_dim == 64 and kv_heads == 1 and qkv.dtype == torch.bfloat16 and os.environ.get("OSUF_ATTN_NO_FWD_ROPE") != "1"


def mqa_fwd_rope(qkv: torch.Tensor, cos: torch.Tensor, sin: torch.Tensor, B: int, N: int, H: int, D: int, out_dtype: torch.dtype, scale: float,
                 write_q: bool = True, zero_dq: Optional[torch.Tensor] = None):
    M, W, ld = _rows(qkv)
    assert qkv.dtype == torch.bfloat16 and D == 64 and W == (H + 2) * D
    qkv_r = torch.empty(qkv.shape, dtype=torch.bfloat16, device=qkv.device)
    kv_in, kv_out = qkv.data_ptr() + 2 * H * D, qkv_r.data_ptr() + 2 * H * D
    call("osuf_rope_cast", _DT[torch.bfloat16], kv_in, ld, kv_out, W, _p(cos), _p(sin), M, N, 1, 2, D, _stream())
    o = torch.empty((B, N, H * D), dtype=out_dtype, device=qkv.device)
    lse = torch.empty((B, H, N), dtype=torch.float32, device=qkv.device)
    assert zero_dq is None or (zero_dq.dtype == torch.float32 and zero_dq.numel() >= B * N * H * D)
    call("osuf_mqa_fwd_rope", qkv.data_ptr(), ld, kv_out, W, kv_out + 2 * D, W, o.data_ptr(), H * D, _DT[out_dtype], lse.data_ptr(), B, H, N, D, scale,
         _p(cos), _p(sin), scale * LOG2E, qkv_r.data_ptr() if write_q else None, W, _p(zero_dq), _stream(), meta=LaunchSize(N, B))
    return qkv_r, o, lse


ATTN_AUTO, ATTN_PLAIN, ATTN_PIPE, ATTN_FUSED, ATTN_FUSED_SLABS = 0, 1, 2, 3, 4
ATTN_FUSED256, ATTN_FUSED512 = 5, 6
ATTN_FUSED512A = 8
_FUSED_DQ_MODE = {ATTN_FUSED: 0, ATTN_FUSED_SLABS: 1, ATTN_FUSED256: 2, ATTN_FUSED512: 3, ATTN_FUSED512A: 5}
ATTN_BWD_DEFAULT = ATTN_FUSED
FUSE_ROWDOT = True


def mqa_bwd(qkv: torch.Tensor, o: torch.Tensor, do: torch.Tensor, lse: torch.Tensor, B: int, N: int, H: int, D: int, scale: float,
            out_dtype: torch.dtype = torch.float32, cos: Optional[torch.Tensor] = None, sin: Optional[torch.Tensor] = None,
            variant: int = ATTN_AUTO, qsplit: int = 0, delta: Optional[torch.Tensor] = None, kv_heads: int = 1, qs: bool = False,
            workspace: Optional[torch.Tensor] = None) -> torch.Tensor:
    M, W, ld = _rows(qkv)
    G = kv_heads
    r = H // G
    assert do.dtype == torch.bfloat16 and W == (H + 2 * G) * D and (G == 1 or delta is None)
    if D != 64:
        if cos is not None:
            raw = mqa_bwd(qkv, o, do, lse, B, N, H, D, scale, torch.float32, None, None, ATTN_AUTO, 0, delta, kv_heads)
            return rope_bwd(raw, out_dtype, cos, sin, N, H + G, H + 2 * G, D)
        variant, qsplit = ATTN_AUTO, 0
    dqkv = torch.empty((B, N, W), dtype=out_dtype, device=qkv.device)
    es, ldo_, ldo2 = dqkv.element_size(), _rows(do)[2], _rows(o)[2]
    if delta is None:
        delta = torch.empty((B, H, N) if G == 1 else (G, B, r, N), dtype=torch.float32, device=qkv.device)
        for g in range(G):
            call("osuf_attn_delta", do.data_ptr() + 2 * g * r * D, ldo_, o.data_ptr() + o.element_size() * g * r * D, ldo2, _DT[o.dtype],
                 delta.data_ptr() + 4 * g * B * r * N, B, r, N, D, _stream())
    for g in range(G):
        q_, k_, v_ = qkv.data_ptr() + 2 * g * r * D, qkv.data_ptr() + 2 * (H + g) * D, qkv.data_ptr() + 2 * (H + G + g) * D
        dq_, dk_, dv_ = dqkv.data_ptr() + es * g * r * D, dqkv.data_ptr() + es * (H + g) * D, dqkv.data_ptr() + es * (H + G + g) * D
        do_, lse_, delta_ = do.data_ptr() + 2 * g * r * D, lse.data_ptr() + 4 * g * B * r * N, delta.data_ptr() + 4 * g * B * r * N
        if variant in _FUSED_DQ_MODE:
            mode = _FUSED_DQ_MODE[variant]
            need = _lib.load().osuf_mqa_bwd_fused_workspace_bytes(B, r, N, _DT[out_dtype], qsplit, mode)
            if workspace is not None and G == 1 and getattr(workspace, "fused_variant", None) == variant and workspace.numel() * 4 >= need:
                ws, mode = workspace, mode | DQ_PREZEROED
            else:
                ws = _workspace(need, qkv.device)
            call("osuf_mqa_bwd_fused_qs" if qs else "osuf_mqa_bwd_fused", q_, ld, k_, ld, v_, ld, do_, ldo_, lse_, delta_, dq_, W, dk_, dv_, W, B, r, N, D, scale, _DT[out_dtype],
                 _p(cos), _p(sin), _p(ws), need, qsplit, mode, _stream(), meta=N)
            continue
        assert not qs, "pre-scaled queries: only the fused sweeps have that form"
        call("osuf_mqa_bwd_dq", q_, ld, k_, ld, v_, ld, do_, ldo_, lse_, delta_, dq_, W, B, r, N, D, scale, _DT[out_dtype],
             _p(cos), _p(sin), variant, _stream(), meta=N)
        need = _lib.load().osuf_mqa_bwd_dkv_workspace_bytes(B, N, qsplit)
        ws = _workspace(need, qkv.device) if need > 0 else None
        call("osuf_mqa_bwd_dkv", q_, ld, k_, ld, v_, ld, do_, ldo_, lse_, delta_, dk_, dv_, W,
             B, r, N, D, scale, _DT[out_dtype], _p(cos), _p(sin), _p(ws), need if ws is not None else 0, qsplit, variant, _stream(), meta=N)
    return dqkv


def ncl_to_rows(x: torch.Tensor, dtype: torch.dtype, width: int, kt: int = 1) -> torch.Tensor:
    assert x.dtype == torch.float32 and x.is_contiguous() and x.is_cuda
    B, C, Lx = x.shape
    out = torch.empty((B, Lx, width), dtype=dtype, device=x.device)
    call("osuf_ncl_to_rows", _DT[dtype], _p(x), _p(out), width, width, B, C, Lx, kt, _stream())
    return out


def rows_to_ncl(rows: torch.Tensor, C: int) -> torch.Tensor:
# ... 315 lines not shown
```

Baseline: 5.677 steps/s.

## Stack Q and KV weight-gradient GEMMs into one split-output TN GEMM

Adds a split-output TN GEMM that computes the weight gradients for the Q and KV projections in a single pass over the stacked dqkv tensor, writing rows before n1_cut into one gradient buffer and the rest into another. This removes one GEMM launch and one re-read of the normalized activations per attention backward. It also adds queue infrastructure so that split-K reduction passes from several weight-gradient GEMMs can be batched into one grouped reduce kernel. In the shown code the queue is never used by callers. The trade-off is extra indexing complexity in the reduce kernels and a fallback path when the shape constraints fail.

```diff
diff --git a/include/osufusion_hip.h b/include/osufusion_hip.h
--- a/include/osufusion_hip.h
+++ b/include/osufusion_hip.h
@@ -38,6 +38,33 @@
 int osuf_gemm_tn_bias(int dtype, const void* dY, long ldy, const void* X, long ldx, float* dW, long ldw, long tapstride,
                       int M, int N1, int N2, int taps, int Lin, int Lout, int stride, int pad, int mode,
                       int splits, int out_layout, int accumulate, float* workspace, long workspace_bytes, float* dbias, hipStream_t stream);
+
+#ifndef OSUF_WGRAD_QUEUE_DEFINED
+#define OSUF_WGRAD_QUEUE_DEFINED
+#define OSUF_WGRAD_QUEUE_MAX 16
+typedef struct osuf_wgrad_desc {
+  const void* ws;
+  float* dW;
+  int N1, N2, taps, splits;
+  int row0, rows;
+  int kind, accumulate;
+  int wg0, wgs;
+  int reserved0, reserved1;
+} osuf_wgrad_desc;
+typedef struct osuf_wgrad_queue {
+  int n, total_wgs;
+  long reserved;
+  osuf_wgrad_desc d[OSUF_WGRAD_QUEUE_MAX];
+} osuf_wgrad_queue;
+#endif
+int osuf_gemm_tn_split(int dtype, const void* dY, long ldy, const void* X, long ldx,
+                       float* dW0, long ldw0, long tapstride0, int out_layout0, int accumulate0,
+                       float* dW1, long ldw1, long tapstride1, int out_layout1, int accumulate1, int n1_cut,
+                       int M, int N1, int N2, int taps, int Lin, int Lout, int stride, int pad, int mode,
+                       float* workspace, long workspace_bytes, float* dbias, osuf_wgrad_queue* queue, hipStream_t stream);
+int osuf_wgrad_queue_push(osuf_wgrad_queue* queue, const void* ws, int pk, int N1, int N2, int taps, int splits,
+                          float* dW0, int out_layout0, int accumulate0, float* dW1, int out_layout1, int accumulate1, int n1_cut);
+int osuf_wgrad_reduce_flush(osuf_wgrad_queue* queue, hipStream_t stream);
 
 int osuf_colsum(int dtype, const void* Y, long ldy, int M, int N, float* out, hipStream_t stream);
 
diff --git a/osufusion_amd/_lib.py b/osufusion_amd/_lib.py
--- a/osufusion_amd/_lib.py
+++ b/osufusion_amd/_lib.py
@@ -17,6 +17,9 @@
     "osuf_gemm_tn": [I, P, L, P, L, P, L, L, I, I, I, I, I, I, I, I, I, I, I, I, P, L, P],
     "osuf_gemm_tn_bias": [I, P, L, P, L, P, L, L, I, I, I, I, I, I, I, I, I, I, I, I, P, L, P, P],
     "osuf_gemm_tn_workspace_bytes": [I, I, I, I, I],
+    "osuf_gemm_tn_split": [I, P, L, P, L, P, L, L, I, I, P, L, L, I, I, I, I, I, I, I, I, I, I, I, I, P, L, P, P, P],
+    "osuf_wgrad_queue_push": [P, P, I, I, I, I, I, P, I, I, P, I, I, I],
+    "osuf_wgrad_reduce_flush": [P, P],
     "osuf_colsum": [I, P, L, I, I, P, P],
     "osuf_gn_finalize": [P, P, I, L, P],
     "osuf_gn_apply_fwd": [I, P, L, P, L, P, P, P, P, I, I, I, P],
diff --git a/osufusion_amd/csrc/common.hpp b/osufusion_amd/csrc/common.hpp
--- a/osufusion_amd/csrc/common.hpp
+++ b/osufusion_amd/csrc/common.hpp
@@ -26,6 +26,25 @@
 } osuf_linear_desc;
 #endif
 static_assert(sizeof(osuf_linear_desc) == 56, "osuf_linear_desc is part of the C ABI");
+#ifndef OSUF_WGRAD_QUEUE_DEFINED
+#define OSUF_WGRAD_QUEUE_DEFINED
+#define OSUF_WGRAD_QUEUE_MAX 16
+typedef struct osuf_wgrad_desc {
+  const void* ws;
+  float* dW;
+  int N1, N2, taps, splits;
+  int row0, rows;
+  int kind, accumulate;
+  int wg0, wgs;
+  int reserved0, reserved1;
+} osuf_wgrad_desc;
+typedef struct osuf_wgrad_queue {
+  int n, total_wgs;
+  long reserved;
+  osuf_wgrad_desc d[OSUF_WGRAD_QUEUE_MAX];
+} osuf_wgrad_queue;
+#endif
+static_assert(sizeof(osuf_wgrad_desc) == 64 && sizeof(osuf_wgrad_queue) == 16 + 64 * OSUF_WGRAD_QUEUE_MAX, "osuf_wgrad_queue is part of the C ABI");
 
 #define OSUF_DT_F32 0
 #define OSUF_DT_BF16 1
diff --git a/osufusion_amd/csrc/gemm.hip b/osufusion_amd/csrc/gemm.hip
--- a/osufusion_amd/csrc/gemm.hip
+++ b/osufusion_amd/csrc/gemm.hip
@@ -1977,17 +1977,21 @@
 }
 
 template <int LAYOUT>
-__global__ __launch_bounds__(256) void wgrad_reduce_kernel(const float* ws, float* dW, long n12, int taps, int splits, int accumulate) {
+__device__ __forceinline__ void wgrad_reduce_rows(const float* ws, float* dW, int N1, int N2, int row0, int rows, int taps, int splits,
+                                                  int accumulate, long bid, long nb) {
+  const long n12 = (long)N1 * N2, n = n12 * taps, d12 = (long)rows * N2;
+  ws += (long)row0 * N2;
   if constexpr (LAYOUT == 0) {
-    const long n = n12 * taps, n4 = n >> 2;
-    for (long i = (long)blockIdx.x * blockDim.x + threadIdx.x; i < n4; i += (long)gridDim.x * blockDim.x) {
-      f32x4 a = sum_partials(ws + 4 * i, n, splits);
+    const long n4 = (d12 * taps) >> 2;
+    for (long i = bid * blockDim.x + threadIdx.x; i < n4; i += nb * blockDim.x) {
+      const long t = (4 * i) / d12, r = 4 * i - t * d12;
+      f32x4 a = sum_partials(ws + t * n12 + r, n, splits);
       if (accumulate) a += reinterpret_cast<f32x4*>(dW)[i];
       reinterpret_cast<f32x4*>(dW)[i] = a;
     }
   } else {
-    const long n = n12 * taps, q12 = n12 >> 2;
-    for (long q = (long)blockIdx.x * blockDim.x + threadIdx.x; q < q12; q += (long)gridDim.x * blockDim.x) {
+    const long q12 = d12 >> 2;
+    for (long q = bid * blockDim.x + threadIdx.x; q < q12; q += nb * blockDim.x) {
       if (taps == 3) {
         f32x4 a[3];
 #pragma unroll
@@ -2011,38 +2015,46 @@
 }
 
 template <int LAYOUT>
-__global__ __launch_bounds__(256) void wgrad_reduce4_kernel(const float* ws, float* dW, long n12, int taps, int splits, int accumulate) {
-  __shared__ f32x4 red[3][3][64];
+__global__ __launch_bounds__(256) void wgrad_reduce_kernel(const float* ws, float* dW, int N1, int N2, int taps, int splits, int accumulate) {
+  wgrad_reduce_rows<LAYOUT>(ws, dW, N1, N2, 0, N1, taps, splits, accumulate, blockIdx.x, gridDim.x);
+}
+
+template <int LAYOUT>
+__device__ __forceinline__ void wgrad_reduce4_rows(const float* ws, float* dW, int N1, int N2, int row0, int rows, int taps, int splits,
+                                                   int accumulate, long bid, f32x4* red) {
   const int tq = threadIdx.x & 63, ts = threadIdx.x >> 6;
-  const long n = n12 * taps;
+  const long n12 = (long)N1 * N2, n = n12 * taps, d12 = (long)rows * N2;
   const int mine = (splits - ts + 3) >> 2;
+  ws += (long)row0 * N2;
+  auto slot = [&](int lane, int t) -> f32x4& { return red[(lane * 3 + t) * 64 + tq]; };
   if constexpr (LAYOUT == 0) {
-    const long n4 = n >> 2;
-    const long i = (long)blockIdx.x * 64 + tq;
+    const long n4 = (d12 * taps) >> 2;
+    const long i = bid * 64 + tq;
     const long ic = min(i, n4 - 1);
-    f32x4 a = sum_partials(ws + (long)ts * n + 4 * ic, 4 * n, mine);
-    if (ts) red[ts - 1][0][tq] = a;
+    const long t = (4 * ic) / d12, r = 4 * ic - t * d12;
+    f32x4 a = sum_partials(ws + (long)ts * n + t * n12 + r, 4 * n, mine);
+    if (ts) slot(ts - 1, 0) = a;
     __syncthreads();
     if (ts == 0 && i < n4) {
-      a = ((a + red[0][0][tq]) + red[1][0][tq]) + red[2][0][tq];
+      a = ((a + slot(0, 0)) + slot(1, 0)) + slot(2, 0);
       if (accumulate) a += reinterpret_cast<f32x4*>(dW)[i];
       reinterpret_cast<f32x4*>(dW)[i] = a;
     }
   } else {
-    const long q12 = n12 >> 2;
-    const long q = (long)blockIdx.x * 64 + tq;
+    const long q12 = d12 >> 2;
+    const long q = bid * 64 + tq;
     const long qc = min(q, q12 - 1);
     f32x4 a[3];
 #pragma unroll
     for (int t = 0; t < 3; ++t) a[t] = sum_partials(ws + (long)ts * n + (long)t * n12 + 4 * qc, 4 * n, mine);
     if (ts) {
 #pragma unroll
-      for (int t = 0; t < 3; ++t) red[ts - 1][t][tq] = a[t];
+      for (int t = 0; t < 3; ++t) slot(ts - 1, t) = a[t];
     }
     __syncthreads();
     if (ts == 0 && q < q12) {
 #pragma unroll
-      for (int t = 0; t < 3; ++t) a[t] = ((a[t] + red[0][t][tq]) + red[1][t][tq]) + red[2][t][tq];
+      for (int t = 0; t < 3; ++t) a[t] = ((a[t] + slot(0, t)) + slot(1, t)) + slot(2, t);
       f32x4* dst = reinterpret_cast<f32x4*>(dW + 12 * q);
       f32x4 o0 = {a[0][0], a[1][0], a[2][0], a[0][1]}, o1 = {a[1][1], a[2][1], a[0][2], a[1][2]}, o2 = {a[2][2], a[0][3], a[1][3], a[2][3]};
       if (accumulate) { o0 += dst[0]; o1 += dst[1]; o2 += dst[2]; }
@@ -2051,17 +2063,24 @@
   }
 }
 
+template <int LAYOUT>
+__global__ __launch_bounds__(256) void wgrad_reduce4_kernel(const float* ws, float* dW, int N1, int N2, int taps, int splits, int accumulate) {
+  __shared__ f32x4 red[3 * 3 * 64];
+  wgrad_reduce4_rows<LAYOUT>(ws, dW, N1, N2, 0, N1, taps, splits, accumulate, blockIdx.x, red);
+}
+
 template <int LAYOUT, int NT>
-__global__ __launch_bounds__(256) void wgrad_reduce_pk_kernel(const uint32_t* ws, float* dW, int N1, int N2, int taps, int splits, int accumulate) {
-  __shared__ f32x4 red[3][2 * NT][64];
+__device__ __forceinline__ void wgrad_reduce_pk_rows(const uint32_t* ws, float* dW, int N1, int N2, int row0, int rows, int taps, int splits,
+                                                     int accumulate, long bid, f32x4* red) {
   const int tq = threadIdx.x & 63, ts = threadIdx.x >> 6;
-  const long quads = N2 >> 2, per_tap = (long)(N1 >> 1) * quads, groups = NT == 3 ? per_tap : per_tap * taps;
-  const long gi = (long)blockIdx.x * 64 + tq, gc = min(gi, groups - 1);
+  const long quads = N2 >> 2, per_tap = (long)(rows >> 1) * quads, groups = NT == 3 ? per_tap : per_tap * taps;
+  const long gi = bid * 64 + tq, gc = min(gi, groups - 1);
   const int t0 = NT == 3 ? 0 : (int)(gc / per_tap);
   const long rem = gc - (long)t0 * per_tap;
   const long p = rem / quads, q = rem - p * quads;
   const long tile = (long)(N1 >> 1) * N2, stride = tile * taps;
-  const uint32_t* src = ws + (long)t0 * tile + p * N2 + 4 * q;
+  const uint32_t* src = ws + (long)t0 * tile + ((long)(row0 >> 1) + p) * N2 + 4 * q;
+  auto slot = [&](int lane, int k) -> f32x4& { return red[(lane * 2 * NT + k) * 64 + tq]; };
   f32x4 ev[NT], od[NT];
 #pragma unroll
   for (int t = 0; t < NT; ++t) { ev[t] = f32x4{0.f, 0.f, 0.f, 0.f}; od[t] = ev[t]; }
@@ -2079,14 +2098,14 @@
   }
   if (ts) {
 #pragma unroll
-    for (int t = 0; t < NT; ++t) { red[ts - 1][2 * t][tq] = ev[t]; red[ts - 1][2 * t + 1][tq] = od[t]; }
+    for (int t = 0; t < NT; ++t) { slot(ts - 1, 2 * t) = ev[t]; slot(ts - 1, 2 * t + 1) = od[t]; }
   }
   __syncthreads();
   if (ts == 0 && gi < groups) {
 #pragma unroll
     for (int t = 0; t < NT; ++t) {
-      ev[t] = ((ev[t] + red[0][2 * t][tq]) + red[1][2 * t][tq]) + red[2][2 * t][tq];
-      od[t] = ((od[t] + red[0][2 * t + 1][tq]) + red[1][2 * t + 1][tq]) + red[2][2 * t + 1][tq];
+      ev[t] = ((ev[t] + slot(0, 2 * t)) + slot(1, 2 * t)) + slot(2, 2 * t);
+      od[t] = ((od[t] + slot(0, 2 * t + 1)) + slot(1, 2 * t + 1)) + slot(2, 2 * t + 1);
     }
 #pragma unroll
     for (int h = 0; h < 2; ++h) {
@@ -2099,7 +2118,7 @@
         dst[0] = o0; dst[1] = o1; dst[2] = o2;
       } else if constexpr (LAYOUT == 0) {
         const f32x4 v = h ? od[0] : ev[0];
-        f32x4* dst = reinterpret_cast<f32x4*>(dW + ((long)t0 * N1 + n1) * N2 + 4 * q);
+        f32x4* dst = reinterpret_cast<f32x4*>(dW + ((long)t0 * rows + n1) * N2 + 4 * q);
         *dst = accumulate ? *dst + v : v;
       } else {
         const f32x4 v = h ? od[0] : ev[0];
@@ -2113,26 +2132,113 @@
   }
 }
 
-static void launch_wgrad_reduce(const WgradArgs& gb, float* dW, int N1, int N2, int taps, int sp, int out_layout, int accumulate, bool many_splits_ok,
-                                hipStream_t stream) {
-  const long n12 = (long)N1 * N2, n = n12 * taps;
-  if (gb.ws_pk) {
-    const uint32_t* w = reinterpret_cast<const uint32_t*>(gb.ws);
-    const long per_tap = (long)(N1 >> 1) * (N2 >> 2);
-    if (out_layout == 1 && taps == 3) hipLaunchKernelGGL((wgrad_reduce_pk_kernel<1, 3>), dim3((int)((per_tap + 63) / 64)), dim3(256), 0, stream, w, dW, N1, N2, taps, sp, accumulate);
-    else if (out_layout == 1) hipLaunchKernelGGL((wgrad_reduce_pk_kernel<1, 1>), dim3((int)((per_tap * taps + 63) / 64)), dim3(256), 0, stream, w, dW, N1, N2, taps, sp, accumulate);
-    else hipLaunchKernelGGL((wgrad_reduce_pk_kernel<0, 1>), dim3((int)((per_tap * taps + 63) / 64)), dim3(256), 0, stream, w, dW, N1, N2, taps, sp, accumulate);
-    return;
-  }
-  const long groups = out_layout == 1 ? n12 / 4 : n / 4;
+template <int LAYOUT, int NT>
+__global__ __launch_bounds__(256) void wgrad_reduce_pk_kernel(const uint32_t* ws, float* dW, int N1, int N2, int taps, int splits, int accumulate) {
+  __shared__ f32x4 red[3 * 2 * NT * 64];
+  wgrad_reduce_pk_rows<LAYOUT, NT>(ws, dW, N1, N2, 0, N1, taps, splits, accumulate, blockIdx.x, red);
+}
+
+enum { kRedPk01 = 0, kRedPk11 = 1, kRedPk13 = 2, kRedF32L0 = 3, kRedF32L1 = 4, kRedF32x4L0 = 5, kRedF32x4L1 = 6 };
+
+static int wgrad_reduce_kind(bool pk, int N1, int N2, int taps, int sp, int out_layout) {
+  if (pk) return out_layout == 1 ? (taps == 3 ? kRedPk13 : kRedPk11) : kRedPk01;
+  const long n12 = (long)N1 * N2, groups = out_layout == 1 ? n12 / 4 : n12 * taps / 4;
   long blocks = (groups + 255) / 256;
   if (blocks > 2048) blocks = 2048;
-  if (sp >= 8 && blocks < 512 && many_splits_ok) {
-    const long b4 = (groups + 63) / 64;
-    if (out_layout == 1) hipLaunchKernelGGL(wgrad_reduce4_kernel<1>, dim3((int)b4), dim3(256), 0, stream, gb.ws, dW, n12, taps, sp, accumulate);
-    else hipLaunchKernelGGL(wgrad_reduce4_kernel<0>, dim3((int)b4), dim3(256), 0, stream, gb.ws, dW, n12, taps, sp, accumulate);
-  } else if (out_layout == 1) hipLaunchKernelGGL(wgrad_reduce_kernel<1>, dim3((int)blocks), dim3(256), 0, stream, gb.ws, dW, n12, taps, sp, accumulate);
-  else hipLaunchKernelGGL(wgrad_reduce_kernel<0>, dim3((int)blocks), dim3(256), 0, stream, gb.ws, dW, n12, taps, sp, accumulate);
+  const bool four = sp >= 8 && blocks < 512 && (out_layout == 0 || taps == 3);
+  return out_layout == 1 ? (four ? kRedF32x4L1 : kRedF32L1) : (four ? kRedF32x4L0 : kRedF32L0);
+}
+
+static int wgrad_reduce_wgs(int kind, int rows, int N2, int taps) {
+  const long d12 = (long)rows * N2;
+  switch (kind) {
+    case kRedPk13: return (int)(((d12 >> 3) + 63) / 64);
+    case kRedPk01: case kRedPk11: return (int)(((d12 >> 3) * taps + 63) / 64);
+    case kRedF32x4L0: return (int)((d12 * taps / 4 + 63) / 64);
+    case kRedF32x4L1: return (int)((d12 / 4 + 63) / 64);
+    default: {
+      const long groups = kind == kRedF32L1 ? d12 / 4 : d12 * taps / 4;
+      const long blocks = (groups + 255) / 256;
+      return (int)(blocks > 2048 ? 2048 : blocks);
+    }
+  }
+}
+
+__global__ __launch_bounds__(256) void wgrad_reduce_group_kernel(osuf_wgrad_queue tb) {
+  __shared__ f32x4 red[3 * 6 * 64];
+  int j = 0;
+  while (j + 1 < tb.n && tb.d[j + 1].wg0 <= (int)blockIdx.x) ++j;
+  const osuf_wgrad_desc d = tb.d[j];
+  const long bid = (int)blockIdx.x - d.wg0;
+  const float* wf = reinterpret_cast<const float*>(d.ws);
+  const uint32_t* wp = reinterpret_cast<const uint32_t*>(d.ws);
+  switch (d.kind) {
+    case kRedPk01: wgrad_reduce_pk_rows<0, 1>(wp, d.dW, d.N1, d.N2, d.row0, d.rows, d.taps, d.splits, d.accumulate, bid, red); break;
+    case kRedPk11: wgrad_reduce_pk_rows<1, 1>(wp, d.dW, d.N1, d.N2, d.row0, d.rows, d.taps, d.splits, d.accumulate, bid, red); break;
+    case kRedPk13: wgrad_reduce_pk_rows<1, 3>(wp, d.dW, d.N1, d.N2, d.row0, d.rows, d.taps, d.splits, d.accumulate, bid, red); break;
+    case kRedF32L0: wgrad_reduce_rows<0>(wf, d.dW, d.N1, d.N2, d.row0, d.rows, d.taps, d.splits, d.accumulate, bid, d.wgs); break;
+    case kRedF32L1: wgrad_reduce_rows<1>(wf, d.dW, d.N1, d.N2, d.row0, d.rows, d.taps, d.splits, d.accumulate, bid, d.wgs); break;
+    case kRedF32x4L0: wgrad_reduce4_rows<0>(wf, d.dW, d.N1, d.N2, d.row0, d.rows, d.taps, d.splits, d.accumulate, bid, red); break;
+    case kRedF32x4L1: wgrad_reduce4_rows<1>(wf, d.dW, d.N1, d.N2, d.row0, d.rows, d.taps, d.splits, d.accumulate, bid, red); break;
+    default: break;
+  }
+}
+
+static void launch_wgrad_reduce(const void* ws, bool pk, float* dW, int N1, int N2, int taps, int sp, int out_layout, int accumulate, hipStream_t stream) {
+  const int kind = wgrad_reduce_kind(pk, N1, N2, taps, sp, out_layout);
+  const dim3 grid(wgrad_reduce_wgs(kind, N1, N2, taps)), block(256);
+  const uint32_t* wp = reinterpret_cast<const uint32_t*>(ws);
+  const float* wf = reinterpret_cast<const float*>(ws);
+  switch (kind) {
+    case kRedPk13: hipLaunchKernelGGL((wgrad_reduce_pk_kernel<1, 3>), grid, block, 0, stream, wp, dW, N1, N2, taps, sp, accumulate); break;
+    case kRedPk11: hipLaunchKernelGGL((wgrad_reduce_pk_kernel<1, 1>), grid, block, 0, stream, wp, dW, N1, N2, taps, sp, accumulate); break;
+    case kRedPk01: hipLaunchKernelGGL((wgrad_reduce_pk_kernel<0, 1>), grid, block, 0, stream, wp, dW, N1, N2, taps, sp, accumulate); break;
+    case kRedF32x4L1: hipLaunchKernelGGL(wgrad_reduce4_kernel<1>, grid, block, 0, stream, wf, dW, N1, N2, taps, sp, accumulate); break;
+    case kRedF32x4L0: hipLaunchKernelGGL(wgrad_reduce4_kernel<0>, grid, block, 0, stream, wf, dW, N1, N2, taps, sp, accumulate); break;
+    case kRedF32L1: hipLaunchKernelGGL(wgrad_reduce_kernel<1>, grid, block, 0, stream, wf, dW, N1, N2, taps, sp, accumulate); break;
+    default: hipLaunchKernelGGL(wgrad_reduce_kernel<0>, grid, block, 0, stream, wf, dW, N1, N2, taps, sp, accumulate); break;
+  }
+}
+
+static int wgrad_queue_add(osuf_wgrad_queue* q, const void* ws, bool pk, int N1, int N2, int taps, int sp, float* dW, int out_layout, int accumulate,
+                           int row0, int rows) {
+  if (q->n < 0 || q->n >= OSUF_WGRAD_QUEUE_MAX || rows <= 0 || row0 < 0 || row0 + rows > N1 || (out_layout != 0 && out_layout != 1)) return OSUF_EINVAL;
+  if (pk && ((row0 | rows | N1) & 1)) return OSUF_EINVAL;
+  if (N2 % 4 || !al16(ws) || !al16(dW) || sp <= 0 || taps <= 0) return OSUF_EINVAL;
+  osuf_wgrad_desc& d = q->d[q->n];
+  d = osuf_wgrad_desc{};
+  d.ws = ws; d.dW = dW; d.N1 = N1; d.N2 = N2; d.taps = taps; d.splits = sp; d.row0 = row0; d.rows = rows;
+  d.kind = wgrad_reduce_kind(pk, N1, N2, taps, sp, out_layout);
+  d.accumulate = accumulate ? 1 : 0;
+  d.wg0 = q->n ? q->d[q->n - 1].wg0 + q->d[q->n - 1].wgs : 0;
+  d.wgs = wgrad_reduce_wgs(d.kind, rows, N2, taps);
+  q->n += 1;
+  q->total_wgs = d.wg0 + d.wgs;
+  return OSUF_OK;
+}
+
+extern "C" int osuf_wgrad_queue_push(osuf_wgrad_queue* queue, const void* ws, int pk, int N1, int N2, int taps, int splits,
+                                     float* dW0, int out_layout0, int accumulate0, float* dW1, int out_layout1, int accumulate1, int n1_cut) {
+  if (!queue || !ws || !dW0 || N1 <= 0 || N2 <= 0) return OSUF_EINVAL;
+  if (!dW1) return wgrad_queue_add(queue, ws, pk != 0, N1, N2, taps, splits, dW0, out_layout0, accumulate0, 0, N1);
+  if (n1_cut <= 0 || n1_cut >= N1 || (n1_cut & 1) || queue->n + 2 > OSUF_WGRAD_QUEUE_MAX) return OSUF_EINVAL;
+  if (int rc = wgrad_queue_add(queue, ws, pk != 0, N1, N2, taps, splits, dW0, out_layout0, accumulate0, 0, n1_cut)) return rc;
+  return wgrad_queue_add(queue, ws, pk != 0, N1, N2, taps, splits, dW1, out_layout1, accumulate1, n1_cut, N1 - n1_cut);
+}
+
+extern "C" int osuf_wgrad_reduce_flush(osuf_wgrad_queue* queue, hipStream_t stream) {
+  if (!queue || queue->n < 0 || queue->n > OSUF_WGRAD_QUEUE_MAX) return OSUF_EINVAL;
+  if (queue->n == 0) return OSUF_OK;
+  int wg = 0;
+  for (int j = 0; j < queue->n; ++j) {
+    if (queue->d[j].wg0 != wg || queue->d[j].wgs <= 0 || queue->d[j].kind < kRedPk01 || queue->d[j].kind > kRedF32x4L1) return OSUF_EINVAL;
+    wg += queue->d[j].wgs;
+  }
+  if (wg != queue->total_wgs) return OSUF_EINVAL;
+  hipLaunchKernelGGL(wgrad_reduce_group_kernel, dim3(wg), dim3(256), 0, stream, *queue);
+  queue->n = 0;
+  queue->total_wgs = 0;
+  return osuf_launch_status();
 }
 
 template <typename T>
@@ -2305,9 +2411,17 @@
   return osuf_launch_status();
 }
 
+struct TnSplit {
+  float* dW;
+  long ldw, tapstride;
+  int out_layout, accumulate, n1_cut;
+};
+static constexpr int kTnNoPartials = -1000;
+
 static int gemm_tn_launch(int dtype, const void* dY, long ldy, const void* X, long ldx, float* dW, long ldw, long tapstride,
                           int M, int N1, int N2, int taps, int Lin, int Lout, int stride, int pad, int mode,
-                          int splits, int out_layout, int accumulate, float* workspace, long workspace_bytes, float* dbias, hipStream_t stream) {
+                          int splits, int out_layout, int accumulate, float* workspace, long workspace_bytes, float* dbias, hipStream_t stream,
+                          const TnSplit* split = nullptr, osuf_wgrad_queue* queue = nullptr) {
   long es = 1;
   if (out_layout == 1) { ldw = (long)N2 * taps; tapstride = 1; es = taps; }
   else if (out_layout != 0) return OSUF_EINVAL;
@@ -2316,6 +2430,9 @@
   if (M <= 0 || N1 <= 0 || N2 <= 0 || taps <= 0 || Lout <= 0 || Lin <= 0 || M % Lout) return OSUF_EINVAL;
   if (N1 % epc || N2 % epc || ldy % epc || ldx % epc) return OSUF_EINVAL;
   if (!aligned16(dY) || !aligned16(X)) return OSUF_EINVAL;
+  if (split && (split->n1_cut <= 0 || split->n1_cut >= N1 || split->n1_cut % epc || (N1 - split->n1_cut) % epc ||
+                (split->out_layout != 0 && split->out_layout != 1))) return OSUF_EINVAL;
+  if (queue && (queue->n < 0 || queue->n + (split ? 2 : 1) > OSUF_WGRAD_QUEUE_MAX)) return OSUF_EINVAL;
   auto bias_by_colsum = [&]() -> int {
     return dbias ? osuf_colsum(dtype == OSUF_DT_BF16 ? OSUF_DT_BF16 : OSUF_DT_F32, dY, ldy, M, N1, dbias, stream) : OSUF_OK;
   };
@@ -2328,17 +2445,34 @@
   };
   auto plan_partials = [&](WgradArgs& gb, int sp) -> int {
     const long n = (long)taps * N1 * N2;
-    const bool dense = (out_layout == 1 && ((long)N1 * N2) % 4 == 0) ||
-                       (out_layout == 0 && ldw == N2 && (taps == 1 || tapstride == (long)N1 * N2) && n % 4 == 0 && aligned16(dW));
+    auto dense_dst = [&](const float* w, int layout, long ld, long ts, int rows) {
+      return (layout == 1 && ((long)rows * N2) % 4 == 0) ||
+             (layout == 0 && ld == N2 && (taps == 1 || ts == (long)rows * N2) && ((long)taps * rows * N2) % 4 == 0 && aligned16(w));
+    };
+    const bool dense = !split ? dense_dst(dW, out_layout, ldw, tapstride, N1)
+                              : dense_dst(dW, out_layout, ldw, tapstride, split->n1_cut) && aligned16(dW) &&
+                                dense_dst(split->dW, split->out_layout, split->ldw, split->tapstride, N1 - split->n1_cut) && aligned16(split->dW);
     gb.ws = (workspace && dense && aligned16(workspace) && workspace_bytes >= (long)sp * n * (long)sizeof(float)) ? workspace : nullptr;
+    if (split && !gb.ws) return kTnNoPartials;
     gb.ws_pk = gb.ws && wgrad_pk(dtype, N1, N2);
     gb.dbias = dtype == OSUF_DT_BF16 ? dbias : nullptr;
     if (dtype != OSUF_DT_BF16) { if (int rc = bias_by_colsum()) return rc; }
     if (!gb.ws && !accumulate) (void)hipMemsetAsync(dW, 0, (size_t)n * sizeof(float), stream);
     return OSUF_OK;
   };
+  auto reduce_partials = [&](const WgradArgs& gb, int sp) -> int {
+    if (!split && !queue) { launch_wgrad_reduce(gb.ws, gb.ws_pk, dW, N1, N2, taps, sp, out_layout, accumulate, stream); return OSUF_OK; }
+    osuf_wgrad_queue own{};
+    osuf_wgrad_queue* q = queue ? queue : &own;
+    const int rows0 = split ? split->n1_cut : N1;
+    if (int rc = wgrad_queue_add(q, gb.ws, gb.ws_pk, N1, N2, taps, sp, dW, out_layout, accumulate, 0, rows0)) return rc;
+    if (split)
+      if (int rc = wgrad_queue_add(q, gb.ws, gb.ws_pk, N1, N2, taps, sp, split->dW, split->out_layout, split->accumulate, rows0, N1 - rows0)) return rc;
+    return queue ? OSUF_OK : osuf_wgrad_reduce_flush(&own, stream);
+  };
   const int bkm = dtype == OSUF_DT_BF16 ? 64 : 32;
   if (splits <= 0 && dtype == OSUF_DT_BF16 && N2 <= 32 && M >= 4096) {
+    if (split) return kTnNoPartials;
     const int tiles_n1 = (N1 + kBig - 1) / kBig;
     int sp = 512 / (tiles_n1 * taps);
     if (sp < 1) sp = 1;
@@ -2373,7 +2507,8 @@
     const dim3 grid_t3(((sp * btiles + 7) / 8) * 8);
     if (dtype == OSUF_DT_F32X3) hipLaunchKernelGGL(gemm_tn_taps3_x3_kernel, grid_t3, dim3(512), lds_t3, stream, gb);
     else hipLaunchKernelGGL(gemm_tn_taps3_kernel, grid_t3, dim3(512), lds_t3, stream, gb);
-    if (gb.ws) launch_wgrad_reduce(gb, dW, N1, N2, taps, sp, out_layout, accumulate, true, stream);
+    if (gb.ws)
+      if (int rc = reduce_partials(gb, sp)) return rc;
     return osuf_launch_status();
   }
   {
@@ -2387,10 +2522,12 @@
       allow_lds<gemm_tn_big_x3_kernel>(lds_big);
       if (dtype == OSUF_DT_F32X3) hipLaunchKernelGGL(gemm_tn_big_x3_kernel, dim3(((sp * btiles + 7) / 8) * 8 * taps), dim3(512), lds_big, stream, gb);
       else hipLaunchKernelGGL(gemm_tn_big_kernel, dim3(((sp * btiles + 7) / 8) * 8 * taps), dim3(512), lds_big, stream, gb);
-      if (gb.ws) launch_wgrad_reduce(gb, dW, N1, N2, taps, sp, out_layout, accumulate, out_layout == 0 || taps == 3, stream);
+      if (gb.ws)
+        if (int rc = reduce_partials(gb, sp)) return rc;
       return osuf_launch_status();
     }
   }
+  if (split) return kTnNoPartials;
   const int tiles = ((N1 + kTile - 1) / kTile) * ((N2 + kTile - 1) / kTile);
   if (splits <= 0) {
     splits = (768 + tiles * taps - 1) / (tiles * taps);
@@ -2430,3 +2567,23 @@
   return gemm_tn_launch(dtype, dY, ldy, X, ldx, dW, ldw, tapstride, M, N1, N2, taps, Lin, Lout, stride, pad, mode, splits, out_layout, accumulate,
                         workspace, workspace_bytes, dbias, stream);
 }
+
+extern "C" int osuf_gemm_tn_split(int dtype, const void* dY, long ldy, const void* X, long ldx,
+                                  float* dW0, long ldw0, long tapstride0, int out_layout0, int accumulate0,
+                                  float* dW1, long ldw1, long tapstride1, int out_layout1, int accumulate1, int n1_cut,
+                                  int M, int N1, int N2, int taps, int Lin, int Lout, int stride, int pad, int mode,
+                                  float* workspace, long workspace_bytes, float* dbias, osuf_wgrad_queue* queue, hipStream_t stream) {
+  if (!dW0) return OSUF_EINVAL;
+  if (!dW1)
+    return gemm_tn_launch(dtype, dY, ldy, X, ldx, dW0, ldw0, tapstride0, M, N1, N2, taps, Lin, Lout, stride, pad, mode, 0, out_layout0, accumulate0,
+                          workspace, workspace_bytes, dbias, stream, nullptr, queue);
+  const TnSplit sp{dW1, ldw1, tapstride1, out_layout1, accumulate1, n1_cut};
+  const int rc = gemm_tn_launch(dtype, dY, ldy, X, ldx, dW0, ldw0, tapstride0, M, N1, N2, taps, Lin, Lout, stride, pad, mode, 0, out_layout0, accumulate0,
+                                workspace, workspace_bytes, dbias, stream, &sp, queue);
+  if (rc != kTnNoPartials) return rc;
+  const long esz = dtype == OSUF_DT_BF16 ? 2 : 4;
+  if (int rc0 = gemm_tn_launch(dtype, dY, ldy, X, ldx, dW0, ldw0, tapstride0, M, n1_cut, N2, taps, Lin, Lout, stride, pad, mode, 0, out_layout0,
+                               accumulate0, workspace, workspace_bytes, dbias, stream)) return rc0;
+  return gemm_tn_launch(dtype, static_cast<const char*>(dY) + n1_cut * esz, ldy, X, ldx, dW1, ldw1, tapstride1, M, N1 - n1_cut, N2, taps, Lin, Lout,
+                        stride, pad, mode, 0, out_layout1, accumulate1, workspace, workspace_bytes, dbias ? dbias + n1_cut : nullptr, stream);
+}
diff --git a/osufusion_amd/functional.py b/osufusion_amd/functional.py
--- a/osufusion_amd/functional.py
+++ b/osufusion_amd/functional.py
@@ -251,6 +251,9 @@
     return dw, db
 
 
+STACK_QKV_WGRAD = True
+
+
 def conv_wgrad(dy, x, w, kind: str, direct: bool = True, bias_out: Optional[torch.Tensor] = None):
     B, Lin, Cin = x.shape
     conv = w.dim() == 3
@@ -263,6 +266,20 @@
         grad_done(w)
         return None
     return g if conv else g[0]
+
+
+def conv_wgrad_stacked(dy, x, w0, w1) -> bool:
+    t0, t1 = grad_target(w0), grad_target(w1)
+    k0 = w0.shape[2] if w0.dim() == 3 else 1
+    k1 = w1.shape[2] if w1.dim() == 3 else 1
+    n0, n1 = w0.shape[0], w1.shape[0]
+    if t0 is None or t1 is None or k0 != 1 or k1 != 1 or n0 % 8 or n1 % 8 or dy.shape[-1] != n0 + n1 or w0.shape[1] != w1.shape[1]:
+        return False
+    B, L, _ = x.shape
+    ops.gemm_tn(dy, x, lin=L, lout=L, out=t0, conv_layout=w0.dim() == 3, accumulate=True, out2=t1, n1_cut=n0, conv_layout2=w1.dim() == 3,
+                accumulate2=True)
+    grad_done(w0); grad_done(w1)
+    return True
 
 
 class Adapter:
@@ -836,8 +853,10 @@
         dqkv = ops.mqa_bwd(qkv_r, o, do16, lse, B, N, H, D, scale, dt, cos, sin, variant=variant, delta=delta,
                            kv_heads=G, qs=ctx.qs, workspace=ctx.dq_ws)
         ctx.dq_ws = None
-        dwq = conv_wgrad(dqkv[..., : H * D], xn, wq, "same") if need[3] else None
-        dwkv = conv_wgrad(dqkv[..., H * D:], xn, wkv, "same") if need[4] else None
+        dwq = dwkv = None
+        if not (STACK_QKV_WGRAD and need[3] and need[4] and conv_wgrad_stacked(dqkv, xn, wq, wkv)):
+            dwq = conv_wgrad(dqkv[..., : H * D], xn, wq, "same") if need[3] else None
+            dwkv = conv_wgrad(dqkv[..., H * D:], xn, wkv, "same") if need[4] else None
         aq, akv = ctx.aq, ctx.akv
         packs = AttentionFn._qkv_packs(cache, dt, wq, wkv, aq, akv, ctx.base)
         gq = gkv = (None, None, None)
diff --git a/osufusion_amd/ops.py b/osufusion_amd/ops.py
--- a/osufusion_amd/ops.py
+++ b/osufusion_amd/ops.py
@@ -231,35 +231,118 @@
 
 def gemm_tn(dy: torch.Tensor, x: torch.Tensor, *, taps: int = 1, lin: Optional[int] = None, lout: Optional[int] = None, stride: int = 1,
             pad: int = 0, mode: int = 0, n1: Optional[int] = None, out: Optional[torch.Tensor] = None, conv_layout: bool = False,
-            accumulate: bool = False, bias_out: Optional[torch.Tensor] = None) -> torch.Tensor:
+            accumulate: bool = False, bias_out: Optional[torch.Tensor] = None, out2: Optional[torch.Tensor] = None,
+            n1_cut: Optional[int] = None, conv_layout2: Optional[bool] = None, accumulate2: Optional[bool] = None,
+            queue: Optional["WgradQueue"] = None):
+    if (out2 is None) != (n1_cut is None):
+        raise ValueError("gemm_tn: out2 and n1_cut go together")
+    if n1_cut is not None and (n1_cut <= 0 or n1_cut % 2):
+        raise ValueError(f"gemm_tn: n1_cut must be positive and even (bf16-pair partial tiles hold rows n1, n1 + 1 in one dword), got {n1_cut}")
     M, N1, ldy = _rows(dy)
     Mx, N2, ldx = _rows(x)
     if n1 is not None:
         N1 = n1
+    if n1_cut is not None and n1_cut >= N1:
+        raise ValueError(f"gemm_tn: n1_cut must lie inside (0, {N1}), got {n1_cut}")
     if lin is None:
         lin = lout = M
     assert dy.dtype == x.dtype and Mx // lin == M // lout
-    shape = (N1, N2, taps) if conv_layout else (taps, N1, N2)
+    R0 = N1 if n1_cut is None else n1_cut
     if out is None:
         assert not accumulate
-        out = torch.empty(shape, dtype=torch.float32, device=dy.device)
-    assert out.dtype == torch.float32 and out.is_contiguous() and out.numel() == taps * N1 * N2
-    need = _lib.load().osuf_gemm_tn_workspace_bytes(gemm_dt(dy), M, N1, N2, taps)
-    ws = _workspace(need, dy.device) if need > 0 else None
-    args = (gemm_dt(dy), _p(dy), ldy, _p(x), ldx, _p(out), N2, N1 * N2, M, N1, N2, taps, lin, lout, stride, pad, mode, 0,
-            1 if conv_layout else 0, 1 if accumulate else 0, _p(ws), need if ws is not None else 0)
+        out = torch.empty((R0, N2, taps) if conv_layout else (taps, R0, N2), dtype=torch.float32, device=dy.device)
+    assert out.dtype == torch.float32 and out.is_contiguous() and out.numel() == taps * R0 * N2
     if bias_out is not None:
         assert bias_out.dtype == torch.float32 and bias_out.is_contiguous() and bias_out.numel() == N1
-        call("osuf_gemm_tn_bias", *args, _p(bias_out), _stream())
-    else:
-        call("osuf_gemm_tn", *args, _stream())
-    return out
+    need = _lib.load().osuf_gemm_tn_workspace_bytes(gemm_dt(dy), M, N1, N2, taps)
+    if out2 is None and queue is None:
+        ws = _workspace(need, dy.device) if need > 0 else None
+        args = (gemm_dt(dy), _p(dy), ldy, _p(x), ldx, _p(out), N2, N1 * N2, M, N1, N2, taps, lin, lout, stride, pad, mode, 0,
+                1 if conv_layout else 0, 1 if accumulate else 0, _p(ws), need if ws is not None else 0)
+        if bias_out is not None:
+            call("osuf_gemm_tn_bias", *args, _p(bias_out), _stream())
+        else:
+            call("osuf_gemm_tn", *args, _stream())
+        return out
+    conv2 = conv_layout if conv_layout2 is None else conv_layout2
+    acc2 = accumulate if accumulate2 is None else accumulate2
+    if out2 is not None:
+        assert out2.dtype == torch.float32 and out2.is_contiguous() and out2.numel() == taps * (N1 - R0) * N2
+    if queue is not None and queue.room() < 2:
+        queue.flush()
+    ws = None
+    if need > 0:
+        ws = queue.region(need, dy.device) if queue is not None else _workspace(need, dy.device)
+    call("osuf_gemm_tn_split", gemm_dt(dy), _p(dy), ldy, _p(x), ldx, _p(out), N2, R0 * N2, 1 if conv_layout else 0, 1 if accumulate else 0,
+         _p(out2), N2, (N1 - R0) * N2, 1 if conv2 else 0, 1 if acc2 else 0, n1_cut or 0, M, N1, N2, taps, lin, lout, stride, pad, mode,
+         _p(ws), need if ws is not None else 0, _p(bias_out), queue.ptr if queue is not None else None, _stream())
+    return out if out2 is None else (out, out2)
+
+
+WGRAD_DESC = np.dtype([("ws", "<u8"), ("dW", "<u8"), ("N1", "<i4"), ("N2", "<i4"), ("taps", "<i4"), ("splits", "<i4"), ("row0", "<i4"),
+                       ("rows", "<i4"), ("kind", "<i4"), ("accumulate", "<i4"), ("wg0", "<i4"), ("wgs", "<i4"), ("reserved0", "<i4"),
+                       ("reserved1", "<i4")])
+WGRAD_QUEUE_MAX = 16
+WGRAD_QUEUE = np.dtype([("n", "<i4"), ("total_wgs", "<i4"), ("reserved", "<i8"), ("d", WGRAD_DESC, (WGRAD_QUEUE_MAX,))])
+
+
+class WgradQueue:
+
+    def __init__(self):
+        self.tab = np.zeros(1, dtype=WGRAD_QUEUE)
+        self.ptr = self.tab.ctypes.data
+        self.offset = 0
+        self._keep = []
+
+    def __len__(self) -> int:
+        return int(self.tab["n"][0])
+
+    def room(self) -> int:
+        return WGRAD_QUEUE_MAX - len(self)
+
+    def entries(self) -> np.ndarray:
+        return self.tab["d"][0][:len(self)]
+
+    def region(self, nbytes: int, device) -> torch.Tensor:
+        global _WS_FLOOR
+        ws = _workspace(self.offset + nbytes, device, whole=True)
+        if not any(k is ws for k in self._keep):
+            self._keep.append(ws)
+        view = ws[self.offset // 4:]
+        self.offset += (nbytes + 255) // 256 * 256
+        _WS_FLOOR = self.offset
+        return view
+
+    def push(self, ws: torch.Tensor, pk: bool, N1: int, N2: int, taps: int, splits: int, out: torch.Tensor, conv_layout: bool = False,
+             accumulate: bool = False, out2: Optional[torch.Tensor] = None, n1_cut: int = 0, conv_layout2: bool = False,
+             accumulate2: bool = False) -> None:
+        call("osuf_wgrad_queue_push", self.ptr, _p(ws), 1 if pk else 0, N1, N2, taps, splits, _p(out), 1 if conv_layout else 0,
+             1 if accumulate else 0, _p(out2), 1 if conv_layout2 else 0, 1 if accumulate2 else 0, n1_cut)
+
+    def reset(self) -> None:
+        global _WS_FLOOR
+        self.tab["n"][0] = self.tab["total_wgs"][0] = 0
+        self.offset = 0
+        self._keep.clear()
+        _WS_FLOOR = 0
+
+    def flush(self) -> None:
+        global _WS_FLOOR
+        if len(self):
+            call("osuf_wgrad_reduce_flush", self.ptr, _stream())
+        self.offset = 0
+        self._keep.clear()
+        _WS_FLOOR = 0
 
 
 _WS = {}
-
-
-def _workspace(nbytes: int, device) -> torch.Tensor:
+_WS_FLOOR = 0
+
+
+def _workspace(nbytes: int, device, whole: bool = False) -> torch.Tensor:
+    floor = 0 if whole else _WS_FLOOR
+    if floor:
+        return _workspace(floor + nbytes, device, whole=True)[floor // 4:]
     key = str(device)
     cur = _WS.get(key)
     if cur is None or cur.numel() * 4 < nbytes:
```

Measured after the change: 5.667 steps/s. No clear change (-0.2%).
